# BerkIGuler/AdaFortiTran

Hardware: AMD Instinct MI355X
Metric: OFDM frames/sec (120x14 grid, batch 128) + channel-estimation MSE vs reference (higher is better)
Workload: dtype f32; 1 GPU; C3: AdaFortiTran default config (6 layers, d=128, 4 heads, adaptive tokens), 120x14 grid, pilots 12x2; 128 frames per GPU per step; step = model(pilots_cpu, meta_cpu) through the module surface + device MSE partial; value = SURVEY 8(d)'s metric: H2D of pilots + meta INSIDE the step, output left on the device (= value_h2d_inclusive); the bare engine call on inputs resident in HBM is value_resident;; frames_per_gpu=128, global_batch=128, parallelism=frames sharded over 1 rank(s), lanes=1

## Files before the change

### adafortitran_amd/_abi.py

```python
from __future__ import annotations

import ctypes as C
from typing import Callable, Dict, Optional

AFT_ABI_VERSION = 10
AFT_ENGINE_PACKED, AFT_ENGINE_GENERAL = 0, 1
AFT_OK, AFT_ERR_ARG, AFT_ERR_SHAPE, AFT_ERR_HIP = 0, 1, 2, 3
AFT_ACT_RELU, AFT_ACT_GELU = 0, 1
AFT_ENCODER_AUTO, AFT_ENCODER_LAUNCHES, AFT_ENCODER_PLANE = 0, 1, 2
AFT_PRECISION_F32, AFT_PRECISION_BF16X3 = 0, 1

_fp = C.c_void_p


class AftConfig(C.Structure):
    _fields_ = [
        ("num_scs", C.c_int32), ("num_symbols", C.c_int32),
        ("pilot_scs", C.c_int32), ("pilot_symbols", C.c_int32),
        ("patch_scs", C.c_int32), ("patch_symbols", C.c_int32),
        ("num_layers", C.c_int32), ("model_dim", C.c_int32), ("num_head", C.c_int32),
        ("activation", C.c_int32), ("adaptive", C.c_int32),
        ("hidden", C.c_int32 * 3), ("encoder_path", C.c_int32), ("precision", C.c_int32),
    ]

# ... 76 lines not shown
        ("layers", C.POINTER(AftLayerWeights)),
    ]


def make_config(*, ofdm, pilot, patch, num_layers: int, model_dim: int, num_head: int,
                activation: str = "gelu", adaptive_hidden=None) -> AftConfig:
    cfg = AftConfig()
    cfg.num_scs, cfg.num_symbols = int(ofdm[0]), int(ofdm[1])
    cfg.pilot_scs, cfg.pilot_symbols = int(pilot[0]), int(pilot[1])
    cfg.patch_scs, cfg.patch_symbols = int(patch[0]), int(patch[1])
    cfg.num_layers, cfg.model_dim, cfg.num_head = int(num_layers), int(model_dim), int(num_head)
    cfg.activation = AFT_ACT_GELU if activation == "gelu" else AFT_ACT_RELU
    cfg.adaptive = 1 if adaptive_hidden is not None else 0
    for i in range(3):
        cfg.hidden[i] = int(adaptive_hidden[i]) if adaptive_hidden is not None else 0
    return cfg


def config_from_pydantic(system_config, model_config, adaptive: bool) -> AftConfig:
    return make_config(
        ofdm=(system_config.ofdm.num_scs, system_config.ofdm.num_symbols),
        pilot=(system_config.pilot.num_scs, system_config.pilot.num_symbols),
        patch=tuple(model_config.patch_size), num_layers=model_config.num_layers,
        model_dim=model_config.model_dim, num_head=model_config.num_head,
        activation=model_config.activation,
        adaptive_hidden=tuple(model_config.channel_adaptivity_hidden_sizes) if adaptive else None)


_ENC = ("snr_encoder", "ds_encoder", "dop_encoder")
_TE = "transformer_encoder"


def make_weights(cfg: AftConfig, ptr: Callable[[str], int], pos_key: Optional[str] = None) -> AftWeights:
    w = AftWeights()
    w.up_w, w.up_b = ptr("pilot_upsampler.weight"), ptr("pilot_upsampler.bias")
    for i, slot in enumerate((0, 2, 4, 6)):
        w.enh_w[i] = ptr(f"initial_enhancer.conv_block.{slot}.weight")
        w.enh_b[i] = ptr(f"initial_enhancer.conv_block.{slot}.bias")
        w.ref_w[i] = ptr(f"final_refiner.conv_block.{slot}.weight")
        w.ref_b[i] = ptr(f"final_refiner.conv_block.{slot}.bias")
    if cfg.adaptive:
        for e, enc in enumerate(_ENC):
            for j, slot in enumerate((0, 2, 4)):
                w.ada_w[e][j] = ptr(f"channel_adapter.{enc}.{slot}.weight")
                w.ada_b[e][j] = ptr(f"channel_adapter.{enc}.{slot}.bias")
    w.lin1_w, w.lin1_b = ptr(f"{_TE}.linear_1.weight"), ptr(f"{_TE}.linear_1.bias")
    w.lin2_w, w.lin2_b = ptr(f"{_TE}.linear_2.weight"), ptr(f"{_TE}.linear_2.bias")
    w.pos = ptr(pos_key or f"{_TE}.positional_encoding.position_embeddings")
    table = (AftLayerWeights * cfg.num_layers)()
    w.layers = C.cast(table, C.POINTER(AftLayerWeights))
    w._layer_table = table
    for i in range(cfg.num_layers):
        lp = f"{_TE}.transformer.layers.{i}"
        lw = table[i]
        lw.in_proj_w, lw.in_proj_b = ptr(lp + ".self_attn.in_proj_weight"), ptr(lp + ".self_attn.in_proj_bias")
        lw.out_proj_w, lw.out_proj_b = ptr(lp + ".self_attn.out_proj.weight"), ptr(lp + ".self_attn.out_proj.bias")
        lw.lin1_w, lw.lin1_b = ptr(lp + ".linear1.weight"), ptr(lp + ".linear1.bias")
        lw.lin2_w, lw.lin2_b = ptr(lp + ".linear2.weight"), ptr(lp + ".linear2.bias")
        lw.norm1_w, lw.norm1_b = ptr(lp + ".norm1.weight"), ptr(lp + ".norm1.bias")
        lw.norm2_w, lw.norm2_b = ptr(lp + ".norm2.weight"), ptr(lp + ".norm2.bias")
    return w


def pos_key_of(state: Dict[str, object]) -> str:
    k = f"{_TE}.positional_encoding.position_embeddings"
    return k if k in state else f"{_TE}.positional_encoding.pe"


vp = C.c_void_p
cfgp, wp, lwp, lgp = C.POINTER(AftConfig), C.POINTER(AftWeights), C.POINTER(AftLayerWeights), C.POINTER(AftLayerGrads)
p3, p4, p9, i3 = C.POINTER(vp * 3), C.POINTER(vp * 4), C.POINTER(vp * 9), C.POINTER(C.c_int32 * 3)
i6 = [C.c_int] * 6
SIGNATURES = {
    "aft_version": (C.c_int, []),
    "aft_last_error": (C.c_char_p, []),
    "aft_check_config": (C.c_int, [cfgp]),
    "aft_engine_of": (C.c_int, [cfgp]),
    "aft_set_switch": (C.c_int, [C.c_char_p, C.c_char_p]),
    "aft_get_switch": (C.c_int, [C.c_char_p, C.c_char_p, C.c_size_t]),
    "aft_max_batch": (C.c_int, [cfgp]),
    "aft_workspace_bytes": (C.c_size_t, [cfgp, C.c_int]),
    "aft_workspace_bytes_layer_fused": (C.c_size_t, [cfgp, C.c_int]),
    "aft_layer_fused_of": (C.c_int, [cfgp, C.c_int]),
    "aft_workspace_lanes": (C.c_int, [cfgp, C.c_int, C.POINTER(C.c_int), C.POINTER(C.c_int), C.POINTER(C.c_size_t)]),
    "aft_workspace_region": (C.c_int, [cfgp, C.c_int, C.c_int, C.POINTER(C.c_size_t), C.POINTER(C.c_size_t)]),
    "aft_forward_f32": (C.c_int, [cfgp, wp, vp, vp, vp, vp, vp, vp, C.c_size_t, C.c_int, vp]),
    "aft_packed_weights_bytes": (C.c_size_t, [cfgp]),
    "aft_pack_weights_f32": (C.c_int, [cfgp, wp, vp, C.c_size_t, vp]),
    "aft_forward_prepacked_f32": (C.c_int, [cfgp, wp, vp, vp, vp, vp, vp, vp, vp, C.c_size_t, C.c_int, vp]),
    "aft_linear_forward_f32": (C.c_int, [vp, vp, vp, vp, C.c_int, C.c_int, C.c_int, vp]),
    "aft_mse_partial_f32": (C.c_int, [vp, vp, vp, C.c_longlong, vp]),
    "aft_pilot_gather_f32": (C.c_int, [vp, vp, vp, C.c_int, C.c_int, C.c_int, vp]),
    "aft_ls_mse_db_f32": (C.c_int, [vp, vp, vp, C.c_int, C.c_int, vp]),
    "aft_frame_gather_f32": (C.c_int, [vp, vp, vp, vp, vp, vp, C.c_int, C.c_longlong, C.c_int, C.c_int, vp]),
    "aft_channel_sim_f32": (C.c_int, [C.POINTER(AftChanSim), C.c_ulonglong] + [C.c_longlong] * 4 + [C.c_int, vp, vp, vp, vp]),
    "aft_channel_sim_group_f32": (C.c_int, [C.POINTER(AftChanSim), C.c_int, C.c_int, vp, C.c_ulonglong] + [C.c_longlong] * 4 +
                                  [C.c_int, vp, vp, vp, vp]),
    "aft_lmmse_table_floats": (C.c_size_t, [C.POINTER(AftLmmse)]),
    "aft_lmmse_f32": (C.c_int, [C.POINTER(AftLmmse), vp, vp, vp, vp, vp, vp, C.c_int, vp]),
    "aft_link_errors_f32": (C.c_int, [C.POINTER(AftLink), vp, vp, vp, vp, vp, C.c_int, vp]),
    "aft_link_soft_f32": (C.c_int, [C.POINTER(AftLink), vp, vp, vp, vp, vp, vp, C.c_int, vp, vp, C.c_int, vp]),
    "aft_link_decode_f32": (C.c_int, [C.POINTER(AftLink), vp, vp, C.c_int, C.c_int, C.c_ulonglong, C.c_ulonglong, C.c_float, vp, vp,
                                      C.c_int, vp]),
    "aft_link_ldpc_f32": (C.c_int, [C.POINTER(AftLink), vp, vp, C.c_int, C.c_int, vp, C.c_ulonglong, C.c_ulonglong, C.c_float, C.c_int,
                                    C.c_int, vp, vp, C.c_int, vp]),
    "aft_link_mrc_f32": (C.c_int, [C.POINTER(AftLink), vp, vp, vp, vp, vp, vp, vp, C.c_int, C.c_int, vp, vp, vp, C.c_int, vp]),
    "aft_link_harq_f32": (C.c_int, [C.POINTER(AftLink), vp, vp, C.c_int, C.c_int, vp, C.c_int, C.c_int, vp, C.c_ulonglong, C.c_ulonglong,
                                    C.c_float, C.c_int, C.c_int, vp, vp, C.c_int, vp]),
    "aft_link_sm_f32": (C.c_int, [C.POINTER(AftLink), vp, vp, vp, vp, vp, vp, vp, vp, C.c_int, C.c_int, C.c_int, vp, vp, vp, C.c_int, vp]),
    "aft_link_joint_f32": (C.c_int, [C.POINTER(AftLink), vp, vp, vp, vp, vp, vp, vp, C.c_int, C.c_int, C.c_int, vp, vp, vp, C.c_int, vp]),
    "aft_encoder_tape_bytes": (C.c_size_t, [cfgp, C.c_int]),
    "aft_encoder_train_scratch_bytes": (C.c_size_t, [cfgp, C.c_int]),
    "aft_encoder_layer_fwd_train_f32": (C.c_int, [cfgp, lwp, vp, vp, vp, C.c_size_t, vp, C.c_size_t, C.c_int, C.c_float, C.c_uint64, vp]),
    "aft_encoder_layer_fwd_train_chained_f32": (C.c_int, [cfgp, lwp, vp, vp, vp, C.c_size_t, vp, C.c_size_t, C.c_int, C.c_float, C.c_uint64,
                                                          C.c_int, lwp, vp, C.c_size_t, C.POINTER(C.c_int), vp]),
    "aft_encoder_layer_bwd_f32": (C.c_int, [cfgp, lwp, vp, vp, C.c_size_t, vp, vp, lgp, C.c_int, vp, C.c_size_t, C.c_int, C.c_float,
                                            C.c_uint64, vp]),
    "aft_dense_fwd_f32": (C.c_int, [vp, vp, vp, vp, C.c_int, C.c_int, C.c_int, vp]),
    "aft_dense_bwd_scratch_bytes": (C.c_size_t, [C.c_int, C.c_int, C.c_int]),
    "aft_dense_bwd_f32": (C.c_int, [vp, vp, vp, vp, vp, vp, C.c_int, vp, C.c_size_t, C.c_int, C.c_int, C.c_int, vp]),
    "aft_conv_enhancer_fwd_scratch_bytes": (C.c_size_t, [C.c_int, C.c_int, C.c_int]),
    "aft_conv_enhancer_fwd_train_f32": (C.c_int, [p4, p4, vp, vp, vp, vp, vp, vp, C.c_size_t, C.c_int, C.c_int, C.c_int, vp]),
    "aft_conv_enhancer_scratch_bytes": (C.c_size_t, [C.c_int, C.c_int, C.c_int]),
    "aft_conv_enhancer_bwd_f32": (C.c_int, [p4, vp, vp, vp, vp, vp, vp, p4, p4, C.c_int, vp, C.c_size_t, C.c_int, C.c_int, C.c_int, vp]),
    "aft_adapter_fwd_train_f32": (C.c_int, [p3, p9, p9, i3, C.c_int, C.c_int, vp, vp, vp, vp]),
    "aft_adapter_bwd_f32": (C.c_int, [p3, p9, p9, i3, C.c_int, C.c_int, vp, vp, vp, vp, vp, p9, p9, C.c_int, vp]),
    "aft_embed_bwd_scratch_bytes": (C.c_size_t, i6 + [C.c_int]),
    "aft_embed_fwd_train_f32": (C.c_int, [vp] * 6 + i6 + [vp]),
    "aft_embed_bwd_f32": (C.c_int, [vp] * 9 + [C.c_int, vp, C.c_size_t] + i6 + [vp]),
    "aft_tail_bwd_scratch_bytes": (C.c_size_t, i6),
    "aft_tail_fwd_train_f32": (C.c_int, [vp] * 5 + i6 + [vp]),
    "aft_tail_bwd_f32": (C.c_int, [vp] * 6 + [C.c_int, vp, C.c_size_t] + i6 + [vp]),
    "aft_adam_step_f32": (C.c_int, [vp, vp, vp, vp, C.c_size_t] + [C.c_float] * 6 + [C.c_int, vp]),
    "aft_grad_sumsq_scratch_bytes": (C.c_size_t, [C.c_size_t]),
    "aft_grad_sumsq_f32": (C.c_int, [vp, C.c_size_t, vp, C.c_size_t, vp, vp, vp]),
    "aft_adam_prepare_f32": (C.c_int, [vp, vp, vp, vp, C.c_double, C.c_double, C.c_float, C.c_float, vp]),
    "aft_adam_step_ctrl_f32": (C.c_int, [vp, vp, vp, vp, C.c_size_t] + [C.c_float] * 5 + [vp, vp]),
    "aft_grad_clip_f32": (C.c_int, [vp, C.c_size_t, vp, C.c_double, C.c_double, vp, vp]),
    "aft_stage_upsample_f32": (C.c_int, [cfgp, wp, vp, vp, C.c_int, vp]),
    "aft_stage_adapter_f32": (C.c_int, [cfgp, wp, vp, vp, vp, vp, C.c_int, vp]),
    "aft_stage_embed_f32": (C.c_int, [cfgp, wp, vp, vp, vp, C.c_int, vp]),
    "aft_stage_encoder_layer_f32": (C.c_int, [cfgp, wp, C.c_int, vp, vp, C.c_size_t, C.c_int, vp]),
    "aft_stage_tail_f32": (C.c_int, [cfgp, wp, vp, vp, vp, C.c_int, vp]),
    "aft_profile_kernel_f32": (C.c_int, [cfgp, wp, C.c_int, vp, vp, C.c_size_t, C.c_int, C.c_int, vp]),
    "aft_debug_fill_lds_f32": (C.c_int, [C.c_float, vp]),
    "aft_debug_peek_lds_f32": (C.c_int, [vp, C.c_int, C.c_int, vp]),
}
EXPORTED_SYMBOLS = tuple(SIGNATURES)
REGION_IDS = {"conv_enhanced": 0, "tokens6": 1, "enc_out": 2}
KERNEL_IDS = {"upsample": 0, "embed": 1, "qkv": 2, "attention": 3, "chain": 4, "tail": 5, "chain_last": 6, "prologue": 8}
```

### adafortitran_amd/csrc/aft_api.hip

```cpp
#include <algorithm>
#include <atomic>
#include <cstdlib>
#include <cstdarg>
#include <cstdio>
#include <cstring>
#include <mutex>
#include <string>
#include <vector>

#include "aft_internal.h"

namespace aft {

static thread_local char g_err[512] = "";

void set_error(const char *fmt, ...) {
    va_list ap;
    va_start(ap, fmt);
    vsnprintf(g_err, sizeof(g_err), fmt, ap);
    va_end(ap);
}

int hip_fail(const char *what, hipError_t e) {
    set_error("%s: %s", what, hipGetErrorString(e));
// ... 252 lines not shown
    p.planned = p.total;
    for (int i = 0; i < p.lanes && layer_fused_ok(c); ++i) {
        const size_t block = (size_t)2 * p.frames[i] * round_up(tokens_of(c), kTile) * c.model_dim;
        p.x_pt[i] = p.take(block);
        p.vt2[i] = p.take(block);
    }
    return p;
}
static size_t workspace_floats_any_lanes(const aft_config &c, int batch, bool fused_blocks) {
    size_t m = 0;
    for (int l = 1; l <= kMaxLanes; ++l) {
        const LanePlan lp = plan_lanes(c, batch, l);
        m = std::max(m, fused_blocks ? lp.total : lp.planned);
    }
    return m;
}
struct LaneStreams {
    hipStream_t side[kMaxLanes - 1];
    hipEvent_t fork, join[kMaxLanes - 1];
    int n_side;
};
namespace {
constexpr int kLaneCacheMax = 16;
struct LaneEntry { bool used; int dev; hipStream_t user; LaneStreams ls; int in_use; unsigned long long tick; };
std::mutex g_lane_mu;
LaneEntry g_lane_cache[kLaneCacheMax];
unsigned long long g_lane_tick = 0;
void destroy_lane_streams(LaneStreams &ls) {
    for (int i = 0; i < ls.n_side; ++i) {
        (void)hipEventDestroy(ls.join[i]);
        (void)hipStreamDestroy(ls.side[i]);
    }
    if (ls.fork) (void)hipEventDestroy(ls.fork);
    ls = LaneStreams{};
}
bool grow_lane_streams(LaneStreams &ls, int sides) {
    if (ls.fork == nullptr && hipEventCreateWithFlags(&ls.fork, hipEventDisableTiming) != hipSuccess) { ls.fork = nullptr; return false; }
    while (ls.n_side < sides) {
        hipStream_t s = nullptr;
        hipEvent_t e = nullptr;
        if (hipStreamCreateWithFlags(&s, hipStreamNonBlocking) != hipSuccess) return false;
        if (hipEventCreateWithFlags(&e, hipEventDisableTiming) != hipSuccess) { (void)hipStreamDestroy(s); return false; }
        ls.side[ls.n_side] = s;
        ls.join[ls.n_side] = e;
        ++ls.n_side;
    }
    return true;
}
}
static LaneStreams *acquire_lane_streams(hipStream_t user, int lanes) {
    int dev = 0;
    if (hipGetDevice(&dev) != hipSuccess) return nullptr;
    std::lock_guard<std::mutex> lock(g_lane_mu);
    LaneEntry *hit = nullptr, *victim = nullptr;
    for (auto &en : g_lane_cache) {
        if (en.used && en.dev == dev && en.user == user) { hit = &en; break; }
        if (!en.used) { if (victim == nullptr || victim->used) victim = &en; }
        else if (en.in_use == 0 && (victim == nullptr || (victim->used && en.tick < victim->tick))) victim = &en;
    }
    if (hit == nullptr) {
        if (victim == nullptr) return nullptr;
        if (victim->used) destroy_lane_streams(victim->ls);
        *victim = LaneEntry{true, dev, user, LaneStreams{}, 0, 0};
        hit = victim;
    }
    if (!grow_lane_streams(hit->ls, lanes - 1)) {
        if (hit->in_use == 0) {
            destroy_lane_streams(hit->ls);
            hit->used = false;
        }
        return nullptr;
    }
    ++hit->in_use;
    hit->tick = ++g_lane_tick;
    return &hit->ls;
}
static void release_lane_streams(LaneStreams *ls) {
    if (ls == nullptr) return;
    std::lock_guard<std::mutex> lock(g_lane_mu);
    for (auto &en : g_lane_cache)
        if (&en.ls == ls) { --en.in_use; return; }
}

static bool l0_fold_selected(const aft_config &c) {
    return packed_engine_ok(c) && c.precision == AFT_PRECISION_F32 && switch_int(SW_L0_FOLD, 1) != 0;
}
static L0Fold l0_fold_at(const aft_config &c, const Workspace &ws, float *base) {
    float *tables = base + ws.attn;
    return L0Fold{tables, tables + (size_t)ws.tokpad * c.model_dim, base + ws.wpack + (size_t)c.model_dim * c.model_dim};
}

enum ChainPos { kChainFirst, kChainMiddle, kChainLast };
static ChainFusion chain_fusion_for(ChainPos pos, const aft_config &c, const WeightsDev &w, const Workspace &ws, float *base) {
    ChainFusion f{};
    f.x_blocked = true;
    if (pos == kChainFirst) {
        f.conv_enhanced = base + ws.conv_enhanced;
        f.tokens6 = c.adaptive ? base + ws.tokens6 : nullptr;
        f.lin1_w = w.lin1_w; f.lin1_b = w.lin1_b; f.pos = w.pos;
    } else if (pos == kChainLast) {
        f.lin2_w = w.lin2_w; f.lin2_b = w.lin2_b; f.out6 = base + ws.out6;
    }
    return f;
}

static int run_encoder(const aft_config &c, const WeightsDev &w, const aft_layer_weights *layers, const Workspace &ws, float *base, float *x,
                       int first_layer, int last_layer, hipStream_t st, bool fused = false, const float *prepacked = nullptr,
                       float *x_pt = nullptr, float *vt2 = nullptr, const L0Fold *fold = nullptr) {
    float *attn = base + ws.attn, *q = base + ws.q, *k = base + ws.k, *vt = base + ws.vt;
    const int rows = ws.planes * ws.tokens;
    const size_t pl = packed_layer_floats(c.model_dim);
    const float *wp = prepacked != nullptr ? prepacked : base + ws.wpack;
    if (prepacked == nullptr)
        STEP("pack_weights", launch_pack_weights(c, layers + first_layer, base + ws.wpack + first_layer * pl, last_layer - first_layer + 1, st));
    ChainFusion first = chain_fusion_for(kChainFirst, c, w, ws, base);
    const ChainFusion middle = chain_fusion_for(kChainMiddle, c, w, ws, base), last = chain_fusion_for(kChainLast, c, w, ws, base);
    if (fused && fold != nullptr && first_layer == 0) {
        first.fold_tk = fold->tk; first.fold_tvt = fold->tvt; first.fold_w = fold->wf;
    }
    if (fused && x_pt != nullptr && x == base + ws.x && first_layer == 0 && last_layer == c.num_layers - 1 &&
        layer_fused_selected(c, ws.planes / 2)) {
        x = x_pt;
        float *kbuf[2] = {k, attn}, *vbuf[2] = {vt, vt2};
        STEP("chain(qkv, plane tiles)", launch_chain_plane_tiles(c, &layers[0], wp, x, q, kbuf[0], vbuf[0], ws.planes, ws.tokens, ws.tokpad, st, &first));
        for (int l = 0; l <= last_layer; ++l) {
            const bool more = l < last_layer;
            STEP("layer", launch_layer(c, &layers[l], wp + l * pl, more ? &layers[l + 1] : nullptr, more ? wp + (l + 1) * pl : nullptr, x, q,
                                       kbuf[l & 1], vbuf[l & 1], kbuf[(l + 1) & 1], vbuf[(l + 1) & 1], ws.planes, ws.tokens, ws.tokpad, st,
                                       more ? &middle : &last));
        }
        return AFT_OK;
    }
    STEP("chain(qkv)", launch_chain(c, nullptr, nullptr, &layers[first_layer], wp + first_layer * pl, nullptr, x, q, k, vt, rows,
                                    ws.tokens, ws.tokpad, st, fused ? &first : nullptr));
    for (int l = first_layer; l <= last_layer; ++l) {
        STEP("attention", launch_attention(c, q, k, vt, layers[l].in_proj_b, attn, ws.planes, ws.tokens, ws.tokpad, st));
        const bool more = l < last_layer;
        STEP("chain(mlp)", launch_chain(c, &layers[l], wp + l * pl, more ? &layers[l + 1] : nullptr, more ? wp + (l + 1) * pl : nullptr, attn,
                                        x, q, k, vt, rows, ws.tokens, ws.tokpad, st, fused ? (more ? &middle : &last) : nullptr));
    }
    return AFT_OK;
}

static int general_layer(const aft_config &c, const aft_layer_weights &lw, const Workspace &ws, float *base, float *x, hipStream_t st) {
    const int rows = ws.planes * ws.tokens, d = c.model_dim, ff = 2 * d;
    float *qkv = base + ws.g_qkv, *attn = base + ws.attn, *y = base + ws.g_y, *x1 = base + ws.g_x1, *s = base + ws.g_s,
          *stats = base + ws.g_stats, *a = base + ws.g_a, *hd = base + ws.g_hd;
    STEP("general: in-projection", launch_gemm(0, x, lw.in_proj_w, qkv, lw.in_proj_b, rows, 3 * d, d, d, d, 3 * d, false, st));
    STEP("general: attention", launch_attn_train_fwd(c, qkv, attn, base + ws.g_lse, ws.planes, ws.tokens, 0.f, 0u, st, base + ws.g_pad));
    STEP("general: out-projection", launch_gemm(0, attn, lw.out_proj_w, y, lw.out_proj_b, rows, d, d, d, d, d, false, st));
    STEP("general: norm1", launch_add_ln_fwd(x, y, lw.norm1_w, lw.norm1_b, s, stats, x1, rows, d, 1e-5f, 0.f, 0u, st));
    STEP("general: linear1", launch_gemm(0, x1, lw.lin1_w, a, lw.lin1_b, rows, ff, d, d, d, ff, false, st));
    STEP("general: activation", launch_act_fwd(c.activation, a, hd, rows, ff, 0.f, 0u, st));
    STEP("general: linear2", launch_gemm(0, hd, lw.lin2_w, y, lw.lin2_b, rows, d, ff, ff, ff, d, false, st));
    STEP("general: norm2", launch_add_ln_fwd(x1, y, lw.norm2_w, lw.norm2_b, s, stats, x, rows, d, 1e-5f, 0.f, 0u, st));
    return AFT_OK;
}
static int run_encoder_general(const aft_config &c, const WeightsDev &w, const aft_layer_weights *layers, const Workspace &ws, float *base,
                               int batch, hipStream_t st) {
    float *x = base + ws.x;
    const int rows = ws.planes * ws.tokens, d = c.model_dim, p = c.patch_scs * c.patch_symbols;
    STEP("general: embedding", launch_embed_any(c, w, base + ws.conv_enhanced, c.adaptive ? base + ws.tokens6 : nullptr, x, batch, st));
    for (int l = 0; l < c.num_layers; ++l) {
        const int rc = general_layer(c, layers[l], ws, base, x, st);
        if (rc != AFT_OK) return rc;
    }
    STEP("general: linear_2", launch_gemm(0, x, w.lin2_w, base + ws.out6, w.lin2_b, rows, p, d, d, d, out6_stride(c), false, st));
    return AFT_OK;
}

}

using namespace aft;

extern "C" {

int aft_version(void) { return AFT_ABI_VERSION; }

const char *aft_last_error(void) { return g_err; }

int aft_check_config(const aft_config *cfg) { return check_config(cfg); }

int aft_engine_of(const aft_config *cfg) {
    if (check_config(cfg) != AFT_OK) return -1;
    return packed_engine_ok(*cfg) ? AFT_ENGINE_PACKED : AFT_ENGINE_GENERAL;
}

int aft_set_switch(const char *name, const char *value) {
    const int i = name == nullptr ? -1 : switch_id(name);
    if (i < 0) {
        set_error("aft_set_switch: %s is not a switch (adafortitran_amd/csrc/switches.h lists them)", name ? name : "(null)");
        return AFT_ERR_ARG;
    }
    std::lock_guard<std::mutex> lock(g_switch_mu);
    store_switch(i, value);
    return AFT_OK;
}

int aft_get_switch(const char *name, char *buf, size_t n) {
    const int i = name == nullptr ? -1 : switch_id(name);
    if (i < 0) return -1;
    std::lock_guard<std::mutex> lock(g_switch_mu);
    if (!g_switch_on[i].load(std::memory_order_relaxed)) return 0;
    if (buf != nullptr && n > 0) {
        strncpy(buf, g_switch_text[i].c_str(), n - 1);
        buf[n - 1] = 0;
    }
    return 1;
}

int aft_max_batch(const aft_config *cfg) {
    if (check_config(cfg) != AFT_OK) return 0;
    return max_batch_of(*cfg);
}

size_t aft_workspace_bytes(const aft_config *cfg, int batch) {
    if (check_config(cfg) != AFT_OK || batch <= 0) return 0;
    return workspace_floats_any_lanes(*cfg, batch, false) * sizeof(float);
}

int aft_workspace_region(const aft_config *cfg, int batch, int region, size_t *offset_bytes, size_t *size_bytes) {
    int rc = check_config(cfg);
    if (rc != AFT_OK) return rc;
    if (batch <= 0 || !offset_bytes || !size_bytes) {
        set_error("aft_workspace_region: bad batch or NULL result pointer");
        return AFT_ERR_ARG;
    }
    const Workspace ws = plan_workspace(*cfg, batch);
    size_t off = 0;
    switch (region) {
        case AFT_REGION_CONV_ENHANCED: off = ws.conv_enhanced; break;
        case AFT_REGION_TOKENS6: off = ws.tokens6; break;
        case AFT_REGION_ENC_OUT: off = ws.out6; break;
        default: set_error("aft_workspace_region: unknown region %d", region); return AFT_ERR_ARG;
    }
    *offset_bytes = off * sizeof(float);
    *size_bytes = ws.floats_at(off) * sizeof(float);
    return AFT_OK;
}

size_t aft_workspace_bytes_layer_fused(const aft_config *cfg, int batch) {
    if (check_config(cfg) != AFT_OK || batch <= 0) return 0;
    return workspace_floats_any_lanes(*cfg, batch, true) * sizeof(float);
}

int aft_layer_fused_of(const aft_config *cfg, int batch) {
    if (check_config(cfg) != AFT_OK || batch <= 0) return -1;
    return layer_fused_selected(*cfg, batch) ? 1 : 0;
}

int aft_workspace_lanes(const aft_config *cfg, int batch, int *lanes, int *frames, size_t *offset_bytes) {
    int rc = check_config(cfg);
    if (rc != AFT_OK) return rc;
    if (batch <= 0 || !lanes || !frames || !offset_bytes) {
        set_error("aft_workspace_lanes: bad batch or NULL result pointer");
        return AFT_ERR_ARG;
    }
    static_assert(kMaxLanes == AFT_MAX_LANES, "header and implementation disagree");
    const LanePlan lp = plan_lanes(*cfg, batch, lanes_wanted(*cfg, batch));
    *lanes = lp.lanes;
    for (int i = 0; i < kMaxLanes; ++i) {
        frames[i] = i < lp.lanes ? lp.frames[i] : 0;
        offset_bytes[i] = i < lp.lanes ? lp.ws_off[i] * sizeof(float) : 0;
    }
    return AFT_OK;
}

static int forward_lane(const aft_config *cfg, const aft_weights *w, const float *prepacked, const float *pilots, const float *snr,
                        const float *ds, const float *dop, float *out, float *base, int batch, hipStream_t st, float *x_pt, float *vt2) {
    const Workspace ws = plan_workspace(*cfg, batch);
    const bool general = !packed_engine_ok(*cfg);
    const WeightsDev wd = weights_window(*w, 0, cfg->num_layers);
    float *wpack = prepacked != nullptr || general ? nullptr : base + ws.wpack;
    float *lent = x_holds_planes(*cfg, ws) ? base + ws.x : nullptr;
    float *up_planes = prologue_upsample_ok(*cfg, wd) ? lent : nullptr;
    const bool fold_on = l0_fold_selected(*cfg);
    const L0Fold fold = fold_on ? l0_fold_at(*cfg, ws, base) : L0Fold{};
    STEP("prologue(adapter + pack_weights + upsampler product)",
         launch_prologue(*cfg, wd, snr, ds, dop, base + ws.tokens6, batch, wpack, pilots, up_planes, st, base + ws.convfrag,
                         fold_on ? &fold : nullptr));
    if (wpack != nullptr && cfg->num_layers > kLayerWindow)
        STEP("pack_weights(layers beyond the prologue's window)",
             launch_pack_weights(*cfg, w->layers + kLayerWindow, wpack + packed_layer_floats(cfg->model_dim) * kLayerWindow,
                                 cfg->num_layers - kLayerWindow, st));
    STEP("upsample", launch_upsample(*cfg, wd, pilots, base + ws.conv_enhanced, batch, st, lent, up_planes != nullptr, base + ws.convfrag));
    const int rc = general ? run_encoder_general(*cfg, wd, w->layers, ws, base, batch, st)
                           : run_encoder(*cfg, wd, w->layers, ws, base, base + ws.x, 0, cfg->num_layers - 1, st, true,
                                         prepacked != nullptr ? prepacked : wpack, x_pt, vt2, fold_on ? &fold : nullptr);
    if (rc != AFT_OK) return rc;
    STEP("tail", launch_tail(*cfg, wd, nullptr, base + ws.conv_enhanced, out, batch, st, base + ws.out6, base + ws.convfrag + kConvFragFloats));
    return AFT_OK;
}

static int forward_impl(const aft_config *cfg, const aft_weights *w, const float *prepacked, const float *pilots,
                        const float *snr, const float *ds, const float *dop, float *out, void *workspace,
                        size_t workspace_bytes, int batch, void *stream) {
    int rc = check_config(cfg);
    if (rc != AFT_OK) return rc;
    AFT_REQUIRE(w && pilots && out && workspace, "NULL pointer argument");
    AFT_REQUIRE(batch > 0, "batch must be positive (got %d)", batch);
    AFT_REQUIRE(batch <= max_batch_of(*cfg), "batch %d exceeds aft_max_batch = %d for this configuration (32-bit buffer "
                "offsets: no workspace region may reach 2 GiB); split the batch", batch, max_batch_of(*cfg));
    AFT_REQUIRE(!cfg->adaptive || (snr && ds && dop), "meta_data is required when channel adaptation is enabled");
    hipStream_t user = static_cast<hipStream_t>(stream);
    AFT_REQUIRE(w->layers != nullptr, "aft_weights.layers is NULL (host array of num_layers entries)");
    const LanePlan lp = plan_lanes(*cfg, batch, lanes_wanted(*cfg, batch));
    AFT_REQUIRE(workspace_bytes >= lp.planned * sizeof(float), "workspace too small: %zu < %zu bytes (aft_workspace_bytes)",
                workspace_bytes, lp.planned * sizeof(float));
    const bool fused_blocks = lp.total > lp.planned && workspace_bytes >= lp.total * sizeof(float);
    LaneStreams *ls = lp.lanes > 1 ? acquire_lane_streams(user, lp.lanes) : nullptr;
    struct Lease { LaneStreams *p; ~Lease() { release_lane_streams(p); } } lease{ls};
    if (ls != nullptr) {
        hipError_t ef = hipEventRecord(ls->fork, user);
        for (int i = 1; i < lp.lanes && ef == hipSuccess; ++i) ef = hipStreamWaitEvent(ls->side[i - 1], ls->fork, 0);
        if (ef != hipSuccess) return hip_fail("lanes(fork)", ef);
    }
    const int pil_floats = 2 * cfg->pilot_scs * cfg->pilot_symbols, out_floats = 2 * cfg->num_scs * cfg->num_symbols;
#ifdef AFT_CHECKED
    {
        int covered = 0;
        for (int i = 0; i < lp.lanes; ++i) {
            const Workspace wl = plan_workspace(*cfg, lp.frames[i]);
            AFT_HOST_ASSERT(lp.first[i] == covered && lp.frames[i] > 0, "lane shares are not a partition of the batch");
            covered += lp.frames[i];
            AFT_HOST_ASSERT(lp.ws_off[i] % 64 == 0 && (lp.ws_off[i] + wl.total) * sizeof(float) <= workspace_bytes, "lane slice outside the workspace");
            AFT_HOST_ASSERT(i + 1 == lp.lanes || lp.ws_off[i] + wl.total <= lp.ws_off[i + 1], "lane slices overlap");
            AFT_HOST_ASSERT(check_layout(wl, workspace_bytes - lp.ws_off[i] * sizeof(float)), "workspace region outside its slice");
        }
        AFT_HOST_ASSERT(covered == batch, "lane shares do not cover the batch");
        AFT_HOST_ASSERT(!fused_blocks || check_layout(lp, workspace_bytes), "fused layer sequence's blocks outside the workspace");
    }
#endif
    int result = AFT_OK;
    for (int i = 0; i < lp.lanes; ++i) {
        const int f0 = lp.first[i];
        const int rc_lane = forward_lane(cfg, w, prepacked, pilots + (size_t)f0 * pil_floats, snr ? snr + f0 : nullptr, ds ? ds + f0 : nullptr,
                                         dop ? dop + f0 : nullptr, out + (size_t)f0 * out_floats, static_cast<float *>(workspace) + lp.ws_off[i],
                                         lp.frames[i], i == 0 || ls == nullptr ? user : ls->side[i - 1],
                                         fused_blocks ? static_cast<float *>(workspace) + lp.x_pt[i] : nullptr,
                                         fused_blocks ? static_cast<float *>(workspace) + lp.vt2[i] : nullptr);
        if (rc_lane != AFT_OK && result == AFT_OK) result = rc_lane;
    }
    if (ls != nullptr) {
        hipError_t ej = hipSuccess;
        for (int i = 1; i < lp.lanes && ej == hipSuccess; ++i) {
            ej = hipEventRecord(ls->join[i - 1], ls->side[i - 1]);
            if (ej == hipSuccess) ej = hipStreamWaitEvent(user, ls->join[i - 1], 0);
        }
        if (ej != hipSuccess && result == AFT_OK) return hip_fail("lanes(join)", ej);
    }
    return result;
}

int aft_forward_f32(const aft_config *cfg, const aft_weights *w, const float *pilots, const float *snr,
                    const float *ds, const float *dop, float *out, void *workspace, size_t workspace_bytes,
                    int batch, void *stream) {
    return forward_impl(cfg, w, nullptr, pilots, snr, ds, dop, out, workspace, workspace_bytes, batch, stream);
}

size_t aft_packed_weights_bytes(const aft_config *cfg) {
// ... 87 lines not shown
                           int batch, void *stream) {
    int rc = check_config(cfg);
    if (rc != AFT_OK) return rc;
    AFT_REQUIRE(w && pilots && conv_enhanced && batch > 0, "bad argument");
    hipError_t e = launch_upsample(*cfg, weights_window(*w, 0, 0), pilots, conv_enhanced, batch, static_cast<hipStream_t>(stream));
    return e == hipSuccess ? AFT_OK : hip_fail("upsample", e);
}

int aft_stage_adapter_f32(const aft_config *cfg, const aft_weights *w, const float *snr, const float *ds,
                          const float *dop, float *tokens6, int batch, void *stream) {
    int rc = check_config(cfg);
    if (rc != AFT_OK) return rc;
    AFT_REQUIRE(cfg->adaptive, "adapter stage needs an adaptive config");
    AFT_REQUIRE(w && snr && ds && dop && tokens6 && batch > 0, "bad argument");
    hipError_t e = launch_adapter(*cfg, weights_window(*w, 0, 0), snr, ds, dop, tokens6, batch, static_cast<hipStream_t>(stream));
    return e == hipSuccess ? AFT_OK : hip_fail("adapter", e);
}

int aft_stage_embed_f32(const aft_config *cfg, const aft_weights *w, const float *conv_enhanced,
                        const float *tokens6, float *x, int batch, void *stream) {
    int rc = check_config(cfg);
    if (rc != AFT_OK) return rc;
    AFT_REQUIRE(w && conv_enhanced && x && batch > 0, "bad argument");
    AFT_REQUIRE(!cfg->adaptive || tokens6, "adaptive config needs tokens6");
    hipError_t e = packed_engine_ok(*cfg) ? launch_embed(*cfg, weights_window(*w, 0, 0), conv_enhanced, tokens6, x, batch, static_cast<hipStream_t>(stream))
                                          : launch_embed_any(*cfg, weights_window(*w, 0, 0), conv_enhanced, tokens6, x, batch, static_cast<hipStream_t>(stream));
    return e == hipSuccess ? AFT_OK : hip_fail("embed", e);
}

int aft_stage_encoder_layer_f32(const aft_config *cfg, const aft_weights *w, int layer, float *x, void *scratch,
                                size_t scratch_bytes, int batch, void *stream) {
    int rc = check_config(cfg);
    if (rc != AFT_OK) return rc;
    AFT_REQUIRE(w && w->layers && x && scratch && batch > 0, "bad argument");
    AFT_REQUIRE(layer >= 0 && layer < cfg->num_layers, "layer %d out of range", layer);
    AFT_REQUIRE(batch <= max_batch_of(*cfg), "batch %d exceeds aft_max_batch = %d", batch, max_batch_of(*cfg));
    const Workspace ws = plan_workspace(*cfg, batch);
    AFT_REQUIRE(scratch_bytes >= ws.total * sizeof(float), "scratch too small");
    float *base = static_cast<float *>(scratch);
    hipStream_t st = static_cast<hipStream_t>(stream);
    if (!packed_engine_ok(*cfg)) return general_layer(*cfg, w->layers[layer], ws, base, x, st);
    return run_encoder(*cfg, weights_window(*w, 0, 0), w->layers, ws, base, x, layer, layer, st);
}

int aft_stage_tail_f32(const aft_config *cfg, const aft_weights *w, const float *x, const float *conv_enhanced,
                       float *out, int batch, void *stream) {
    int rc = check_config(cfg);
    if (rc != AFT_OK) return rc;
    AFT_REQUIRE(w && x && conv_enhanced && out && batch > 0, "bad argument");
    {
        const int p = cfg->patch_scs * cfg->patch_symbols;
        if (cfg->model_dim % 16 != 0 || !conv_plan_ok(cfg->num_scs, cfg->num_symbols, p * cfg->model_dim + p)) {
            set_error("aft_stage_tail_f32: linear_2 (%d x %d) does not fit the conv kernel's LDS beside the plane, or model_dim is not a "
                      "multiple of 16 -- only aft_forward_f32 serves this configuration", p, cfg->model_dim);
            return AFT_ERR_SHAPE;
        }
    }
    hipError_t e = launch_tail(*cfg, weights_window(*w, 0, 0), x, conv_enhanced, out, batch, static_cast<hipStream_t>(stream));
    return e == hipSuccess ? AFT_OK : hip_fail("tail", e);
}

int aft_profile_kernel_f32(const aft_config *cfg, const aft_weights *w, int which, float *out, void *workspace,
                           size_t workspace_bytes, int batch, int reps, void *stream) {
    int rc = check_config(cfg);
    if (rc != AFT_OK) return rc;
    AFT_REQUIRE(w && w->layers && workspace && batch > 0 && reps > 0, "bad argument");
    AFT_REQUIRE(batch <= max_batch_of(*cfg), "batch %d exceeds aft_max_batch = %d", batch, max_batch_of(*cfg));
    if (!packed_engine_ok(*cfg)) {
        set_error("aft_profile_kernel_f32 replays the packed engine's kernel classes; this configuration runs the general engine");
        return AFT_ERR_SHAPE;
    }
    const Workspace ws = plan_workspace(*cfg, batch);
    AFT_REQUIRE(workspace_bytes >= ws.total * sizeof(float), "workspace too small");
    const WeightsDev wd = weights_window(*w, 0, cfg->num_layers);
    AFT_REQUIRE(cfg->num_layers >= 2 || which != AFT_KERNEL_CHAIN, "chain profile needs >= 2 layers");
    hipStream_t st = static_cast<hipStream_t>(stream);
    float *base = static_cast<float *>(workspace);
    float *x = base + ws.x, *attn = base + ws.attn, *q = base + ws.q, *k = base + ws.k, *vt = base + ws.vt;
    const int rows = ws.planes * ws.tokens;
    float *lent = x_holds_planes(*cfg, ws) ? x : nullptr;
    const float *wp = base + ws.wpack;
    ChainFusion first = chain_fusion_for(kChainFirst, *cfg, wd, ws, base);
    const ChainFusion middle = chain_fusion_for(kChainMiddle, *cfg, wd, ws, base), last = chain_fusion_for(kChainLast, *cfg, wd, ws, base);
    const bool fold_on = l0_fold_selected(*cfg);
    const L0Fold fold = fold_on ? l0_fold_at(*cfg, ws, base) : L0Fold{};
    if (fold_on) { first.fold_tk = fold.tk; first.fold_tvt = fold.tvt; first.fold_w = fold.wf; }
    hipError_t e = hipSuccess;
    for (int i = 0; i < reps && e == hipSuccess; ++i) {
        switch (which) {
            case AFT_KERNEL_UPSAMPLE:
                AFT_REQUIRE(out != nullptr, "upsample profile needs the pilots pointer in `out`");
                e = launch_upsample(*cfg, wd, out, base + ws.conv_enhanced, batch, st, lent, prologue_upsample_ok(*cfg, wd), base + ws.convfrag);
                break;
            case AFT_KERNEL_EMBED:
                e = launch_embed(*cfg, wd, base + ws.conv_enhanced, cfg->adaptive ? base + ws.tokens6 : nullptr, x, batch, st);
                break;
            case AFT_KERNEL_QKV:
                e = launch_chain(*cfg, nullptr, nullptr, &w->layers[0], wp, nullptr, x, q, k, vt, rows, ws.tokens, ws.tokpad, st, &first);
                break;
            case AFT_KERNEL_ATTENTION:
                e = launch_attention(*cfg, q, k, vt, w->layers[0].in_proj_b, attn, ws.planes, ws.tokens, ws.tokpad, st);
                break;
            case AFT_KERNEL_CHAIN:
                e = launch_chain(*cfg, &w->layers[0], wp, &w->layers[1], wp + packed_layer_floats(cfg->model_dim), attn, x, q, k, vt, rows,
                                 ws.tokens, ws.tokpad, st, &middle);
                break;
            case AFT_KERNEL_CHAIN_LAST:
                e = launch_chain(*cfg, &w->layers[0], wp, nullptr, nullptr, attn, x, q, k, vt, rows, ws.tokens, ws.tokpad, st, &last);
                break;
            case AFT_KERNEL_PROLOGUE: {
                AFT_REQUIRE(out != nullptr, "prologue profile needs the pilots pointer in `out`");
                const float *cond = out + (size_t)batch * cfg->pilot_scs * cfg->pilot_symbols * 2;
                e = launch_prologue(*cfg, wd, cond, cond + batch, cond + 2 * batch, base + ws.tokens6, batch, base + ws.wpack, out,
                                    prologue_upsample_ok(*cfg, wd) && !switch_on(SW_PROLOGUE_NO_UP) ? lent : nullptr, st,
                                    base + ws.convfrag, fold_on ? &fold : nullptr);
                break;
            }
            case AFT_KERNEL_TAIL:
                AFT_REQUIRE(out != nullptr, "tail profile needs an output buffer");
                e = launch_tail(*cfg, wd, nullptr, base + ws.conv_enhanced, out, batch, st, base + ws.out6, base + ws.convfrag + kConvFragFloats);
                break;
            default:
                set_error("unknown kernel id %d", which);
                return AFT_ERR_ARG;
        }
    }
    return e == hipSuccess ? AFT_OK : hip_fail("profile", e);
}

}
```

### adafortitran_amd/csrc/aft_internal.h

```cpp
#pragma once

#include <hip/hip_runtime.h>

#include <cstddef>
#include <cstdint>

#include "../../include/adafortitran_amd.h"
#include "switches.h"
#ifdef AFT_DIAG_STAMPS
#include "stamp_report.h"
#endif

namespace aft {

using f32x2 = __attribute__((ext_vector_type(2))) float;
using f32x4 = __attribute__((ext_vector_type(4))) float;
using f32x16 = __attribute__((ext_vector_type(16))) float;

constexpr int kWave = 64;
constexpr int kHeadDim = 32;
constexpr int kTile = 32;
constexpr int kMaxPatchFeatures = 16;

inline __host__ __device__ int round_up(int v, int m) { return (v + m - 1) / m * m; }
// ... 109 lines not shown
            if (regions[i].off == off) return regions[i].floats;
        return 0;
    }
};
inline bool check_layout(const Layout &l, size_t bytes) {
    if (l.n > kMaxRegions || l.total % 64 != 0 || l.total * sizeof(float) > bytes) return false;
    for (int i = 0; i < l.n; ++i) {
        const size_t end = i + 1 < l.n ? l.regions[i + 1].off : l.total;
        if (l.regions[i].off % 64 != 0 || l.regions[i].off + l.regions[i].floats > end) return false;
    }
    return true;
}

inline int tokens_of(const aft_config &c) { return (c.num_scs / c.patch_scs) * (c.num_symbols / c.patch_symbols); }

struct Workspace : Layout {
    size_t conv_enhanced, tokens6, x, attn, q, k, vt, wpack, out6, convfrag;
    size_t g_x1, g_y, g_s, g_stats, g_qkv, g_lse, g_a, g_hd, g_pad;
    int tokens, tokpad, planes;
};

Workspace plan_workspace(const aft_config &c, int batch);

void set_error(const char *fmt, ...);
int hip_fail(const char *what, hipError_t e);
#define STEP(name, call)                                    \
    do {                                                    \
        hipError_t e_ = (call);                             \
        if (e_ != hipSuccess) return hip_fail(name, e_);    \
    } while (0)
#define AFT_REQUIRE(cond, ...) do { if (!(cond)) { set_error(__VA_ARGS__); return AFT_ERR_ARG; } } while (0)
int check_config(const aft_config *c);
bool packed_engine_ok(const aft_config &c);

constexpr int kLayerWindow = 32;
struct WeightsDev {
    const float *up_w, *up_b;
    const float *enh_w[4], *enh_b[4];
    const float *ref_w[4], *ref_b[4];
    const float *ada_w[3][3], *ada_b[3][3];
    const float *lin1_w, *lin1_b;
    const float *pos;
    const float *lin2_w, *lin2_b;
    aft_layer_weights layers[kLayerWindow];
};
WeightsDev weights_window(const aft_weights &w, int first, int count);

constexpr int kMaxDevices = 64;
int current_device();
int current_device_cus();
struct PerDeviceOnce {
    unsigned long long done = 0;
    bool needed(int dev) const { return !((__atomic_load_n(&done, __ATOMIC_RELAXED) >> dev) & 1ull); }
    void mark(int dev) { __atomic_fetch_or(&done, 1ull << dev, __ATOMIC_RELAXED); }
};
hipError_t ensure_dynamic_lds(PerDeviceOnce &once, const void *kernel, size_t bytes);

#ifdef AFT_DIAG_STAMPS
enum StampKind { kStampChainQkv, kStampChainMlpQkv, kStampChainMlp, kStampAttn, kStampConv, kStampConvStream, kStampChainTrain, kStampKinds };
class StampRun {
public:
    StampRun(Switch sw, StampKind kind, long long rows, hipStream_t st);
    unsigned long long *buffer() const { return dev_; }
    const unsigned long long *collect();
private:
    unsigned long long *dev_ = nullptr;
    std::vector<unsigned long long> host_;
    StampKind kind_;
    long long rows_;
    hipStream_t st_;
};
#endif

constexpr size_t kConvFragFloats = 22 * 64 * 4 + 160;
hipError_t launch_upsample(const aft_config &c, const WeightsDev &w, const float *pilots,
                           float *conv_enhanced, int batch, hipStream_t st, float *scratch_planes = nullptr, bool planes_ready = false,
                           const float *conv_frag = nullptr);
hipError_t launch_adapter(const aft_config &c, const WeightsDev &w, const float *snr, const float *ds,
                          const float *dop, float *tokens6, int batch, hipStream_t st);
bool prologue_upsample_ok(const aft_config &c, const WeightsDev &w);
constexpr int kFoldSteps = (kMaxPatchFeatures + 6 + 1) / 2;
struct L0Fold {
    float *tk, *tvt, *wf;
};
hipError_t launch_prologue(const aft_config &c, const WeightsDev &w, const float *snr, const float *ds, const float *dop,
                           float *tokens6, int batch, float *packed, const float *pilots, float *up_planes, hipStream_t st,
                           float *conv_frag = nullptr, const L0Fold *fold = nullptr);
hipError_t launch_embed(const aft_config &c, const WeightsDev &w, const float *conv_enhanced,
                        const float *tokens6, float *x, int batch, hipStream_t st);
constexpr int kMaxPatchGeneral = 32;
hipError_t launch_embed_any(const aft_config &c, const WeightsDev &w, const float *conv_enhanced,
                            const float *tokens6, float *x, int batch, hipStream_t st);
struct ChainFusion {
    const float *conv_enhanced = nullptr, *tokens6 = nullptr, *lin1_w = nullptr, *lin1_b = nullptr, *pos = nullptr;
    const float *lin2_w = nullptr, *lin2_b = nullptr;
    float *out6 = nullptr;
    const float *fold_tk = nullptr, *fold_tvt = nullptr, *fold_w = nullptr;
    bool x_blocked = false;
};
inline int out6_stride(const aft_config &c) { return round_up(c.patch_scs * c.patch_symbols, 8); }
hipError_t launch_chain(const aft_config &c, const aft_layer_weights *mlp_w, const float *mlp_packed,
                        const aft_layer_weights *qkv_w, const float *qkv_packed, const float *attn, float *x,
                        float *q, float *k, float *vt, int rows, int tokens, int tokpad, hipStream_t st,
                        const ChainFusion *fuse = nullptr);
size_t packed_layer_floats(int d);
bool layer_fused_ok(const aft_config &c);
hipError_t launch_chain_plane_tiles(const aft_config &c, const aft_layer_weights *qkv_w, const float *qkv_packed, float *x, float *q,
                                    float *k, float *vt, int planes, int tokens, int tokpad, hipStream_t st, const ChainFusion *fuse);
hipError_t launch_layer(const aft_config &c, const aft_layer_weights *mlp_w, const float *mlp_packed, const aft_layer_weights *qkv_w,
                        const float *qkv_packed, float *x, float *q, const float *k_in, const float *vt_in, float *k_out, float *vt_out,
                        int planes, int tokens, int tokpad, hipStream_t st, const ChainFusion *fuse);
hipError_t launch_pack_weights(const aft_config &c, const aft_layer_weights *layers, float *packed, int count, hipStream_t st);
hipError_t launch_attention(const aft_config &c, const float *q, const float *k, const float *vt, const float *qbias,
                            float *attn, int planes, int tokens, int tokpad, hipStream_t st);
bool conv_plan_ok(int S, int T, int extra_floats);
hipError_t launch_tail(const aft_config &c, const WeightsDev &w, const float *x, const float *conv_enhanced,
                       float *out, int batch, hipStream_t st, const float *out6 = nullptr, const float *conv_frag = nullptr);
hipError_t launch_linear(const float *weight, const float *bias, const float *pilots, float *out, int batch,
                         int in_features, int out_features, hipStream_t st);
hipError_t launch_pilot_gather(const float *hzero_ls, float *pilots, int *counts, int batch, int grid_elems,
                               int expected, hipStream_t st);
hipError_t launch_ls_mse_db(const float *ls, const float *ideal, float *db, int batch, int grid_elems, hipStream_t st);
hipError_t launch_frame_gather(const float *ideal_all, const float *pilots_all, const long long *index, float *ideal_out,
                               float *pilots_out, int *flags, int batch, long long frames, int grid_elems, int pilot_elems,
                               hipStream_t st);
hipError_t launch_channel_sim(const aft_chansim &sim, unsigned long long seed, long long base, long long start, long long stride,
                              long long modulo, int batch, float *ideal, float *pilots, float *meta, hipStream_t st);
hipError_t launch_channel_sim_group(const aft_chansim &sim, int group, const float *mix_packed, unsigned long long seed, long long base,
                                    long long start, long long stride, long long modulo, int batch, float *ideal, float *pilots,
                                    float *meta, hipStream_t st);

size_t lmmse_fblock_floats(const aft_lmmse &plan);
size_t lmmse_tblock_floats(const aft_lmmse &plan);
hipError_t launch_lmmse(const aft_lmmse &plan, const float *tables, const float *pilots, const float *snr, const float *ds,
                        const float *dop, float *est, int batch, hipStream_t st);
hipError_t launch_link_errors(const aft_link &link, const float *ideal, const float *est, const unsigned long long *keys,
                              const float *sigma, int32_t *counts, int batch, hipStream_t st);
hipError_t launch_link_soft(const aft_link &link, const float *ideal, const float *est, const unsigned long long *keys,
                            const float *sigma, const float *scale, const float *factors, int n_factors, float *loss, float *llr,
                            int batch, hipStream_t st);
hipError_t launch_link_mrc(const aft_link &link, const float *ideal, const float *est, const unsigned long long *keys,
                           const float *sigma, const float *rho, const float *scale, const float *factors, int n_factors, int branches,
                           int32_t *counts, float *loss, float *llr, int batch, hipStream_t st);
int link_code_waves(unsigned steps, unsigned blocks);
hipError_t launch_link_decode(const aft_link &link, const float *llr, const unsigned long long *keys, int info_bits, int rate,
                              unsigned coded_bits, unsigned blocks, unsigned long long stride, float qgain, int32_t *counts,
                              unsigned char *bits, int batch, hipStream_t st);
int link_ldpc_waves(int base_cols, int edges, unsigned blocks);
hipError_t launch_link_ldpc(const aft_link &link, const float *llr, const unsigned long long *keys, int base_rows, int base_cols,
                            const int32_t *shifts, unsigned blocks, unsigned long long stride, float qgain, int offset, int max_iters,
                            int32_t *counts, unsigned char *bits, int batch, hipStream_t st);
int link_harq_waves(int base_cols, int edges, unsigned blocks);
hipError_t launch_link_harq(const aft_link &link, const float *llr, const unsigned long long *keys, int base_rows, int base_cols,
                            const int32_t *shifts, int tx_cols, int rounds, const int32_t *starts, unsigned blocks,
                            unsigned long long stride, float qgain, int offset, int max_iters, int32_t *counts, unsigned char *bits,
                            int batch, hipStream_t st);
hipError_t launch_link2(bool joint, const aft_link &link, const float *ideal, const float *est, const unsigned long long *keys,
                        const float *sigma, const float *rho, const float *scale, const float *reg, const float *factors, int n_factors,
                        int branches, int32_t *counts, float *loss, float *llr, int batch, hipStream_t st);
hipError_t launch_mse(const float *est, const float *ref, double *sum_sq, long long n_complex, hipStream_t st);
hipError_t launch_fill_lds(float value, hipStream_t st);
hipError_t launch_peek_lds(float *out, int workgroups, int n, hipStream_t st);


constexpr int kGemmMaxSlices = 256;
constexpr int kColsumMaxSlices = 1024;
int colsum_slices(int rows);
int gemm_split_slices(int rows, int tiles);
size_t gemm_tn_slice_floats(int M, int N, int R);
constexpr int kMaxReduceJobs = 12;
struct ReduceJobs;
struct ReduceBatchScope {
    ReduceJobs *jobs;
    ReduceBatchScope();
    ~ReduceBatchScope();
    hipError_t flush(hipStream_t st);
    ReduceBatchScope(const ReduceBatchScope &) = delete;
    ReduceBatchScope &operator=(const ReduceBatchScope &) = delete;
};
int ln_bwd_blocks(int rows);
hipError_t launch_gemm(int op, const float *A, const float *B, float *C, const float *bias, int M, int N, int K, int lda,
                       int ldb, int ldc, bool accumulate, hipStream_t st);
hipError_t launch_gemm_tn(const float *A, const float *B, float *C, float *slices, int M, int N, int R, int lda, int ldb,
                          bool accumulate, hipStream_t st);
bool gemm_add_ln_ok(int M, int N, int K, int lda, int ldb);
hipError_t launch_gemm_add_ln(const float *A, const float *W, const float *bias, const float *res, const float *gamma,
                              const float *beta, float *s_out, float *stats, float *out, int M, int N, int K, int lda, int ldw,
                              float eps, float keep_scale, uint32_t threshold, uint32_t seed, hipStream_t st);
bool gemm_act_ok(int M, int N, int K, int lda, int ldb, int ldc);
hipError_t launch_gemm_act(const float *A, const float *W, const float *bias, float *a_out, float *hd, int M, int N, int K, int lda,
                           int ldw, int ldc, int activation, float keep_scale, uint32_t threshold, uint32_t seed, hipStream_t st);
bool gemm_actbwd_ok(int M, int N, int K, int lda, int ldb, int ldc);
hipError_t launch_gemm_actbwd(const float *dy, const float *W, const float *a, float *da, int M, int N, int K, int lda, int ldw,
                              int ldc, int activation, float keep_scale, uint32_t threshold, uint32_t seed, hipStream_t st);
// ... 79 lines not shown
```

### adafortitran_amd/csrc/attn_device.h

```cpp
#pragma once
#include <math.h>

#include <type_traits>

#include "aft_internal.h"
#include "srd.h"
#include "stamps.h"

namespace aft {

#ifndef AFT_ATTN_WAVES
#define AFT_ATTN_WAVES 3
#endif

constexpr float kRescaleThreshold = 64.0f;
constexpr float kZeroRefThreshold = 32.0f;

__device__ __forceinline__ float other_half(float x) {
    const unsigned u = __builtin_bit_cast(unsigned, x);
    const auto r = __builtin_amdgcn_permlane32_swap(u, u, false, false);
    return __builtin_bit_cast(float, (threadIdx.x & 32) ? r[0] : r[1]);
}

__device__ __forceinline__ float max16(const f32x16 &v) {
    float m = __builtin_fmaxf(v[0], v[1]);
#pragma unroll
    for (int e = 2; e < 16; e += 2) m = __builtin_fmaxf(__builtin_fmaxf(m, v[e]), v[e + 1]);
    return m;
}

template <int NB, int NMF = 16 * NB>
__device__ __forceinline__ f32x16 qk_tile(const f32x4 (&kreg)[NB][4], const f32x4 (&qreg)[NB][4], bool zero_ref, float a_one,
                                          float neg_m) {
    f32x16 c;
    if (zero_ref) {
        c = mfma_f32(kreg[0][0][0], qreg[0][0][0], f32x16{0});
    } else {
        c = mfma_f32(a_one, neg_m, f32x16{0});
        c = mfma_f32(kreg[0][0][0], qreg[0][0][0], c);
    }
#pragma unroll
    for (int i = 1; i < NMF; ++i) c = mfma_f32(kreg[i >> 4][(i >> 2) & 3][i & 3], qreg[i >> 4][(i >> 2) & 3][i & 3], c);
    return c;
}

template <int NB>
struct AttnRow {
    float m_ref;
    f32x2 lsum2;
    f32x16 oacc[NB];
    bool zero_ref;
};

__device__ __forceinline__ f32x16 qk_tile_bs(const f32x4 (&kreg)[4], const f32x4 (&qreg)[4], bool zero_ref, float neg_m, int h) {
    f32x16 c = f32x16{0};
    if (!zero_ref) {
        bf16x8 one = {}, mref = {};
        one[0] = (__bf16)(h == 0 ? 1.0f : 0.0f);
        mref[0] = (__bf16)(h == 0 ? neg_m : 0.0f);
        c = __builtin_amdgcn_mfma_f32_32x32x16_bf16(one, mref, c, 0, 0, 0);
    }
#pragma unroll
    for (int m = 0; m < 2; ++m) {
        const bf16x8 kh = __builtin_bit_cast(bf16x8, kreg[2 * m]), kl = __builtin_bit_cast(bf16x8, kreg[2 * m + 1]);
        const bf16x8 qh = __builtin_bit_cast(bf16x8, qreg[2 * m]), ql = __builtin_bit_cast(bf16x8, qreg[2 * m + 1]);
        c = __builtin_amdgcn_mfma_f32_32x32x16_bf16(kh, qh, c, 0, 0, 0);
        c = __builtin_amdgcn_mfma_f32_32x32x16_bf16(kh, ql, c, 0, 0, 0);
        c = __builtin_amdgcn_mfma_f32_32x32x16_bf16(kl, qh, c, 0, 0, 0);
    }
    return c;
}
__device__ __forceinline__ float round_to_bf16(float x) { return (float)(__bf16)x; }

template <bool BS = false, int HD = 32, int TOK = 0, bool SINK = false>
__device__ __forceinline__ void attn_body(const float *__restrict__ q, const float *__restrict__ k,
                                          const float *__restrict__ vt, const float *__restrict__ qbias,
                                          float *__restrict__ out, int nblk, int tokens_rt, int tokpad_rt, int model_dim,
                                          float scale_log2e, const int first_task, const int total_waves, int ntasks,
                                          unsigned long long *stamps, const int tail_task = -1, float *sink = nullptr) {
    static_assert(!SINK || (!BS && HD == 32), "the LDS sink is instantiated for the fp32 head-dimension-32 body");
    int lane_l = threadIdx.x & 63;
    asm volatile("" : "+v"(lane_l));
    const int lane = lane_l;
    const Srd qs = make_srd(q), ks = make_srd(k), vs = make_srd(vt), os = make_srd(out);
    static_assert(HD % 8 == 0 && HD >= 8 && HD <= 64 && HD != 56, "head dimension");
    static_assert(!BS || HD == 32, "the split-precision tier is instantiated for head dimension 32");
    static_assert(HD != 16, "head dimension 16 runs attn16_body (attn16_device.h)");
    constexpr bool GEN = HD != 32 && HD != 64;
    constexpr int NS = HD / 8;
    constexpr int NB = GEN ? (32 % HD == 0 ? 1 : 2) : HD == 64 ? 2 : 1;
    constexpr int NQ = GEN ? (NS + 3) / 4 : NB;
    const int heads = model_dim / HD;
    const int tokens = TOK > 0 ? TOK : tokens_rt;
    const int tokpad = TOK > 0 ? (TOK + kTile - 1) / kTile * kTile : tokpad_rt;
    const int nkt = tokpad / kTile;
    const int r = lane & 31, h = lane >> 5;
    const bool ragged = (tokens & (kTile - 1)) != 0;
    const float a_one = h == 0 ? 1.0f : 0.0f;
    auto first_group = [&](int task) { const int ph = task / nkt, plane = ph / heads; return plane * nblk * 4 + (ph - plane * heads) * NS; };
    auto first_block = [&](int task) {
        if constexpr (GEN) return first_group(task) >> 2;
        return task / nkt * NB;
    };
    auto head_base = [&](int task) { return ((unsigned)first_block(task) * tokpad * kHeadDim + lane * 4) * 4; };
    const unsigned blk_bytes = (unsigned)tokpad * kHeadDim * 4;
    auto second_block_bytes = [&](int task) {
        if constexpr (GEN && NB == 2) return ((first_group(task) + NS - 1) >> 2) != first_block(task) ? blk_bytes : 0u;
        return blk_bytes;
    };
    auto load_tile = [&](Srd src, int kt, f32x4 (&dst)[NB][4], unsigned base, unsigned b1_bytes) {
#pragma unroll
        for (int b = 0; b < NB; ++b)
#pragma unroll
            for (int s = 0; s < 4; ++s) dst[b][s] = srd_load(src, base + b * b1_bytes + (unsigned)(kt * 1024 + s * 256) * 4);
    };
    constexpr int NMF = GEN ? 4 * NS : 16 * NB;
    auto load_qk = [&](Srd src, int kt, f32x4 (&dst)[NQ][4], unsigned base, int sub_) {
        if constexpr (GEN) {
#pragma unroll
            for (int i = 0; i < NS; ++i) {
                const int sl = sub_ + i;
                dst[i >> 2][i & 3] = srd_load(src, base + (unsigned)(sl >> 2) * blk_bytes + (unsigned)(kt * 1024 + (sl & 3) * 256) * 4);
            }
        } else {
            load_tile(src, kt, dst, base, blk_bytes);
        }
    };
    auto sub_of = [&](int task) {
        if constexpr (GEN) return first_group(task) & 3;
        return 0;
    };
    const bool pad8 = (tokens & 7) == 0;
    auto mask_logits = [&](f32x16 &sv, int kt) {
        if (pad8) {
#pragma unroll
            for (int g = 0; g < 4; ++g)
                if (kt * kTile + 8 * g >= tokens) sv[4 * g] = sv[4 * g + 1] = sv[4 * g + 2] = sv[4 * g + 3] = -INFINITY;
            return;
        }
#pragma unroll
        for (int e = 0; e < 16; ++e)
            if (kt * kTile + (e & 3) + 8 * (e >> 2) + 4 * h >= tokens) sv[e] = -INFINITY;
    };
    auto mask_values = [&](f32x4 (&vvb)[NB][4], int kt) {
      if (!BS && pad8) return;
#pragma unroll
      for (int b = 0; b < NB; ++b) {
        f32x4 (&vv)[4] = vvb[b];
        if constexpr (BS) {
#pragma unroll
            for (int sl = 0; sl < 4; ++sl) {
                bf16x8 e = __builtin_bit_cast(bf16x8, vv[sl]);
#pragma unroll
                for (int j = 0; j < 8; ++j)
                    if (kt * kTile + 16 * (sl >> 1) + 8 * (j >> 2) + 4 * h + (j & 3) >= tokens) e[j] = (__bf16)0.0f;
                vv[sl] = __builtin_bit_cast(f32x4, e);
            }
        } else {
#pragma unroll
            for (int g = 0; g < 4; ++g)
#pragma unroll
                for (int j = 0; j < 4; ++j)
                    if (kt * kTile + 8 * g + 4 * h + j >= tokens) vv[g][j] = 0.f;
        }
      }
    };

  const int rounds = SINK ? 1 : (ntasks + total_waves - 1) / total_waves + (tail_task >= 0 ? 1 : 0);
  int round = 0;
  int task = first_task < ntasks ? first_task : tail_task;
  f32x4 qreg[NQ][4], kcur[NQ][4], vcur[NB][4];
  if (task >= 0) {
      const unsigned hb0 = head_base(task);
      load_qk(qs, task % nkt, qreg, hb0, sub_of(task));
      load_qk(ks, 0, kcur, hb0, sub_of(task));
      load_tile(vs, 0, vcur, hb0, second_block_bytes(task));
  }
  for (; task >= 0; ++round) {
    AFT_STAMP(lane == 0, stamps, task, 0);
    AFT_STAMP_WALL(lane == 0, stamps, task, 6);
    const int qt = task % nkt;
    const int pb = first_block(task);
    const int sub = sub_of(task);
    const unsigned hb = head_base(task);
    const unsigned vb1 = second_block_bytes(task);
    const int next_task = SINK || task >= ntasks ? -1 : (task + total_waves < ntasks ? task + total_waves : tail_task);
    const bool has_next = next_task >= 0;

    if constexpr (!BS) {
        const float *bq = qbias + (pb % nblk) * kHeadDim + 4 * h + (GEN ? 8 * sub : 0);
#pragma unroll
        for (int b = 0; b < NQ; ++b)
#pragma unroll
            for (int s = 0; s < 4; ++s)
                if (4 * b + s < (GEN ? NS : 4 * NB))
                    qreg[b][s] = (qreg[b][s] + *reinterpret_cast<const f32x4 *>(bq + 32 * b + 8 * s)) * scale_log2e;
    }
    if (ragged && qt == nkt - 1 && qt * kTile + r >= tokens) {
#pragma unroll
        for (int b = 0; b < NQ; ++b)
#pragma unroll
            for (int s = 0; s < 4; ++s)
                if (4 * b + s < (GEN ? NS : 4 * NB)) qreg[b][s] = f32x4{0.f, 0.f, 0.f, 0.f};
    }

    AttnRow<NB> st;
    f32x16 sA, sB;
    if constexpr (BS) sA = qk_tile_bs(kcur[0], qreg[0], true, 0.f, h);
    else sA = qk_tile<NQ, NMF>(kcur, qreg, true, a_one, 0.f);
    if (nkt > 1) load_qk(ks, 1, kcur, hb, sub);
    if (ragged && nkt == 1) { mask_logits(sA, 0); mask_values(vcur, 0); }
    {
        float m0 = max16(sA);
        m0 = fmaxf(m0, other_half(m0));
        if constexpr (BS) m0 = round_to_bf16(m0);
        st.zero_ref = !__any(fabsf(m0) > kZeroRefThreshold);
        st.m_ref = st.zero_ref ? 0.f : m0;
        if (!st.zero_ref) {
#pragma unroll
            for (int e = 0; e < 16; ++e) sA[e] -= m0;
        }
    }
#pragma unroll
    for (int b = 0; b < NB; ++b) st.oacc[b] = f32x16{0};
    st.lsum2 = f32x2{0.f, 0.f};
    AFT_STAMP(lane == 0, stamps, task, 1);

    auto step = [&](auto fast, f32x16 &cur, f32x16 &nxt, int kt) {
        constexpr bool FAST = decltype(fast)::value;
        set_progress_priority((rounds - 1 - round) * nkt + (nkt - 1 - kt), rounds * nkt);
        const bool more = FAST || kt + 1 < nkt;
        if (more) {
            if constexpr (BS) nxt = qk_tile_bs(kcur[0], qreg[0], st.zero_ref, -st.m_ref, h);
            else nxt = qk_tile<NQ, NMF>(kcur, qreg, st.zero_ref, a_one, -st.m_ref);
            if (FAST || kt + 2 < nkt) load_qk(ks, kt + 2, kcur, hb, sub);
        } else if (has_next) {
            const unsigned hbn = head_base(next_task);
            load_qk(qs, next_task % nkt, qreg, hbn, sub_of(next_task));
            load_qk(ks, 0, kcur, hbn, sub_of(next_task));
        }
        const float tmax = max16(cur);
        if (__builtin_expect(__any(tmax > kRescaleThreshold), 0)) {
            const float tm = fmaxf(tmax, other_half(tmax));
            float grow = fmaxf(tm, 0.f);
            if constexpr (BS) grow = round_to_bf16(st.m_ref + grow) - st.m_ref;
            const float f = __builtin_amdgcn_exp2f(-grow);
            st.m_ref += grow;
            st.zero_ref = false;
#pragma unroll
            for (int e = 0; e < 16; ++e) {
                cur[e] -= grow;
                if (more) nxt[e] -= grow;
#pragma unroll
                for (int b = 0; b < NB; ++b) st.oacc[b][e] *= f;
            }
            st.lsum2 *= f;
        }
        if (!FAST && ragged && more && kt + 2 == nkt) mask_logits(nxt, kt + 1);
        f32x16 p;
// ... 82 lines not shown
```

### adafortitran_amd/csrc/chain_device.h

```cpp
#pragma once
#include "aft_internal.h"
#include "srd.h"
#include "stamps.h"

namespace aft {

template <int D>
struct ChainShape {
    static constexpr int WAVES = D / 32;
    static constexpr int THREADS = 64 * WAVES;
    static constexpr int XB = WAVES * 1024;
    static constexpr int HB = 2 * WAVES * 1024;
    static constexpr int ST = 32 * WAVES * 2;
    static constexpr int PAR = 4 * D;
    static constexpr size_t LDS_BYTES = sizeof(float) * (size_t)(XB + HB + ST + PAR);
};

struct ChainArgs {
    const float *attn;
    float *x;
    const float *wo, *w1, *w2, *wqkv;
    const float *bo, *b1, *b2, *g1, *be1, *g2, *be2;
    const float *bv;
    float *q, *k, *vt;
    int rows, tokens, tokpad, heads;
    int x_blocked;
    const float *lin2_w, *lin2_b;
    float *out6;
    int out6_features, out6_stride;
    const float *emb_conv, *emb_tok6, *emb_w1, *emb_b1, *emb_pos;
    int emb_S, emb_T, emb_p0, emb_p1, emb_K;
    const float *fold_tk;
    const float *fold_tvt;
    const float *fold_w;
    unsigned long long *stamps;
    int tpp;
};

ChainArgs make_chain_args(const aft_config &c, const aft_layer_weights *mlp_w, const float *mlp_packed, const aft_layer_weights *qkv_w,
                          const float *qkv_packed, const float *attn, float *x, float *q, float *k, float *vt, int rows, int tokens,
                          int tokpad, const ChainFusion *fuse);

template <int NT, int PFS>
struct WRing {
    f32x4 b[PFS + 1][NT];
};


template <int NKB, int NT, int PFS, int TS>
__device__ __forceinline__ void ring_load(WRing<NT, PFS> &ring, Srd w, unsigned w_lane, int step) {
    const int kb = step >> 2, s = step & 3;
#pragma unroll
    for (int t = 0; t < NT; ++t)
        ring.b[step % (PFS + 1)][t] = srd_load_c(w, w_lane, (unsigned)((t * TS * NKB + kb) * 1024 + s * 256) * 4);
}

template <int NKB, int NT, int PFS, int TS>
__device__ __forceinline__ void gemm_preload(WRing<NT, PFS> &ring, Srd w, unsigned w_lane) {
#pragma unroll
    for (int p = 0; p < PFS && p < 4 * NKB; ++p) ring_load<NKB, NT, PFS, TS>(ring, w, w_lane, p);
    __builtin_amdgcn_sched_barrier(0);
}

template <int NKB, int NT, int PFS, int TS, unsigned NORMAL, class Act, unsigned ZERO = 0>
__device__ __forceinline__ void gemm_run(WRing<NT, PFS> &ring, Srd w, unsigned w_lane, f32x16 (&acc)[NT], Act act) {
#pragma unroll
    for (int step = 0; step < 4 * NKB; ++step) {
        if (step + PFS < 4 * NKB) ring_load<NKB, NT, PFS, TS>(ring, w, w_lane, step + PFS);
        __builtin_amdgcn_sched_barrier(0);
        const f32x4 a = act(step >> 2, step & 3);
#pragma unroll
        for (int t = 0; t < NT; ++t)
#pragma unroll
            for (int j = 0; j < 4; ++j) {
                const float wv = ring.b[step % (PFS + 1)][t][j];
                if (((ZERO >> t) & 1) && step == 0 && j == 0)
                    acc[t] = (NORMAL >> t) & 1 ? __builtin_amdgcn_mfma_f32_32x32x2f32(a[j], wv, f32x16{0}, 0, 0, 0)
                                               : __builtin_amdgcn_mfma_f32_32x32x2f32(wv, a[j], f32x16{0}, 0, 0, 0);
                else
                    acc[t] = (NORMAL >> t) & 1 ? __builtin_amdgcn_mfma_f32_32x32x2f32(a[j], wv, acc[t], 0, 0, 0)
                                               : __builtin_amdgcn_mfma_f32_32x32x2f32(wv, a[j], acc[t], 0, 0, 0);
            }
        __builtin_amdgcn_sched_barrier(0);
    }
}

__device__ __forceinline__ void bs_publish(float *buf, int block, int lane, const f32x16 &v) {
#pragma unroll
    for (int m = 0; m < 2; ++m) {
        const BsFrag f = bs_split(f32x4{v[8 * m], v[8 * m + 1], v[8 * m + 2], v[8 * m + 3]},
                                  f32x4{v[8 * m + 4], v[8 * m + 5], v[8 * m + 6], v[8 * m + 7]});
        *reinterpret_cast<f32x4 *>(buf + (block * 4 + 2 * m) * 256 + lane * 4) = f.hi;
        *reinterpret_cast<f32x4 *>(buf + (block * 4 + 2 * m + 1) * 256 + lane * 4) = f.lo;
    }
}
__device__ __forceinline__ BsFrag bs_fetch(const float *buf, int kb, int m, int lane) {
    return BsFrag{*reinterpret_cast<const f32x4 *>(buf + (kb * 4 + 2 * m) * 256 + lane * 4),
                  *reinterpret_cast<const f32x4 *>(buf + (kb * 4 + 2 * m + 1) * 256 + lane * 4)};
}

template <int NKB, int NT, int PFS, int TS, unsigned NORMAL, class Act, unsigned ZERO = 0>
__device__ __forceinline__ void gemm_run_bs(WRing<NT, PFS> &ring, Srd w, unsigned w_lane, f32x16 (&acc)[NT], Act act) {
    BsFrag bfrag{};
#pragma unroll
    for (int step = 0; step < 4 * NKB; ++step) {
        if (step + PFS < 4 * NKB) ring_load<NKB, NT, PFS, TS>(ring, w, w_lane, step + PFS);
        __builtin_amdgcn_sched_barrier(0);
        const bool lo_step = step & 1;
        if (!lo_step) bfrag = act(step >> 2, (step & 3) >> 1);
        const bf16x8 bh = __builtin_bit_cast(bf16x8, bfrag.hi), bl = __builtin_bit_cast(bf16x8, bfrag.lo);
#pragma unroll
        for (int t = 0; t < NT; ++t) {
            const bf16x8 wv = __builtin_bit_cast(bf16x8, ring.b[step % (PFS + 1)][t]);
            const bool normal = (NORMAL >> t) & 1;
            if (((ZERO >> t) & 1) && step == 0)
                acc[t] = normal ? __builtin_amdgcn_mfma_f32_32x32x16_bf16(bh, wv, f32x16{0}, 0, 0, 0)
                                : __builtin_amdgcn_mfma_f32_32x32x16_bf16(wv, bh, f32x16{0}, 0, 0, 0);
            else
                acc[t] = normal ? __builtin_amdgcn_mfma_f32_32x32x16_bf16(bh, wv, acc[t], 0, 0, 0)
                                : __builtin_amdgcn_mfma_f32_32x32x16_bf16(wv, bh, acc[t], 0, 0, 0);
            if (!lo_step)
                acc[t] = normal ? __builtin_amdgcn_mfma_f32_32x32x16_bf16(bl, wv, acc[t], 0, 0, 0)
                                : __builtin_amdgcn_mfma_f32_32x32x16_bf16(wv, bl, acc[t], 0, 0, 0);
        }
        __builtin_amdgcn_sched_barrier(0);
    }
}

template <int D>
__device__ __forceinline__ void layernorm_rows(f32x16 &v, float *stats, const float *gamma, const float *beta,
                                               int wave, int r, int h) {
    constexpr int W = D / 32;
    float s = 0.f;
#pragma unroll
    for (int e = 0; e < 16; ++e) s += v[e];
    const float mp = s * (1.0f / 16.0f);
    float m2 = 0.f;
#pragma unroll
    for (int e = 0; e < 16; ++e) m2 = fmaf(v[e] - mp, v[e] - mp, m2);
    const float mo = __shfl_xor(mp, 32), m2o = __shfl_xor(m2, 32);
    const float dlt = mp - mo;
    if (h == 0) *reinterpret_cast<float2 *>(stats + (r * W + wave) * 2) = make_float2(0.5f * (mp + mo), m2 + m2o + 8.0f * dlt * dlt);
    __syncthreads();
    float mean = 0.f, msum = 0.f;
    float pm[W], pM[W];
#pragma unroll
    for (int u = 0; u < W; ++u) {
        const float2 p = *reinterpret_cast<const float2 *>(stats + (r * W + u) * 2);
        pm[u] = p.x;
        pM[u] = p.y;
        mean += p.x;
    }
    mean *= (1.0f / W);
#pragma unroll
    for (int u = 0; u < W; ++u) msum += pM[u] + 32.0f * (pm[u] - mean) * (pm[u] - mean);
    const float rstd = rsqrtf(msum * (1.0f / D) + 1e-5f);
#pragma unroll
    for (int s4 = 0; s4 < 4; ++s4) {
        const f32x4 g = *reinterpret_cast<const f32x4 *>(gamma + 8 * s4 + 4 * h);
        const f32x4 b = *reinterpret_cast<const f32x4 *>(beta + 8 * s4 + 4 * h);
#pragma unroll
        for (int j = 0; j < 4; ++j) v[4 * s4 + j] = (v[4 * s4 + j] - mean) * rstd * g[j] + b[j];
    }
}

__device__ __forceinline__ f32x16 bias_acc(Srd bias, int f0, int h) {
    f32x16 acc;
#pragma unroll
    for (int s = 0; s < 4; ++s) {
        const f32x4 b = srd_load(bias, (unsigned)(f0 + 8 * s + 4 * h) * 4);
#pragma unroll
        for (int j = 0; j < 4; ++j) acc[4 * s + j] = b[j];
    }
    return acc;
}

struct ChainNoPre {
    __device__ __forceinline__ void operator()(int) const {}
};

template <int D, int ACT, bool MLP, bool QKV, bool BS = false, bool PT = false, class Pre = ChainNoPre>
__device__ __forceinline__ void chain_body(const ChainArgs &a, float *smem, const int tid_in, const int first_tile,
                                           const int tile_stride, const int tile_end, Pre pre = Pre{}) {
    using S = ChainShape<D>;
    constexpr int W = S::WAVES;
    static_assert(!PT || !BS, "plane-aligned tiles are instantiated for the fp32 body");
    int tid = tid_in;
    asm volatile("" : "+v"(tid));
    float *xb = smem;
    float *hb = xb + S::XB;
    float *stats = hb + S::HB;
    float *par = stats + S::ST;

    int lane = tid & 63;
    const int w = __builtin_amdgcn_readfirstlane(tid >> 6);
    int r = lane & 31, h = lane >> 5;
    const int fb = 32 * w;

    const Srd srd_wo = make_srd(a.wo), srd_w1 = make_srd(a.w1), srd_w2 = make_srd(a.w2), srd_wq = make_srd(a.wqkv);
    const Srd srd_attn = make_srd(a.attn), srd_x = make_srd(a.x);
    const Srd srd_bo = make_srd(a.bo), srd_b1 = make_srd(a.b1), srd_b2 = make_srd(a.b2);
    const Srd srd_q = make_srd(a.q), srd_k = make_srd(a.k), srd_vt = make_srd(a.vt);
    const unsigned wo_off = (unsigned)w * W * 1024 + lane * 4, w1_off = (unsigned)(2 * w) * W * 1024 + lane * 4;
    const unsigned w2_off = (unsigned)w * (2 * W) * 1024 + lane * 4;
    const unsigned wq_off = (unsigned)w * W * 1024 + lane * 4;
    const Srd srd_bv = make_srd(a.bv);

    if constexpr (MLP) {
        for (int i = tid; i < D; i += S::THREADS) {
            par[i] = a.g1[i];
            par[D + i] = a.be1[i];
            par[2 * D + i] = a.g2[i];
            par[3 * D + i] = a.be2[i];
        }
        __syncthreads();
    }
    constexpr int kEmbSteps = kFoldSteps;
    constexpr int kFoldSteps0 = 6;
    float *emb_w = hb + S::XB;
    int *emb_offs = reinterpret_cast<int *>(emb_w + D * (kMaxPatchFeatures + 6));
    if constexpr (!MLP) {
        if (a.emb_conv != nullptr) {
            const int pk = a.emb_p0 * a.emb_p1;
            for (int i = tid; i < D * a.emb_K; i += S::THREADS) emb_w[i] = a.emb_w1[i];
            for (int k = tid; k < a.emb_K; k += S::THREADS)
                emb_offs[k] = k < pk ? (k / a.emb_p1) * a.emb_T + k % a.emb_p1 : ~(k - pk);
            __syncthreads();
        }
    }
    const int ntiles = (a.rows + 31) / 32;
    const int rounds = (tile_end - first_tile + tile_stride - 1) / tile_stride;
    int round = 0;
#ifndef AFT_CHAIN_PFK
#define AFT_CHAIN_PFK 0
#endif
    constexpr int PFK = MLP ? (AFT_CHAIN_PFK < W ? AFT_CHAIN_PFK : W) : 0;
    constexpr bool AHEAD = AFT_CHAIN_PFK > 0;
    static_assert(!PT || !AHEAD, "plane-aligned tiles request a tile's operands at the tile's start");
    f32x4 of[MLP ? W : 1][4], xres[4];
    auto request_attn = [&](int t, int kb0, int kb1) {
        const unsigned ap = ((unsigned)t * W * 1024 + lane * 4) * 4;
#pragma unroll
        for (int kb = 0; kb < W; ++kb)
#pragma unroll
            for (int s = 0; s < 4; ++s)
                if (kb >= kb0 && kb < kb1) of[kb][s] = srd_load_c(srd_attn, ap, (unsigned)(kb * 1024 + s * 256) * 4);
    };
    auto request_x_pt = [&](int t, int valid) {
        const unsigned xr = ((unsigned)t * 32 * D + w * 1024 + (min(r, valid - 1) + 32 * h) * 4) * 4;
#pragma unroll
        for (int s = 0; s < 4; ++s) xres[s] = srd_load(srd_x, xr + 1024 * s);
    };
    auto request_x = [&](int t) {
        if (a.x_blocked) {
            const unsigned xr = ((unsigned)t * 32 * D + w * 1024 + lane * 4) * 4;
#pragma unroll
            for (int s = 0; s < 4; ++s) xres[s] = srd_load(srd_x, xr + 1024 * s);
        } else {
            const unsigned xr = ((unsigned)min(t * 32 + r, a.rows - 1) * D + fb + 4 * h) * 4;
#pragma unroll
            for (int s = 0; s < 4; ++s) xres[s] = srd_load(srd_x, xr + 32 * s);
        }
    };
    auto request_tile = [&](int t) {
        if constexpr (MLP) request_attn(t, 0, PFK);
        if (MLP || a.emb_conv == nullptr) request_x(t);
    };
    if (AHEAD && first_tile < ntiles) request_tile(first_tile);
    f32x16 emb_acc0;
    float emb_bv[kEmbSteps];
    auto emb_request = [&](int t) {
        int plane, tok;
        if constexpr (PT) {
            plane = t / a.tpp;
            tok = min((t - plane * a.tpp) * 32 + r, a.tokens - 1);
        } else {
            const int grow_n = min(t * 32 + r, a.rows - 1);
            plane = grow_n / a.tokens;
            tok = grow_n - plane * a.tokens;
        }
        const int tpr = a.emb_T / a.emb_p1, g = tok / tpr, tc = tok - g * tpr;
        const float *cplane = a.emb_conv + ((size_t)plane * a.emb_S + g * a.emb_p0) * a.emb_T + tc * a.emb_p1;
        const float *t6 = a.emb_tok6 ? a.emb_tok6 + ((size_t)(plane >> 1) * a.tokens + tok) * 6 : nullptr;
#pragma unroll
        for (int s = 0; s < 4; ++s) {
            const f32x4 b = *reinterpret_cast<const f32x4 *>(a.emb_b1 + fb + 8 * s + 4 * h);
            const f32x4 ps = *reinterpret_cast<const f32x4 *>(a.emb_pos + (size_t)tok * D + fb + 8 * s + 4 * h);
#pragma unroll
            for (int j = 0; j < 4; ++j) emb_acc0[4 * s + j] = b[j] + ps[j];
        }
#pragma unroll
        for (int st = 0; st < kEmbSteps; ++st) {
            const int k = 2 * st + h;
            emb_bv[st] = 0.f;
            if (k < a.emb_K) {
                const int off = emb_offs[k];
                emb_bv[st] = off >= 0 ? cplane[off] : t6[~off];
            }
        }
    };
    if constexpr (!MLP) {
        if (a.emb_conv != nullptr && first_tile < tile_end) emb_request(first_tile);
    }
    bool fold = false;
    if constexpr (!MLP && !BS) fold = a.emb_conv != nullptr && a.fold_tk != nullptr;
    const Srd srd_tk = make_srd(a.fold_tk), srd_tvt = make_srd(a.fold_tvt), srd_fw = make_srd(a.fold_w);
    int pending_row0 = -1, pending_valid = 0;
    auto reduce_out6 = [&]() {
        const int P = a.out6_features;
        if (PT ? r < pending_valid : pending_row0 + r < a.rows) {
#pragma unroll
            for (int half = 0; half < 2; ++half) {
                const int f0 = 8 * half + 4 * h;
                if (f0 < P) {
                    f32x4 sum = *reinterpret_cast<const f32x4 *>(hb + lane * 8 + 4 * half);
#pragma unroll
                    for (int u = 1; u < W; ++u) {
                        const f32x4 t = *reinterpret_cast<const f32x4 *>(hb + (u * 64 + lane) * 8 + 4 * half);
                        sum += t;
                    }
#pragma unroll
                    for (int j = 0; j < 4; ++j) sum[j] += f0 + j < P ? a.lin2_b[f0 + j] : 0.f;
                    *reinterpret_cast<f32x4 *>(a.out6 + (size_t)(pending_row0 + r) * a.out6_stride + f0) = sum;
                }
            }
        }
    };
#pragma unroll 1
  for (int tile = first_tile; tile < tile_end; tile += tile_stride, ++round) {
    if constexpr (MLP && !QKV) {
        if (pending_row0 >= 0 && w == (round & (W - 1 < 3 ? W - 1 : 3))) reduce_out6();
    }
    pre(tile);
    if constexpr (PT && MLP) {
        int tid2 = tid_in;
        asm volatile("" : "+v"(tid2));
        lane = tid2 & 63;
        r = lane & 31;
        h = lane >> 5;
    }
#ifndef AFT_NO_PROGRESS_PRIORITY
    {
        const int left = rounds - 1 - round;
        if (left >= 3) __builtin_amdgcn_s_setprio(3);
        else if (left == 2) __builtin_amdgcn_s_setprio(2);
        else if (left == 1) __builtin_amdgcn_s_setprio(1);
        else __builtin_amdgcn_s_setprio(0);
    }
#endif
    const int row0 = tile * 32;
    const int grow = min(row0 + r, a.rows - 1);
    int plane_pt = 0, qt_pt = 0, valid_pt = 32;
    if constexpr (PT) {
        plane_pt = tile / a.tpp;
        qt_pt = tile - plane_pt * a.tpp;
        valid_pt = min(32, a.tokens - qt_pt * 32);
    }
    const bool row_ok = PT ? r < valid_pt : row0 + r < a.rows;
    const bool blocked = PT || a.x_blocked;
    const unsigned xrow = ((unsigned)grow * D + fb + 4 * h) * 4;
    unsigned lo = 0;
    asm volatile("" : "+v"(lo));
    const unsigned lo_lane = PT && MLP ? lo + lane * 4 : lo;
    const unsigned wo_lane = ((PT && MLP ? (unsigned)w * W * 1024 : wo_off) + lo_lane) * 4,
                   w1_lane = ((PT && MLP ? (unsigned)(2 * w) * W * 1024 : w1_off) + lo_lane) * 4,
                   w2_lane = ((PT && MLP ? (unsigned)w * (2 * W) * 1024 : w2_off) + lo_lane) * 4,
                   wq_lane = ((PT && MLP ? (unsigned)w * W * 1024 : wq_off) + lo_lane) * 4;
    AFT_STAMP(tid == 0, a.stamps, tile, 0);
    AFT_STAMP_WALL(tid == 0, a.stamps, tile, 12);
    AFT_STAMP_VALUE(tid == 0, a.stamps, tile, 14, ((unsigned long long)__builtin_amdgcn_s_getreg((4 << 0) | (0 << 6) | (31 << 11)) << 32) |
                                                      __builtin_amdgcn_s_getreg((20 << 0) | (0 << 6) | (31 << 11)));
#ifndef AFT_CHAIN_PFS
#define AFT_CHAIN_PFS 4
#endif
    constexpr int PFD = AFT_CHAIN_PFS, PFF = (AFT_CHAIN_PFS + 1) / 2, PFQ = (AFT_CHAIN_PFS + 2) / 3;
    WRing<1, PFD> ring_d;
    WRing<2, PFF> ring_ff;
    WRing<3, PFQ> ring_qkv;
    f32x16 cur;
    f32x16 acc[3];
    auto in_projection = [&]() {
        const float bias_v = __builtin_bit_cast(float, __builtin_amdgcn_raw_buffer_load_b32(srd_bv, (unsigned)(fb + r) * 4, 0, 0));
        float *xq = xb;
        if constexpr (!MLP) xq = (round & 1) ? hb : xb;
        if constexpr (BS) {
            bs_publish(xq, w, lane, cur);
        } else {
#pragma unroll
            for (int s = 0; s < 4; ++s)
                *reinterpret_cast<f32x4 *>(xq + (w * 4 + s) * 256 + lane * 4) = f32x4{cur[4 * s], cur[4 * s + 1], cur[4 * s + 2], cur[4 * s + 3]};
        }
        __syncthreads();
        AFT_STAMP(tid == 0, a.stamps, tile, 9);
        f32x16 vinit;
#pragma unroll
        for (int e = 0; e < 16; ++e) vinit[e] = bias_v;
        acc[2] = vinit;
        if constexpr (BS) {
            acc[0] = bias_acc(make_srd(a.bv - 2 * D), fb, h);
            auto xq_bs = [&](int kb, int m) { return bs_fetch(xq, kb, m, lane); };
            gemm_run_bs<W, 3, PFQ, W, 0x4, decltype(xq_bs), 0x2>(ring_qkv, srd_wq, wq_lane, acc, xq_bs);
        } else {
            auto xq_frag = [&](int kb, int s) { return *reinterpret_cast<const f32x4 *>(xq + (kb * 4 + s) * 256 + lane * 4); };
            gemm_run<W, 3, PFQ, W, 0x4, decltype(xq_frag), 0x3>(ring_qkv, srd_wq, wq_lane, acc, xq_frag);
        }
    };
    if constexpr (MLP) {
        f32x16 acc_o[1] = {bias_acc(srd_bo, fb, h)};
        gemm_preload<W, 1, PFD, 1>(ring_d, srd_wo, wo_lane);
        if constexpr (PT) {
            request_x_pt(tile, valid_pt);
        } else {
            request_attn(tile, AHEAD ? PFK : 0, W);
            if (!AHEAD) request_x(tile);
        }
        AFT_STAMP(tid == 0, a.stamps, tile, 1);
        if constexpr (BS)
            gemm_run_bs<W, 1, PFD, 1, 0>(ring_d, srd_wo, wo_lane, acc_o, [&](int kb, int m) { return bs_split(of[kb][2 * m], of[kb][2 * m + 1]); });
        else if constexpr (PT)
            gemm_run<W, 1, PFD, 1, 0>(ring_d, srd_wo, wo_lane, acc_o, [&](int kb, int s) {
                return *reinterpret_cast<const f32x4 *>(hb + S::XB + (kb * 4 + s) * 256 + lane * 4);
            });
        else
            gemm_run<W, 1, PFD, 1, 0>(ring_d, srd_wo, wo_lane, acc_o, [&](int kb, int s) { return of[kb][s]; });
        f32x16 acc_h[2] = {bias_acc(srd_b1, 2 * fb, h), bias_acc(srd_b1, 2 * fb + 32, h)};
        gemm_preload<W, 2, PFF, 1>(ring_ff, srd_w1, w1_lane);
#pragma unroll
        for (int s = 0; s < 4; ++s)
#pragma unroll
            for (int j = 0; j < 4; ++j) cur[4 * s + j] = acc_o[0][4 * s + j] + xres[s][j];
        AFT_STAMP(tid == 0, a.stamps, tile, 2);
        layernorm_rows<D>(cur, stats, par + fb, par + D + fb, w, r, h);
        AFT_STAMP(tid == 0, a.stamps, tile, 3);
        if constexpr (BS) {
            bs_publish(xb, w, lane, cur);
        } else {
#pragma unroll
            for (int s = 0; s < 4; ++s)
                *reinterpret_cast<f32x4 *>(xb + (w * 4 + s) * 256 + lane * 4) = f32x4{cur[4 * s], cur[4 * s + 1], cur[4 * s + 2], cur[4 * s + 3]};
        }
        __syncthreads();
        AFT_STAMP(tid == 0, a.stamps, tile, 4);
        if constexpr (BS)
            gemm_run_bs<W, 2, PFF, 1, 0>(ring_ff, srd_w1, w1_lane, acc_h, [&](int kb, int m) { return bs_fetch(xb, kb, m, lane); });
        else
            gemm_run<W, 2, PFF, 1, 0>(ring_ff, srd_w1, w1_lane, acc_h, [&](int kb, int s) {
                return *reinterpret_cast<const f32x4 *>(xb + (kb * 4 + s) * 256 + lane * 4);
            });
        f32x16 acc_d[1] = {bias_acc(srd_b2, fb, h)};
        gemm_preload<2 * W, 1, PFD, 1>(ring_d, srd_w2, w2_lane);
        AFT_STAMP(tid == 0, a.stamps, tile, 5);
#pragma unroll
        for (int t = 0; t < 2; ++t) {
            f32x16 hid;
#pragma unroll
            for (int s = 0; s < 4; ++s) {
                const f32x2 g0 = activate2<ACT>(f32x2{acc_h[t][4 * s], acc_h[t][4 * s + 1]});
                const f32x2 g1 = activate2<ACT>(f32x2{acc_h[t][4 * s + 2], acc_h[t][4 * s + 3]});
                if constexpr (BS) {
                    hid[4 * s] = g0[0]; hid[4 * s + 1] = g0[1]; hid[4 * s + 2] = g1[0]; hid[4 * s + 3] = g1[1];
                } else {
                    *reinterpret_cast<f32x4 *>(hb + ((2 * w + t) * 4 + s) * 256 + lane * 4) = f32x4{g0[0], g0[1], g1[0], g1[1]};
                }
            }
            if constexpr (BS) bs_publish(hb, 2 * w + t, lane, hid);
        }
        __syncthreads();
        AFT_STAMP(tid == 0, a.stamps, tile, 6);
        if constexpr (BS)
            gemm_run_bs<2 * W, 1, PFD, 1, 0>(ring_d, srd_w2, w2_lane, acc_d, [&](int kb, int m) { return bs_fetch(hb, kb, m, lane); });
        else
            gemm_run<2 * W, 1, PFD, 1, 0>(ring_d, srd_w2, w2_lane, acc_d, [&](int kb, int s) {
                return *reinterpret_cast<const f32x4 *>(hb + (kb * 4 + s) * 256 + lane * 4);
            });
        if constexpr (QKV) gemm_preload<W, 3, PFQ, W>(ring_qkv, srd_wq, wq_lane);
#pragma unroll
        for (int e = 0; e < 16; ++e) cur[e] += acc_d[0][e];
        AFT_STAMP(tid == 0, a.stamps, tile, 7);
        layernorm_rows<D>(cur, stats, par + 2 * D + fb, par + 3 * D + fb, w, r, h);
        AFT_STAMP(tid == 0, a.stamps, tile, 8);
        if constexpr (!QKV) {
            if (AHEAD && tile + tile_stride < ntiles) request_tile(tile + tile_stride);
        }
        bool store_x = true;
        if constexpr (!QKV) {
            if (a.out6 != nullptr) {
                store_x = false;
                const int P = a.out6_features;
                f32x16 acc6 = f32x16{0};
#pragma unroll
                for (int s = 0; s < 4; ++s) {
                    f32x4 wv = {0.f, 0.f, 0.f, 0.f};
                    if (r < P) wv = *reinterpret_cast<const f32x4 *>(a.lin2_w + (size_t)r * D + fb + 8 * s + 4 * h);
#pragma unroll
                    for (int j = 0; j < 4; ++j) acc6 = __builtin_amdgcn_mfma_f32_32x32x2f32(wv[j], cur[4 * s + j], acc6, 0, 0, 0);
                }
                float *part = hb + (w * 64 + lane) * 8;
                *reinterpret_cast<f32x4 *>(part) = f32x4{acc6[0], acc6[1], acc6[2], acc6[3]};
                *reinterpret_cast<f32x4 *>(part + 4) = f32x4{acc6[4], acc6[5], acc6[6], acc6[7]};
                pending_row0 = PT ? plane_pt * a.tokens + qt_pt * 32 : row0;
                pending_valid = valid_pt;
            }
        }
        if (store_x && row_ok) {
            if (blocked) {
                const unsigned xblk = ((unsigned)row0 * D + w * 1024 + lane * 4) * 4;
#pragma unroll
                for (int s = 0; s < 4; ++s)
                    srd_store(srd_x, xblk + 1024 * s, f32x4{cur[4 * s], cur[4 * s + 1], cur[4 * s + 2], cur[4 * s + 3]});
            } else {
#pragma unroll
                for (int s = 0; s < 4; ++s)
                    srd_store(srd_x, xrow + 32 * s, f32x4{cur[4 * s], cur[4 * s + 1], cur[4 * s + 2], cur[4 * s + 3]});
            }
        }
    } else {
        auto embed_x0 = [&]() {
            f32x16 acc0 = emb_acc0;
            float av[kEmbSteps];
#pragma unroll
            for (int st = 0; st < kEmbSteps; ++st) {
                const int k = 2 * st + h;
                av[st] = k < a.emb_K ? emb_w[(fb + r) * a.emb_K + k] : 0.f;
            }
#pragma unroll
            for (int st = 0; st < kEmbSteps; ++st)
                if (2 * st < a.emb_K) acc0 = __builtin_amdgcn_mfma_f32_32x32x2f32(av[st], emb_bv[st], acc0, 0, 0, 0);
            return acc0;
        };
        auto store_x0 = [&](const f32x16 &v) {
            if (row_ok) {
                if (blocked) {
                    const unsigned xblk = ((unsigned)row0 * D + w * 1024 + lane * 4) * 4;
#pragma unroll
                    for (int s = 0; s < 4; ++s)
                        srd_store(srd_x, xblk + 1024 * s, f32x4{v[4 * s], v[4 * s + 1], v[4 * s + 2], v[4 * s + 3]});
                } else {
#pragma unroll
                    for (int s = 0; s < 4; ++s)
                        srd_store(srd_x, xrow + 32 * s, f32x4{v[4 * s], v[4 * s + 1], v[4 * s + 2], v[4 * s + 3]});
                }
            }
        };
        if (fold) {
          if constexpr (!BS) {
            gemm_preload<W, 1, PFD, 1>(ring_d, srd_wq, wq_lane);
            const f32x16 x0 = embed_x0();
            const unsigned tok_k = PT ? (unsigned)min(qt_pt * 32 + r, a.tokens - 1) : (unsigned)grow % (unsigned)a.tokens;
#pragma unroll
            for (int s = 0; s < 4; ++s) {
                const f32x4 t = srd_load(srd_tk, (tok_k * D + fb + 8 * s + 4 * h) * 4);
#pragma unroll
                for (int j = 0; j < 4; ++j) acc[1][4 * s + j] = t[j];
            }
            const unsigned vrow = (unsigned)(fb + r) * (unsigned)a.tokpad;
#pragma unroll
            for (int g = 0; g < 4; ++g) {
                if constexpr (PT) {
                    const f32x4 t = srd_load(srd_tvt, (vrow + qt_pt * 32 + 8 * g + 4 * h) * 4);
#pragma unroll
                    for (int j = 0; j < 4; ++j) acc[2][4 * g + j] = t[j];
                } else {
                    unsigned t = (unsigned)(row0 + 8 * g + 4 * h) % (unsigned)a.tokens;
#pragma unroll
                    for (int j = 0; j < 4; ++j) {
                        acc[2][4 * g + j] = __builtin_bit_cast(float, __builtin_amdgcn_raw_buffer_load_b32(srd_tvt, (vrow + t) * 4, 0, 0));
                        if (++t >= (unsigned)a.tokens) t = 0;
                    }
                }
            }
            float fold_wk[kEmbSteps], fold_wv[kEmbSteps];
            auto frag = [&](int st) {
                const unsigned fo = ((unsigned)(w * kEmbSteps + st) * 64 + lane + lo) * 4;
                fold_wk[st] = __builtin_bit_cast(float, __builtin_amdgcn_raw_buffer_load_b32(srd_fw, fo, 0, 0));
                fold_wv[st] = __builtin_bit_cast(float, __builtin_amdgcn_raw_buffer_load_b32(srd_fw, fo + W * kEmbSteps * 64 * 4, 0, 0));
            };
            const bool more_steps = a.emb_K > 2 * kFoldSteps0;
#pragma unroll
            for (int st = 0; st < kEmbSteps; ++st) fold_wk[st] = fold_wv[st] = 0.f;
#pragma unroll
            for (int st = 0; st < kFoldSteps0; ++st) frag(st);
            if (more_steps) {
#pragma unroll
                for (int st = kFoldSteps0; st < kEmbSteps; ++st) frag(st);
            }
            store_x0(x0);
            float *xq = (round & 1) ? hb : xb;
#pragma unroll
            for (int s = 0; s < 4; ++s)
                *reinterpret_cast<f32x4 *>(xq + (w * 4 + s) * 256 + lane * 4) = f32x4{x0[4 * s], x0[4 * s + 1], x0[4 * s + 2], x0[4 * s + 3]};
            auto kv_step = [&](int st) {
                acc[1] = __builtin_amdgcn_mfma_f32_32x32x2f32(fold_wk[st], emb_bv[st], acc[1], 0, 0, 0);
                acc[2] = __builtin_amdgcn_mfma_f32_32x32x2f32(emb_bv[st], fold_wv[st], acc[2], 0, 0, 0);
            };
#pragma unroll
            for (int st = 0; st < kFoldSteps0; ++st) kv_step(st);
            if (more_steps) {
#pragma unroll
                for (int st = kFoldSteps0; st < kEmbSteps; ++st) kv_step(st);
            }
            __syncthreads();
            AFT_STAMP(tid == 0, a.stamps, tile, 9);
            f32x16 acc_q[1];
            auto xq_frag = [&](int kb, int s) { return *reinterpret_cast<const f32x4 *>(xq + (kb * 4 + s) * 256 + lane * 4); };
            gemm_run<W, 1, PFD, 1, 0, decltype(xq_frag), 0x1>(ring_d, srd_wq, wq_lane, acc_q, xq_frag);
            acc[0] = acc_q[0];
          }
        } else {
            gemm_preload<W, 3, PFQ, W>(ring_qkv, srd_wq, wq_lane);
            if (a.emb_conv == nullptr) {
                if (!AHEAD) request_x(tile);
#pragma unroll
                for (int s = 0; s < 4; ++s)
#pragma unroll
                    for (int j = 0; j < 4; ++j) cur[4 * s + j] = xres[s][j];
            } else {
                cur = embed_x0();
                store_x0(cur);
            }
            if constexpr (QKV) in_projection();
        }
    }

    if constexpr (QKV) {
      if constexpr (MLP) in_projection();
        AFT_STAMP(tid == 0, a.stamps, tile, 10);
        if (AHEAD && tile + tile_stride < ntiles) request_tile(tile + tile_stride);
        if constexpr (!MLP) {
            if (a.emb_conv != nullptr && tile + tile_stride < tile_end) emb_request(tile + tile_stride);
        }
        if constexpr (PT) {
            const unsigned ph_base = (unsigned)(plane_pt * a.heads + w) * ((unsigned)a.tokpad * kHeadDim) + (unsigned)qt_pt * 1024;
            if (row_ok) {
#pragma unroll
                for (int s = 0; s < 4; ++s) {
                    srd_store(srd_q, (ph_base + lane * 4 + s * 256) * 4, f32x4{acc[0][4 * s], acc[0][4 * s + 1], acc[0][4 * s + 2], acc[0][4 * s + 3]});
                    srd_store(srd_k, (ph_base + lane * 4 + s * 256) * 4, f32x4{acc[1][4 * s], acc[1][4 * s + 1], acc[1][4 * s + 2], acc[1][4 * s + 3]});
                }
            }
#pragma unroll
            for (int gq = 0; gq < 4; ++gq) {
                const int tok = qt_pt * 32 + 8 * gq + 4 * h;
                const f32x4 v = {acc[2][4 * gq], acc[2][4 * gq + 1], acc[2][4 * gq + 2], acc[2][4 * gq + 3]};
                if (tok + 3 < a.tokens) {
                    srd_store(srd_vt, (ph_base + gq * 256 + lane * 4) * 4, v);
                } else {
#pragma unroll
                    for (int j = 0; j < 4; ++j)
                        if (tok + j < a.tokens) {
                            const float vj = acc[2][4 * gq + j];
                            __builtin_amdgcn_raw_buffer_store_b32(__builtin_bit_cast(unsigned, vj), srd_vt, (ph_base + gq * 256 + lane * 4 + j) * 4, 0, 0);
                        }
                }
            }
        } else {
        const int plane0 = row0 / a.tokens, tok0 = row0 - plane0 * a.tokens;
        const unsigned head_stride = (unsigned)a.tokpad * kHeadDim;
        auto wrap_plane = [&](int &tok, unsigned &ph) {
            if (tok >= a.tokens) { tok -= a.tokens; ph += a.heads; }
            if (a.tokens < kTile)
                while (tok >= a.tokens) { tok -= a.tokens; ph += a.heads; }
        };
        const unsigned ph0 = (unsigned)(plane0 * a.heads + w);
        const bool full = row0 + 32 <= a.rows;
        if constexpr (BS) {
            const float qscale = 1.4426950408889634f * 0.17677669529663687f;
#pragma unroll
            for (int e = 0; e < 16; ++e) acc[0][e] *= qscale;
            {
                int tok = tok0 + r;
                unsigned ph = ph0;
                wrap_plane(tok, ph);
                const unsigned lane_off = (ph * head_stride + (unsigned)(tok >> 5) * 1024 + ((tok & 31) + 32 * h) * 4) * 4;
                if (full || row_ok) {
#pragma unroll
                    for (int t = 0; t < 2; ++t)
#pragma unroll
                        for (int m = 0; m < 2; ++m) {
                            const BsFrag f = bs_split(f32x4{acc[t][8 * m], acc[t][8 * m + 1], acc[t][8 * m + 2], acc[t][8 * m + 3]},
                                                      f32x4{acc[t][8 * m + 4], acc[t][8 * m + 5], acc[t][8 * m + 6], acc[t][8 * m + 7]});
                            srd_store(t == 0 ? srd_q : srd_k, lane_off + (2 * m) * 1024, f.hi);
                            srd_store(t == 0 ? srd_q : srd_k, lane_off + (2 * m + 1) * 1024, f.lo);
                        }
                }
            }
            __bf16 *vt16 = reinterpret_cast<__bf16 *>(a.vt);
#pragma unroll
            for (int gq = 0; gq < 4; ++gq) {
                int tok = tok0 + 8 * gq + 4 * h;
                unsigned ph = ph0;
                wrap_plane(tok, ph);
                __bf16 vh[4], vl[4];
#pragma unroll
                for (int j = 0; j < 4; ++j) {
                    vh[j] = (__bf16)acc[2][4 * gq + j];
                    vl[j] = (__bf16)(acc[2][4 * gq + j] - (float)vh[j]);
                }
                const bool in_rows = full || row0 + 8 * gq + 4 * h + 3 < a.rows;
                if ((tok & 3) == 0 && tok + 3 < a.tokens && in_rows) {
                    const unsigned g = (tok >> 3) & 3, hh = (tok >> 2) & 1;
                    const size_t e16 = ((size_t)ph * head_stride + (size_t)(tok >> 5) * 1024 + (2 * (g >> 1)) * 256 + (r + 32 * hh) * 4) * 2 + 4 * (g & 1);
                    using bf16x4 = __attribute__((__vector_size__(4 * sizeof(__bf16)))) __bf16;
                    *reinterpret_cast<bf16x4 *>(vt16 + e16) = bf16x4{vh[0], vh[1], vh[2], vh[3]};
                    *reinterpret_cast<bf16x4 *>(vt16 + e16 + 512) = bf16x4{vl[0], vl[1], vl[2], vl[3]};
                } else {
#pragma unroll
                    for (int j = 0; j < 4; ++j) {
                        int tj = tok + j;
                        unsigned pj = ph;
                        wrap_plane(tj, pj);
                        if (row0 + 8 * gq + 4 * h + j < a.rows) {
                            const unsigned g = (tj >> 3) & 3, hh = (tj >> 2) & 1;
                            const size_t e16 = ((size_t)pj * head_stride + (size_t)(tj >> 5) * 1024 + (2 * (g >> 1)) * 256 + (r + 32 * hh) * 4) * 2 +
                                               4 * (g & 1) + (tj & 3);
                            vt16[e16] = vh[j];
                            vt16[e16 + 512] = vl[j];
                        }
                    }
                }
// ... 71 lines not shown
```

### adafortitran_amd/csrc/k_chain.hip

```cpp
#include <algorithm>
#include <cstdlib>

#include "chain_device.h"
#include "pack_device.h"

#ifndef AFT_CHAIN_MANY_MAX_D
#define AFT_CHAIN_MANY_MAX_D 96
#endif

namespace aft {

template <int D, int ACT, bool MLP, bool QKV>
__global__ __launch_bounds__(D * 2, D <= 128 ? 3 : 2) void chain_kernel(const ChainArgs a) {
    extern __shared__ __attribute__((aligned(16))) float smem[];
    chain_body<D, ACT, MLP, QKV>(a, smem, threadIdx.x, blockIdx.x, gridDim.x, (a.rows + 31) / 32);
}


template <int D, int ACT, bool MLP, bool QKV>
__global__ __launch_bounds__(D * 2, D <= 128 ? 3 : 2) void chain_split_kernel(const ChainArgs a) {
    extern __shared__ __attribute__((aligned(16))) float smem[];
    chain_body<D, ACT, MLP, QKV, true>(a, smem, threadIdx.x, blockIdx.x, gridDim.x, (a.rows + 31) / 32);
}

// ... 11 lines not shown
template <int D, int ACT>
static hipError_t launch_chain_split_t(const ChainArgs &args, bool mlp, bool qkv, hipStream_t st) {
    if (mlp && qkv) return launch_chain_split_v<D, ACT, true, true>(args, st);
    if (mlp) return launch_chain_split_v<D, ACT, true, false>(args, st);
    return launch_chain_split_v<D, ACT, false, true>(args, st);
}

template <int D, int ACT, bool MLP, bool QKV>
static hipError_t launch_chain_v(const ChainArgs &args, hipStream_t st) {
    using S = ChainShape<D>;
    static PerDeviceOnce lds_attr;
    hipError_t ea = ensure_dynamic_lds(lds_attr, reinterpret_cast<const void *>(chain_kernel<D, ACT, MLP, QKV>), S::LDS_BYTES);
    if (ea != hipSuccess) return ea;
    constexpr int kGranules = (int)((S::LDS_BYTES + 1279) / 1280);
    constexpr int kPerCu = D <= AFT_CHAIN_MANY_MAX_D ? std::min(12 / S::WAVES, 128 / kGranules) : (D <= 128 ? 3 : 1);
    const int resident = current_device_cus() * kPerCu;
    const int blocks = std::min((args.rows + 31) / 32, resident);
    const size_t lds = S::LDS_BYTES;
#ifdef AFT_DIAG_STAMPS
    StampRun run(SW_STAMPS, MLP && QKV ? kStampChainMlpQkv : MLP ? kStampChainMlp : kStampChainQkv, (args.rows + 31) / 32, st);
    ChainArgs stamped = args;
    stamped.stamps = run.buffer();
    const ChainArgs &a = stamped;
#else
    const ChainArgs &a = args;
#endif
    hipLaunchKernelGGL((chain_kernel<D, ACT, MLP, QKV>), dim3(blocks), dim3(S::THREADS), lds, st, a);
    const hipError_t e = hipGetLastError();
#ifdef AFT_DIAG_STAMPS
    if (const unsigned long long *h = run.collect()) {
        int per_cu = 0;
        (void)hipOccupancyMaxActiveBlocksPerMultiprocessor(&per_cu, chain_kernel<D, ACT, MLP, QKV>, S::THREADS, lds);
        report_chain(stdout, h, (args.rows + 31) / 32, blocks, D, (int)MLP, (int)QKV, per_cu, lds);
    }
#endif
    return e;
}

size_t packed_layer_floats(int d) { return (size_t)8 * d * d; }

__global__ __launch_bounds__(256) void pack_weights_kernel(const WeightsDev w, float *__restrict__ packed, int d,
                                                           int num_layers, int split) {
    pack_weights_vec(w, packed, d, 0, num_layers, split, (size_t)blockIdx.x * 256 + threadIdx.x);
}

hipError_t launch_pack_weights(const aft_config &c, const aft_layer_weights *layers, float *packed, int count, hipStream_t st) {
    for (int first = 0; first < count; first += kLayerWindow) {
        const int n = std::min(kLayerWindow, count - first);
        WeightsDev win{};
        for (int i = 0; i < n; ++i) win.layers[i] = layers[first + i];
        const size_t vecs = packed_layer_floats(c.model_dim) * n / 4;
        hipLaunchKernelGGL(pack_weights_kernel, dim3((unsigned)((vecs + 255) / 256)), dim3(256), 0, st, win,
                           packed + packed_layer_floats(c.model_dim) * first, c.model_dim, n, c.precision == AFT_PRECISION_BF16X3 ? 1 : 0);
        hipError_t e = hipGetLastError();
        if (e != hipSuccess) return e;
    }
    return hipSuccess;
}

template <int D, int ACT>
static hipError_t launch_chain_t(const ChainArgs &args, bool mlp, bool qkv, hipStream_t st) {
    if (mlp && qkv) return launch_chain_v<D, ACT, true, true>(args, st);
    if (mlp) return launch_chain_v<D, ACT, true, false>(args, st);
    return launch_chain_v<D, ACT, false, true>(args, st);
}

ChainArgs make_chain_args(const aft_config &c, const aft_layer_weights *m, const float *m_packed, const aft_layer_weights *qw,
                          const float *q_packed, const float *attn, float *x, float *q, float *k, float *vt, int rows, int tokens,
                          int tokpad, const ChainFusion *fuse) {
    const size_t dd = (size_t)c.model_dim * c.model_dim;
    ChainArgs a{};
    if (fuse != nullptr && fuse->out6 != nullptr && m != nullptr && qw == nullptr) {
        a.lin2_w = fuse->lin2_w; a.lin2_b = fuse->lin2_b; a.out6 = fuse->out6;
        a.out6_features = c.patch_scs * c.patch_symbols;
        a.out6_stride = out6_stride(c);
    }
    if (fuse != nullptr && fuse->conv_enhanced != nullptr && m == nullptr) {
        a.emb_conv = fuse->conv_enhanced; a.emb_tok6 = fuse->tokens6; a.emb_w1 = fuse->lin1_w; a.emb_b1 = fuse->lin1_b;
        a.emb_pos = fuse->pos;
        a.emb_S = c.num_scs; a.emb_T = c.num_symbols; a.emb_p0 = c.patch_scs; a.emb_p1 = c.patch_symbols;
        a.emb_K = c.patch_scs * c.patch_symbols + (fuse->tokens6 ? 6 : 0);
        if (fuse->fold_tk != nullptr && c.precision == AFT_PRECISION_F32) {
            a.fold_tk = fuse->fold_tk; a.fold_tvt = fuse->fold_tvt; a.fold_w = fuse->fold_w;
        }
    }
    a.attn = attn;
    a.x = x;
    a.x_blocked = fuse != nullptr && fuse->x_blocked ? 1 : 0;
    if (m != nullptr) {
        a.wo = m_packed + 3 * dd; a.bo = m->out_proj_b;
        a.w1 = m_packed + 4 * dd; a.b1 = m->lin1_b;
        a.w2 = m_packed + 6 * dd; a.b2 = m->lin2_b;
        a.g1 = m->norm1_w; a.be1 = m->norm1_b;
        a.g2 = m->norm2_w; a.be2 = m->norm2_b;
    }
    if (qw != nullptr) {
        a.wqkv = q_packed;
        a.bv = qw->in_proj_b + 2 * c.model_dim;
    }
    a.q = q; a.k = k; a.vt = vt;
    a.rows = rows; a.tokens = tokens; a.tokpad = tokpad;
    a.heads = c.model_dim / kHeadDim;
    return a;
}

hipError_t launch_chain(const aft_config &c, const aft_layer_weights *m, const float *m_packed,
                        const aft_layer_weights *qw, const float *q_packed,
                        const float *attn, float *x, float *q, float *k, float *vt, int rows, int tokens,
                        int tokpad, hipStream_t st, const ChainFusion *fuse) {
    const ChainArgs a = make_chain_args(c, m, m_packed, qw, q_packed, attn, x, q, k, vt, rows, tokens, tokpad, fuse);
    const bool gelu = c.activation == AFT_ACT_GELU;
    const bool mlp = m != nullptr, qkv = qw != nullptr;
    if (c.precision == AFT_PRECISION_BF16X3) {
        if (c.model_dim == 128)
            return gelu ? launch_chain_split_t<128, AFT_ACT_GELU>(a, mlp, qkv, st) : launch_chain_split_t<128, AFT_ACT_RELU>(a, mlp, qkv, st);
        if (c.model_dim == 256)
            return gelu ? launch_chain_split_t<256, AFT_ACT_GELU>(a, mlp, qkv, st) : launch_chain_split_t<256, AFT_ACT_RELU>(a, mlp, qkv, st);
        return hipErrorInvalidValue;
    }
#define AFT_CHAIN_DIM(DD) \
    if (c.model_dim == DD) return gelu ? launch_chain_t<DD, AFT_ACT_GELU>(a, mlp, qkv, st) : launch_chain_t<DD, AFT_ACT_RELU>(a, mlp, qkv, st);
    AFT_CHAIN_DIM(32) AFT_CHAIN_DIM(96) AFT_CHAIN_DIM(160) AFT_CHAIN_DIM(224)
#undef AFT_CHAIN_DIM
    if (c.model_dim == 64)
        return gelu ? launch_chain_t<64, AFT_ACT_GELU>(a, mlp, qkv, st) : launch_chain_t<64, AFT_ACT_RELU>(a, mlp, qkv, st);
    if (c.model_dim == 192)
        return gelu ? launch_chain_t<192, AFT_ACT_GELU>(a, mlp, qkv, st) : launch_chain_t<192, AFT_ACT_RELU>(a, mlp, qkv, st);
    if (c.model_dim == 128)
        return gelu ? launch_chain_t<128, AFT_ACT_GELU>(a, mlp, qkv, st) : launch_chain_t<128, AFT_ACT_RELU>(a, mlp, qkv, st);
    if (c.model_dim == 256)
        return gelu ? launch_chain_t<256, AFT_ACT_GELU>(a, mlp, qkv, st) : launch_chain_t<256, AFT_ACT_RELU>(a, mlp, qkv, st);
    return hipErrorInvalidValue;
}

}
```

### adafortitran_amd/csrc/k_layer.hip

```cpp
#include <algorithm>

#include "attn_device.h"
#include "chain_device.h"

namespace aft {

struct LayerArgs {
    ChainArgs c;
    const float *aq, *ak, *avt, *qbias;
    float scale_log2e;
    int planes;
};

template <int D, int TOK>
struct LayerAttention {
    const LayerArgs &a;
    float *sink;
    __device__ __forceinline__ void operator()(int tile) const {
        const int w = __builtin_amdgcn_readfirstlane(threadIdx.x >> 6);
        const int plane = tile / a.c.tpp, qt = tile - plane * a.c.tpp;
        const int task = (plane * (D / kHeadDim) + w) * a.c.tpp + qt;
        attn_body<false, kHeadDim, TOK, true>(a.aq, a.ak, a.avt, a.qbias, nullptr, D / kHeadDim, a.c.tokens, a.c.tokpad, D, a.scale_log2e, task,
                                              1 << 30, task + 1, nullptr, -1, sink + w * 1024);
        __syncthreads();
    }
};

template <int D, int ACT, bool QKV, int TOK>
__global__ __launch_bounds__(D * 2, 3) void layer_kernel(const LayerArgs a) {
    extern __shared__ __attribute__((aligned(16))) float smem[];
    using S = ChainShape<D>;
    int vblock = blockIdx.x;
    if ((gridDim.x & 7) == 0) vblock = (blockIdx.x & 7) * (gridDim.x >> 3) + (blockIdx.x >> 3);
    chain_body<D, ACT, true, QKV, false, true>(a.c, smem, threadIdx.x, vblock, gridDim.x, a.planes * a.c.tpp,
                                               LayerAttention<D, TOK>{a, smem + S::XB + S::XB});
}

template <int D>
__global__ __launch_bounds__(D * 2, 3) void chain_plane_tiles_kernel(const ChainArgs a, int planes) {
    extern __shared__ __attribute__((aligned(16))) float smem[];
    int vblock = blockIdx.x;
    if ((gridDim.x & 7) == 0) vblock = (blockIdx.x & 7) * (gridDim.x >> 3) + (blockIdx.x >> 3);
    chain_body<D, AFT_ACT_RELU, false, true, false, true>(a, smem, threadIdx.x, vblock, gridDim.x, planes * a.tpp);
}

template <class K, class A, class... Rest>
static hipError_t launch_plane_tiles(K kernel, const A &args, int planes, int tpp, hipStream_t st, PerDeviceOnce &lds_attr, Rest... rest) {
    using S = ChainShape<128>;
    hipError_t ea = ensure_dynamic_lds(lds_attr, reinterpret_cast<const void *>(kernel), S::LDS_BYTES);
    if (ea != hipSuccess) return ea;
    const int blocks = std::min(planes * tpp, current_device_cus() * 3);
    hipLaunchKernelGGL(kernel, dim3(blocks), dim3(S::THREADS), S::LDS_BYTES, st, args, rest...);
    return hipGetLastError();
}

bool layer_fused_ok(const aft_config &c) {
    return packed_engine_ok(c) && c.precision == AFT_PRECISION_F32 && c.model_dim == 128 && c.num_head * kHeadDim == c.model_dim &&
           tokens_of(c) >= kTile;
}

hipError_t launch_chain_plane_tiles(const aft_config &c, const aft_layer_weights *qw, const float *q_packed, float *x, float *q, float *k,
                                    float *vt, int planes, int tokens, int tokpad, hipStream_t st, const ChainFusion *fuse) {
    if (!layer_fused_ok(c) || fuse == nullptr || fuse->conv_enhanced == nullptr) return hipErrorInvalidValue;
    ChainArgs a = make_chain_args(c, nullptr, nullptr, qw, q_packed, nullptr, x, q, k, vt, planes * tokens, tokens, tokpad, fuse);
    a.tpp = tokpad / kTile;
    static PerDeviceOnce once;
    return launch_plane_tiles(chain_plane_tiles_kernel<128>, a, planes, a.tpp, st, once, planes);
}

template <int ACT, bool QKV, int TOK>
static hipError_t launch_layer_v(const LayerArgs &a, hipStream_t st) {
    static PerDeviceOnce once;
    return launch_plane_tiles(layer_kernel<128, ACT, QKV, TOK>, a, a.planes, a.c.tpp, st, once);
}
template <int ACT, bool QKV>
static hipError_t launch_layer_t(const LayerArgs &a, hipStream_t st) {
    return a.c.tokens == 280 ? launch_layer_v<ACT, QKV, 280>(a, st) : launch_layer_v<ACT, QKV, 0>(a, st);
}

hipError_t launch_layer(const aft_config &c, const aft_layer_weights *m, const float *m_packed, const aft_layer_weights *qw,
                        const float *q_packed, float *x, float *q, const float *k_in, const float *vt_in, float *k_out, float *vt_out,
                        int planes, int tokens, int tokpad, hipStream_t st, const ChainFusion *fuse) {
    if (!layer_fused_ok(c) || m == nullptr || k_in == k_out || vt_in == vt_out) return hipErrorInvalidValue;
    LayerArgs a{};
    a.c = make_chain_args(c, m, m_packed, qw, q_packed, nullptr, x, q, k_out, vt_out, planes * tokens, tokens, tokpad, fuse);
    a.c.tpp = tokpad / kTile;
    a.aq = q; a.ak = k_in; a.avt = vt_in;
    a.qbias = m->in_proj_b;
    a.scale_log2e = 1.4426950408889634f / sqrtf((float)kHeadDim);
    a.planes = planes;
    const bool gelu = c.activation == AFT_ACT_GELU;
    if (qw != nullptr) return gelu ? launch_layer_t<AFT_ACT_GELU, true>(a, st) : launch_layer_t<AFT_ACT_RELU, true>(a, st);
    return gelu ? launch_layer_t<AFT_ACT_GELU, false>(a, st) : launch_layer_t<AFT_ACT_RELU, false>(a, st);
}

}
```

### adafortitran_amd/csrc/k_misc.hip

```cpp
#include <algorithm>

#include "aft_internal.h"
#include "conv_device.h"
#include "pack_device.h"

namespace aft {

struct AdapterArgs {
    const float *cond[3];
    const float *w[3][3], *b[3][3];
    float *tokens6;
    int h0, h1, h2, tokens;
};

__device__ __forceinline__ void adapter_body(const AdapterArgs &a, int b, int e, float *sm) {
    float *a0 = sm, *a1 = sm + a.h0;
    const int tid = threadIdx.x;
    const float x = a.cond[e][b];
    constexpr int kH0Max = 8, kPer2 = 3;
    const bool fast = a.h0 <= kH0Max && a.h1 == 42 && a.h2 <= kPer2 * 256 && a.h1 <= 256;
    if (fast) {
        float w0 = 0.f, b0 = 0.f, w1[kH0Max], b1 = 0.f, b2[kPer2];
        f32x2 w2[kPer2][21];
        if (tid < a.h0) { w0 = a.w[e][0][tid]; b0 = a.b[e][0][tid]; }
#pragma unroll
        for (int k = 0; k < kH0Max; ++k) w1[k] = (tid < a.h1 && k < a.h0) ? a.w[e][1][tid * a.h0 + k] : 0.f;
        if (tid < a.h1) b1 = a.b[e][1][tid];
#pragma unroll
        for (int u = 0; u < kPer2; ++u) {
            const int i = tid + 256 * u;
            const bool ok = i < a.h2;
            const float *wr = a.w[e][2] + (size_t)(ok ? i : 0) * 42;
#pragma unroll
            for (int k = 0; k < 21; ++k) w2[u][k] = *reinterpret_cast<const f32x2 *>(wr + 2 * k);
            b2[u] = ok ? a.b[e][2][i] : 0.f;
        }
        if (tid < a.h0) a0[tid] = fmaxf(fmaf(w0, x, b0), 0.f);
        __syncthreads();
        if (tid < a.h1) {
            float acc = b1;
#pragma unroll
            for (int k = 0; k < kH0Max; ++k)
                if (k < a.h0) acc = fmaf(w1[k], a0[k], acc);
            a1[tid] = fmaxf(acc, 0.f);
        }
        __syncthreads();
#pragma unroll
        for (int u = 0; u < kPer2; ++u) {
            const int i = tid + 256 * u;
            if (i >= a.h2) break;
            float acc = b2[u];
#pragma unroll
            for (int k = 0; k < 21; ++k) {
                acc = fmaf(w2[u][k][0], a1[2 * k], acc);
                acc = fmaf(w2[u][k][1], a1[2 * k + 1], acc);
            }
            a.tokens6[((size_t)b * a.tokens + (i >> 1)) * 6 + 2 * e + (i & 1)] = acc;
        }
        return;
    }
    for (int i = tid; i < a.h0; i += 256) a0[i] = fmaxf(fmaf(a.w[e][0][i], x, a.b[e][0][i]), 0.f);
    __syncthreads();
    for (int i = tid; i < a.h1; i += 256) {
        float acc = a.b[e][1][i];
        for (int k = 0; k < a.h0; ++k) acc = fmaf(a.w[e][1][i * a.h0 + k], a0[k], acc);
        a1[i] = fmaxf(acc, 0.f);
    }
    __syncthreads();
    for (int i = tid; i < a.h2; i += 256) {
        float acc = a.b[e][2][i];
        const float *wr = a.w[e][2] + (size_t)i * a.h1;
        for (int k = 0; k < a.h1; ++k) acc = fmaf(wr[k], a1[k], acc);
        a.tokens6[((size_t)b * a.tokens + (i >> 1)) * 6 + 2 * e + (i & 1)] = acc;
    }
}

__global__ __launch_bounds__(256) void adapter_kernel(const AdapterArgs a) {
    extern __shared__ float sm[];
    adapter_body(a, blockIdx.x, blockIdx.y, sm);
}

static AdapterArgs adapter_args(const aft_config &c, const WeightsDev &w, const float *snr, const float *ds,
                                const float *dop, float *tokens6) {
    AdapterArgs a{};
    a.cond[0] = snr; a.cond[1] = ds; a.cond[2] = dop;
    for (int e = 0; e < 3; ++e)
        for (int j = 0; j < 3; ++j) { a.w[e][j] = w.ada_w[e][j]; a.b[e][j] = w.ada_b[e][j]; }
    a.tokens6 = tokens6;
    a.h0 = c.hidden[0]; a.h1 = c.hidden[1]; a.h2 = c.hidden[2];
    a.tokens = (c.num_scs / c.patch_scs) * (c.num_symbols / c.patch_symbols);
    return a;
}

hipError_t launch_adapter(const aft_config &c, const WeightsDev &w, const float *snr, const float *ds,
                          const float *dop, float *tokens6, int batch, hipStream_t st) {
    const AdapterArgs a = adapter_args(c, w, snr, ds, dop, tokens6);
    hipLaunchKernelGGL(adapter_kernel, dim3(batch, 3), dim3(256), sizeof(float) * (a.h0 + a.h1), st, a);
    return hipGetLastError();
}


constexpr int kFoldTok = 2, kFoldChunk = 16;
struct FoldArgs {
    const float *wkv, *bv;
    const float *w1, *b1, *pos;
    float *tk, *tvt, *wf;
    int d, K, tokens, tokpad;
};
inline size_t fold_tables_lds(int d) { return sizeof(float) * ((size_t)256 * (kFoldChunk + 1) + (size_t)kFoldTok * d); }

__device__ __forceinline__ void fold_tables_body(const FoldArgs &f, int blk, float *sm) {
    float *sw = sm, *sc = sm + 256 * (kFoldChunk + 1);
    const int tid = threadIdx.x, chunks = (2 * f.d + 255) / 256;
    const int t0 = (blk / chunks) * kFoldTok, row0 = (blk % chunks) * 256, row = row0 + tid;
    for (int i = tid; i < kFoldTok * f.d; i += 256) {
        const int tt = i / f.d, k = i - tt * f.d, t = t0 + tt;
        sc[i] = t < f.tokens ? f.b1[k] + f.pos[(size_t)t * f.d + k] : 0.f;
    }
    float acc[kFoldTok];
#pragma unroll
    for (int tt = 0; tt < kFoldTok; ++tt) acc[tt] = row >= f.d && row < 2 * f.d ? f.bv[row - f.d] : 0.f;
    constexpr int kPieces = kFoldChunk / 4;
    f32x4 piece[kPieces];
    auto request = [&](int kc) {
#pragma unroll
        for (int m = 0; m < kPieces; ++m) {
            const int i = tid + 256 * m, rr = i / kPieces, c4 = (i % kPieces) * 4;
            piece[m] = f32x4{0.f, 0.f, 0.f, 0.f};
            if (row0 + rr < 2 * f.d) piece[m] = *reinterpret_cast<const f32x4 *>(f.wkv + (size_t)(row0 + rr) * f.d + kc + c4);
        }
    };
    request(0);
    for (int kc = 0; kc < f.d; kc += kFoldChunk) {
        __syncthreads();
#pragma unroll
        for (int m = 0; m < kPieces; ++m) {
            const int i = tid + 256 * m, rr = i / kPieces, c4 = (i % kPieces) * 4;
#pragma unroll
            for (int j = 0; j < 4; ++j) sw[rr * (kFoldChunk + 1) + c4 + j] = piece[m][j];
        }
        if (kc + kFoldChunk < f.d) request(kc + kFoldChunk);
        __syncthreads();
#pragma unroll
        for (int kk = 0; kk < kFoldChunk; ++kk) {
            const float wv = sw[tid * (kFoldChunk + 1) + kk];
#pragma unroll
            for (int tt = 0; tt < kFoldTok; ++tt) acc[tt] = fmaf(wv, sc[tt * f.d + kc + kk], acc[tt]);
        }
    }
#pragma unroll
    for (int tt = 0; tt < kFoldTok; ++tt) {
        const int t = t0 + tt;
        if (row < f.d) {
            if (t < f.tokens) f.tk[(size_t)t * f.d + row] = acc[tt];
        } else if (row < 2 * f.d && t < f.tokpad) {
            f.tvt[(size_t)(row - f.d) * f.tokpad + t] = t < f.tokens ? acc[tt] : 0.f;
        }
    }
}

__device__ __forceinline__ void fold_matrices_body(const FoldArgs &f, int blk) {
    const int o = blk * 256 + threadIdx.x, per_part = (f.d / 32) * kFoldSteps * 64;
    if (o >= 2 * per_part) return;
    const int part = o / per_part, rem = o - part * per_part;
    const int wblock = rem / (kFoldSteps * 64), st = rem / 64 % kFoldSteps, lane = rem & 63;
    const int row = part * f.d + 32 * wblock + (lane & 31), k = 2 * st + (lane >> 5);
    float acc = 0.f;
    if (k < f.K) {
        const float *wr = f.wkv + (size_t)row * f.d;
        for (int j = 0; j < f.d; j += 4) {
            const f32x4 wv = *reinterpret_cast<const f32x4 *>(wr + j);
#pragma unroll
            for (int jj = 0; jj < 4; ++jj) acc = fmaf(wv[jj], f.w1[(size_t)(j + jj) * f.K + k], acc);
        }
    }
    f.wf[o] = acc;
}

struct PrologueArgs {
    AdapterArgs ad;
    float *packed;
    const float *pilots;
    float *up_planes;
    int adapter_blocks, pack_blocks, d, num_layers, split;
    int up_bx, npix, pf, nplanes;
    float *conv_frag;
    int frag_blocks;
    FoldArgs fold;
    int fold_table_blocks, fold_matrix_blocks;
};

__global__ __launch_bounds__(256) void prologue_kernel(const WeightsDev w, const PrologueArgs a) {
    extern __shared__ __attribute__((aligned(16))) float sm[];
    int blk = blockIdx.x;
    if (blk < a.adapter_blocks) {
        adapter_body(a.ad, blk / 3, blk % 3, sm);
        return;
    }
    blk -= a.adapter_blocks;
    if (blk < a.fold_table_blocks) {
        fold_tables_body(a.fold, blk, sm);
        return;
    }
    blk -= a.fold_table_blocks;
    if (blk < a.fold_matrix_blocks) {
        fold_matrices_body(a.fold, blk);
        return;
    }
    blk -= a.fold_matrix_blocks;
    if (blk < a.pack_blocks) {
        const size_t v = (size_t)blk * 256 + threadIdx.x, dd4 = (size_t)a.d * a.d / 4;
        if (a.fold_table_blocks > 0 && v >= dd4 && v < 3 * dd4) return;
        pack_weights_vec(w, a.packed, a.d, 0, a.num_layers, a.split, v);
        return;
    }
    blk -= a.pack_blocks;
    if (blk < a.frag_blocks) {
        const int v = blk * 256 + threadIdx.x;
        constexpr int kPerStack = kFragFloats / 4;
        if (v < 2 * kPerStack) {
            const int stack = v / kPerStack, rem = v - stack * kPerStack;
            const float *const *cw = stack ? w.ref_w : w.enh_w;
            const float *const *cb = stack ? w.ref_b : w.enh_b;
            f32x4 o;
            if (rem < kFragQuads * 64) {
                const int quad = rem >> 6, lane = rem & 63;
#pragma unroll
                for (int jj = 0; jj < 4; ++jj) o[jj] = conv_frag16_entry(cw[1], cb[1], cw[2], cb[2], 4 * quad + jj, lane);
            } else {
                const int i0 = 4 * (rem - kFragQuads * 64), h = i0 / 80;
#pragma unroll
                for (int jj = 0; jj < 4; ++jj) o[jj] = conv_helper_entry(cw[0], cb[0], cw[3], cb[3], h, i0 - 80 * h + jj);
            }
            *reinterpret_cast<f32x4 *>(a.conv_frag + (size_t)v * 4) = o;
        }
        return;
    }
    blk -= a.frag_blocks;
    upsample_planes_body(sm, w.up_w, w.up_b, a.pilots, a.up_planes, a.npix, a.pf, a.nplanes, blk % a.up_bx, blk / a.up_bx);
}

bool prologue_upsample_ok(const aft_config &c, const WeightsDev &w) {
    return upsample_planes_ok(w.up_w, c.pilot_scs * c.pilot_symbols);
}

hipError_t launch_prologue(const aft_config &c, const WeightsDev &w, const float *snr, const float *ds, const float *dop,
                           float *tokens6, int batch, float *packed, const float *pilots, float *up_planes, hipStream_t st,
                           float *conv_frag, const L0Fold *fold) {
    PrologueArgs a{};
    if (conv_frag != nullptr) {
        a.conv_frag = conv_frag;
        a.frag_blocks = (2 * (kFragFloats / 4) + 255) / 256;
    }
    size_t lds = 0;
    if (c.adaptive) {
        a.ad = adapter_args(c, w, snr, ds, dop, tokens6);
        a.adapter_blocks = 3 * batch;
        lds = sizeof(float) * (a.ad.h0 + a.ad.h1);
    }
    if (packed != nullptr) {
        a.packed = packed; a.d = c.model_dim; a.num_layers = std::min(c.num_layers, kLayerWindow);
        a.split = c.precision == AFT_PRECISION_BF16X3 ? 1 : 0;
        a.pack_blocks = (int)((packed_layer_floats(c.model_dim) * a.num_layers / 4 + 255) / 256);
    }
    int up_blocks = 0;
    if (up_planes != nullptr && prologue_upsample_ok(c, w)) {
        a.pilots = pilots; a.up_planes = up_planes;
        a.npix = c.num_scs * c.num_symbols; a.pf = c.pilot_scs * c.pilot_symbols; a.nplanes = 2 * batch;
        a.up_bx = (a.npix + kUpPix - 1) / kUpPix;
        up_blocks = a.up_bx * ((a.nplanes + kUpPlanes - 1) / kUpPlanes);
        lds = std::max(lds, upsample_planes_lds(a.pf));
    }
    if (fold != nullptr && fold->tk != nullptr) {
        FoldArgs &f = a.fold;
        f.d = c.model_dim; f.K = c.patch_scs * c.patch_symbols + (c.adaptive ? 6 : 0);
        f.tokens = tokens_of(c); f.tokpad = round_up(f.tokens, kTile);
        f.wkv = w.layers[0].in_proj_w + (size_t)f.d * f.d; f.bv = w.layers[0].in_proj_b + 2 * f.d;
        f.w1 = w.lin1_w; f.b1 = w.lin1_b; f.pos = w.pos;
        f.tk = fold->tk; f.tvt = fold->tvt; f.wf = fold->wf;
        a.d = c.model_dim;
        a.fold_table_blocks = (f.tokpad + kFoldTok - 1) / kFoldTok * ((2 * f.d + 255) / 256);
        a.fold_matrix_blocks = (2 * (f.d / 32) * kFoldSteps * 64 + 255) / 256;
        lds = std::max(lds, fold_tables_lds(f.d));
    }
    const int blocks = a.adapter_blocks + a.fold_table_blocks + a.fold_matrix_blocks + a.pack_blocks + a.frag_blocks + up_blocks;
    if (blocks == 0) return hipSuccess;
    hipLaunchKernelGGL(prologue_kernel, dim3(blocks), dim3(256), lds, st, w, a);
    return hipGetLastError();
}

struct EmbedArgs {
    const float *conv_enhanced, *tokens6, *w1, *b1, *pos;
    float *x;
    int S, T, p0, p1, tokens, d, din, planes;
};

template <int D, bool ADAPTIVE, int PMAX>
__global__ __launch_bounds__(256) void embed_kernel(const EmbedArgs a) {
    constexpr int PER = D / 32, NF = ADAPTIVE ? PMAX + 6 : PMAX;
    const int tid = threadIdx.x, hw = tid >> 5, lane32 = tid & 31;
    const int tw = a.T / a.p1, p = a.p0 * a.p1;
    extern __shared__ float sm[];
    for (int i = tid; i < a.din * D; i += 256) sm[(i % a.din) * D + i / a.din] = a.w1[i];
    __syncthreads();
    float w[NF][PER], b1[PER];
#pragma unroll
    for (int f = 0; f < NF; ++f) {
        const int frow = f < PMAX ? f : p + (f - PMAX);
#pragma unroll
        for (int i = 0; i < PER; ++i) w[f][i] = (f < PMAX && f >= p) ? 0.f : sm[frow * D + lane32 * PER + i];
    }
#pragma unroll
    for (int i = 0; i < PER; ++i) b1[i] = a.b1[lane32 * PER + i];
    const unsigned rows = (unsigned)a.planes * a.tokens, rstep = gridDim.x * 8u, tokens = a.tokens;
    const unsigned dn = rstep / tokens, dt = rstep % tokens;
    int poff[PMAX];
#pragma unroll
    for (int f = 0; f < PMAX; ++f) poff[f] = (f / a.p1) * a.T + f % a.p1;
    struct Tok { unsigned row, n, t; };
    auto advance = [&](Tok k) {
        k.row += rstep; k.n += dn; k.t += dt;
        if (k.t >= tokens) { k.t -= tokens; ++k.n; }
        return k;
    };
    auto fetch = [&](const Tok &k, float (&vin)[NF], float (&ps)[PER]) {
        const unsigned tq = k.t / (unsigned)tw, tr = k.t - tq * tw;
        const float *ce = a.conv_enhanced + ((size_t)k.n * a.S + tq * a.p0) * a.T + tr * a.p1;
#pragma unroll
        for (int f = 0; f < PMAX; ++f) vin[f] = f < p ? ce[poff[f]] : 0.f;
        if constexpr (ADAPTIVE) {
            const float *tk = a.tokens6 + ((size_t)(k.n >> 1) * tokens + k.t) * 6;
#pragma unroll
            for (int f = 0; f < 6; ++f) vin[PMAX + f] = tk[f];
        }
#pragma unroll
        for (int i = 0; i < PER; ++i) ps[i] = a.pos[k.t * D + lane32 * PER + i];
    };
    auto emit = [&](const Tok &k, const float (&vin)[NF], const float (&ps)[PER]) {
        float acc[PER];
#pragma unroll
        for (int i = 0; i < PER; ++i) acc[i] = b1[i] + ps[i];
#pragma unroll
        for (int f = 0; f < NF; ++f)
#pragma unroll
            for (int i = 0; i < PER; ++i) acc[i] = fmaf(w[f][i], vin[f], acc[i]);
#pragma unroll
        for (int i = 0; i < PER; ++i) a.x[(size_t)k.row * D + lane32 * PER + i] = acc[i];
    };
    float va[NF], pa[PER], vb[NF], pb[PER];
    Tok k0;
    k0.row = blockIdx.x * 8u + hw;
    k0.n = k0.row / tokens;
    k0.t = k0.row - k0.n * tokens;
    if (k0.row < rows) fetch(k0, va, pa);
    while (k0.row < rows) {
        const Tok k1 = advance(k0), k2 = advance(k1);
        if (k1.row < rows) fetch(k1, vb, pb);
        emit(k0, va, pa);
        if (k1.row < rows) {
            if (k2.row < rows) fetch(k2, va, pa);
            emit(k1, vb, pb);
        }
        k0 = k2;
    }
}
// ... 327 lines not shown
```

### adafortitran_amd/csrc/switches.h

```cpp
#pragma once

#define AFT_SWITCHES(X) \
    X(LANES, "AFT_LANES", "1 = never split a forward into lanes; 2 .. 4 = always that many shares (header section \"Lanes\")") \
    X(L0_FOLD, "AFT_L0_FOLD", "0 = layer 0's keys and values by the model_dim-deep product over x0, not from the input features on the prologue's tables (DESIGN.md 4.1)") \
    X(LAYER_FUSED, "AFT_LAYER_FUSED", "0 = never the one-launch-per-layer sequence (k_layer.hip), 1 = wherever its shape is covered (default: where plane-aligned tiles add no round)") \
    X(PROLOGUE_NO_UP, "AFT_PROLOGUE_NO_UP", "measurement: the profiled prologue launch without the pilot upsampler product") \
    X(CONV_NSPLIT, "AFT_CONV_NSPLIT", "1 | 2 | 4 column ranges per plane in the streaming conv kernels (default: by the batch)") \
    X(CONV_BANDED, "AFT_CONV_BANDED", "the banded conv kernel instead of the column- / row-streaming ones") \
    X(CONV_COLUMN_TILES, "AFT_CONV_COLUMN_TILES", "the column-tiled conv path even where a band plan fits; n > 2 = at least n tiles per plane") \
    X(GEMM_BM, "AFT_GEMM_BM", "64 | 96: row tile of the training GEMM (default: by the shape)") \
    X(EMBED_ANY_OLD, "AFT_EMBED_ANY_OLD", "the general engine's own embedding kernel instead of the training path's") \
    X(EMBED_BWD_GENERIC, "AFT_EMBED_BWD_GENERIC", "the vector embedding backward instead of the MFMA one (model_dim 128)") \
    X(TRAIN_UNFUSED_FWD, "AFT_TRAIN_UNFUSED_FWD", "the launch sequence the fused forward chain of a training layer replaced") \
    X(TRAIN_UNFUSED_BWD, "AFT_TRAIN_UNFUSED_BWD", "the launch sequence the fused backward chain of a training layer replaced") \
    X(TRAIN_ATTN_BWD_SPLIT, "AFT_TRAIN_ATTN_BWD_SPLIT", "the two-pass attention backward instead of the one-pass kernel") \
    X(ATTN_BWD_GROUPS, "AFT_ATTN_BWD_GROUPS", "1 | 4 problems per workgroup of the one-pass attention backward (default: by shape)") \
    X(STAMPS, "AFT_STAMPS", "phase stamps printed on the host: the diag variant only (libaft_hip_diag.so, build.build_diag(): -DAFT_DIAG_STAMPS)") \
    X(ALLOW_COMPOSITE, "AFT_ALLOW_COMPOSITE", "1 = run a configuration the kernels do not cover on the PyTorch-ROCm composite") \
    X(TRAIN_NO_FUSED_ENDS, "AFT_TRAIN_NO_FUSED_ENDS", "training: PyTorch's unfold / cat / add around the dense ends, not fused") \
    X(TRAIN_NO_QKV_CHAIN, "AFT_TRAIN_NO_QKV_CHAIN", "training: every layer runs its own in-projection GEMM (no chained tapes)") \
    X(PRECISION, "AFT_PRECISION", "f32 | bf16x3: the estimators' default hip_precision") \
    X(ENCODER_PATH, "AFT_ENCODER_PATH", "auto | launches | plane: aft_config.encoder_path of every HipEngine (`plane`: retired, runs the launches)")

namespace aft {

enum Switch : int {
#define AFT_SWITCH_ID(id, name, purpose) SW_##id,
    AFT_SWITCHES(AFT_SWITCH_ID)
#undef AFT_SWITCH_ID
    kNumSwitches
};

bool switch_on(Switch s);
int switch_int(Switch s, int dflt);

}
```

### include/adafortitran_amd.h

```cpp
#ifndef ADAFORTITRAN_AMD_H
#define ADAFORTITRAN_AMD_H

#include <stddef.h>
#include <stdint.h>

#ifdef __cplusplus
extern "C" {
#endif

#define AFT_ABI_VERSION 10

#define AFT_OK 0
#define AFT_ERR_ARG 1
#define AFT_ERR_SHAPE 2
#define AFT_ERR_HIP 3

#define AFT_ENCODER_AUTO 0
#define AFT_ENCODER_LAUNCHES 1
#define AFT_ENCODER_PLANE 2

#define AFT_PRECISION_F32 0
#define AFT_PRECISION_BF16X3 1

#define AFT_ACT_RELU 0
#define AFT_ACT_GELU 1

typedef struct aft_config {
    int32_t num_scs, num_symbols;
    int32_t pilot_scs, pilot_symbols;
    int32_t patch_scs, patch_symbols;
    int32_t num_layers, model_dim, num_head;
    int32_t activation;
    int32_t adaptive;
    int32_t hidden[3];
    int32_t encoder_path;
    int32_t precision;
} aft_config;

typedef struct aft_layer_weights {
    const float *in_proj_w, *in_proj_b;
    const float *out_proj_w, *out_proj_b;
    const float *lin1_w, *lin1_b;
    const float *lin2_w, *lin2_b;
    const float *norm1_w, *norm1_b, *norm2_w, *norm2_b;
} aft_layer_weights;

typedef struct aft_weights {
    const float *up_w, *up_b;
    const float *enh_w[4], *enh_b[4];
    const float *ref_w[4], *ref_b[4];
    const float *ada_w[3][3], *ada_b[3][3];
    const float *lin1_w, *lin1_b;
    const float *pos;
    const float *lin2_w, *lin2_b;
    const aft_layer_weights *layers;
} aft_weights;

int aft_version(void);
const char *aft_last_error(void);

int aft_check_config(const aft_config *cfg);

#define AFT_ENGINE_PACKED 0
#define AFT_ENGINE_GENERAL 1
int aft_engine_of(const aft_config *cfg);

int aft_set_switch(const char *name, const char *value);
int aft_get_switch(const char *name, char *buf, size_t n);

int aft_max_batch(const aft_config *cfg);

size_t aft_workspace_bytes(const aft_config *cfg, int batch);

size_t aft_workspace_bytes_layer_fused(const aft_config *cfg, int batch);
int aft_layer_fused_of(const aft_config *cfg, int batch);

#define AFT_MAX_LANES 4
int aft_workspace_lanes(const aft_config *cfg, int batch, int *lanes, int *frames, size_t *offset_bytes);

#define AFT_REGION_CONV_ENHANCED 0
#define AFT_REGION_TOKENS6 1
#define AFT_REGION_ENC_OUT 2
int aft_workspace_region(const aft_config *cfg, int batch, int region, size_t *offset_bytes, size_t *size_bytes);

int aft_forward_f32(const aft_config *cfg, const aft_weights *w, const float *pilots,
                    const float *snr, const float *ds, const float *dop, float *out,
                    void *workspace, size_t workspace_bytes, int batch, void *stream);

size_t aft_packed_weights_bytes(const aft_config *cfg);
int aft_pack_weights_f32(const aft_config *cfg, const aft_weights *w, void *packed, size_t packed_bytes, void *stream);
int aft_forward_prepacked_f32(const aft_config *cfg, const aft_weights *w, const void *packed, const float *pilots,
                              const float *snr, const float *ds, const float *dop, float *out, void *workspace,
                              size_t workspace_bytes, int batch, void *stream);

int aft_linear_forward_f32(const float *weight, const float *bias, const float *pilots,
                           float *out, int batch, int in_features, int out_features,
                           void *stream);

int aft_mse_partial_f32(const float *est, const float *ref, double *sum_sq,
                        long long n_complex, void *stream);


int aft_pilot_gather_f32(const float *hzero_ls, float *pilots, int *counts, int batch, int grid_elems,
                         int expected, void *stream);

int aft_ls_mse_db_f32(const float *ls, const float *ideal, float *db, int batch, int grid_elems, void *stream);

int aft_frame_gather_f32(const float *ideal_all, const float *pilots_all, const long long *index, float *ideal_out,
                         float *pilots_out, int *flags, int batch, long long frames, int grid_elems, int pilot_elems, void *stream);

#define AFT_CHANSIM_MAX_TAPS 32
#define AFT_CHANSIM_MAX_RAYS 16
#define AFT_CHANSIM_MAX_VALUES 16
#define AFT_CHANSIM_MAX_PILOT_SCS 64
#define AFT_CHANSIM_MAX_PILOT_SYMBOLS 16
typedef struct aft_chansim {
    int32_t num_scs, num_symbols;
    int32_t pilot_scs, pilot_symbols;
    int32_t taps, rays;
    int32_t n_snr, n_ds, n_dop;
    int32_t reserved;
    double subcarrier_spacing_hz, symbol_period_s;
    float tap_delay[AFT_CHANSIM_MAX_TAPS];
    float tap_amp[AFT_CHANSIM_MAX_TAPS];
    float snr_db[AFT_CHANSIM_MAX_VALUES], noise_sigma[AFT_CHANSIM_MAX_VALUES];
    float delay_spread_ns[AFT_CHANSIM_MAX_VALUES], doppler_hz[AFT_CHANSIM_MAX_VALUES];
    int32_t pilot_sc_index[AFT_CHANSIM_MAX_PILOT_SCS], pilot_symbol_index[AFT_CHANSIM_MAX_PILOT_SYMBOLS];
} aft_chansim;

int aft_channel_sim_f32(const aft_chansim *sim, unsigned long long seed, long long base, long long start, long long stride,
                        long long modulo, int batch, float *ideal, float *pilots, float *meta, void *stream);

#define AFT_CHANSIM_MAX_GROUP 16
int aft_channel_sim_group_f32(const aft_chansim *sim, int rx, int tx, const float *mix, unsigned long long seed, long long base,
                              long long start, long long stride, long long modulo, int batch, float *ideal, float *pilots,
                              float *meta, void *stream);

typedef struct aft_lmmse {
    int32_t num_scs, num_symbols;
    int32_t pilot_scs, pilot_symbols;
    int32_t n_snr, n_ds, n_dop;
    int32_t fixed_snr, fixed_ds, fixed_dop;
    float snr_db[AFT_CHANSIM_MAX_VALUES], delay_spread_ns[AFT_CHANSIM_MAX_VALUES], doppler_hz[AFT_CHANSIM_MAX_VALUES];
    float noise_var[AFT_CHANSIM_MAX_VALUES];
} aft_lmmse;

size_t aft_lmmse_table_floats(const aft_lmmse *plan);

int aft_lmmse_f32(const aft_lmmse *plan, const float *tables, const float *pilots, const float *snr, const float *ds,
                  const float *dop, float *est, int batch, void *stream);

typedef struct aft_link {
    int32_t num_scs, num_symbols;
    int32_t pilot_scs, pilot_symbols;
    int32_t bits_per_symbol, reserved;
    int32_t pilot_sc_index[AFT_CHANSIM_MAX_PILOT_SCS], pilot_symbol_index[AFT_CHANSIM_MAX_PILOT_SYMBOLS];
} aft_link;

// ... 173 lines not shown
```

Before: 85950 frames/s.

## Fold layer-0 queries into prologue tables and rebuild them inside the layer-0 launch

Extends the layer-0 fold so the queries, as well as the keys and values, are computed from the raw input features through precomputed per-token tables and folded weight matrices. Layer 0's fused launch regathers the embedding inputs, forms Q in registers with a short MFMA product, and passes it straight into attention. A lighter fold kernel produces only K and V. This drops the separate model_dim-deep QKV chain launch for layer 0 and the write and reread of Q. In exchange the prologue does more folding work, and the layer kernel and attention body gain new template variants that use more registers.

```diff
diff --git a/adafortitran_amd/_abi.py b/adafortitran_amd/_abi.py
--- a/adafortitran_amd/_abi.py
+++ b/adafortitran_amd/_abi.py
@@ -182,6 +182,7 @@
     "aft_workspace_bytes": (C.c_size_t, [cfgp, C.c_int]),
     "aft_workspace_bytes_layer_fused": (C.c_size_t, [cfgp, C.c_int]),
     "aft_layer_fused_of": (C.c_int, [cfgp, C.c_int]),
+    "aft_l0_fold_of": (C.c_int, [cfgp]),
     "aft_workspace_lanes": (C.c_int, [cfgp, C.c_int, C.POINTER(C.c_int), C.POINTER(C.c_int), C.POINTER(C.c_size_t)]),
     "aft_workspace_region": (C.c_int, [cfgp, C.c_int, C.c_int, C.POINTER(C.c_size_t), C.POINTER(C.c_size_t)]),
     "aft_forward_f32": (C.c_int, [cfgp, wp, vp, vp, vp, vp, vp, vp, C.c_size_t, C.c_int, vp]),
diff --git a/adafortitran_amd/csrc/aft_api.hip b/adafortitran_amd/csrc/aft_api.hip
--- a/adafortitran_amd/csrc/aft_api.hip
+++ b/adafortitran_amd/csrc/aft_api.hip
@@ -358,12 +358,18 @@
         if (&en.ls == ls) { --en.in_use; return; }
 }
 
-static bool l0_fold_selected(const aft_config &c) {
-    return packed_engine_ok(c) && c.precision == AFT_PRECISION_F32 && switch_int(SW_L0_FOLD, 1) != 0;
-}
-static L0Fold l0_fold_at(const aft_config &c, const Workspace &ws, float *base) {
+static int l0_fold_selected(const aft_config &c) {
+    if (!packed_engine_ok(c) || c.precision != AFT_PRECISION_F32) return 0;
+    const int want = switch_int(SW_L0_FOLD, 2);
+    if (want == 0) return 0;
+    const size_t d = (size_t)c.model_dim;
+    const bool home = 3 * fold_matrix_floats(c.model_dim) + (size_t)tokens_of(c) * d <= 3 * d * d;
+    return want == 2 && home ? 2 : 1;
+}
+static L0Fold l0_fold_at(const aft_config &c, const Workspace &ws, float *base, int level) {
     float *tables = base + ws.attn;
-    return L0Fold{tables, tables + (size_t)ws.tokpad * c.model_dim, base + ws.wpack + (size_t)c.model_dim * c.model_dim};
+    const size_t dd = (size_t)c.model_dim * c.model_dim;
+    return L0Fold{tables, tables + (size_t)ws.tokpad * c.model_dim, base + ws.wpack + (level == 2 ? 0 : dd), level == 2};
 }
 
 enum ChainPos { kChainFirst, kChainMiddle, kChainLast };
@@ -392,14 +398,22 @@
     ChainFusion first = chain_fusion_for(kChainFirst, c, w, ws, base);
     const ChainFusion middle = chain_fusion_for(kChainMiddle, c, w, ws, base), last = chain_fusion_for(kChainLast, c, w, ws, base);
     if (fused && fold != nullptr && first_layer == 0) {
-        first.fold_tk = fold->tk; first.fold_tvt = fold->tvt; first.fold_w = fold->wf;
+        first.fold_tk = fold->tk; first.fold_tvt = fold->tvt; first.fold_w = fold->wf; first.fold_q = fold->q;
     }
     if (fused && x_pt != nullptr && x == base + ws.x && first_layer == 0 && last_layer == c.num_layers - 1 &&
         layer_fused_selected(c, ws.planes / 2)) {
         x = x_pt;
         float *kbuf[2] = {k, attn}, *vbuf[2] = {vt, vt2};
-        STEP("chain(qkv, plane tiles)", launch_chain_plane_tiles(c, &layers[0], wp, x, q, kbuf[0], vbuf[0], ws.planes, ws.tokens, ws.tokpad, st, &first));
-        for (int l = 0; l <= last_layer; ++l) {
+        const bool self0 = first.fold_q;
+        if (self0) {
+            STEP("fold(k, v; plane tiles)", launch_fold_kv_plane_tiles(c, &layers[0], kbuf[0], vbuf[0], ws.planes, ws.tokens, ws.tokpad, st, &first));
+            const bool more = last_layer > 0;
+            STEP("layer 0", launch_layer(c, &layers[0], wp, more ? &layers[1] : nullptr, more ? wp + pl : nullptr, x, q, kbuf[0], vbuf[0],
+                                         kbuf[1], vbuf[1], ws.planes, ws.tokens, ws.tokpad, st, more ? &middle : &last, &first));
+        } else {
+            STEP("chain(qkv, plane tiles)", launch_chain_plane_tiles(c, &layers[0], wp, x, q, kbuf[0], vbuf[0], ws.planes, ws.tokens, ws.tokpad, st, &first));
+        }
+        for (int l = self0 ? 1 : 0; l <= last_layer; ++l) {
             const bool more = l < last_layer;
             STEP("layer", launch_layer(c, &layers[l], wp + l * pl, more ? &layers[l + 1] : nullptr, more ? wp + (l + 1) * pl : nullptr, x, q,
                                        kbuf[l & 1], vbuf[l & 1], kbuf[(l + 1) & 1], vbuf[(l + 1) & 1], ws.planes, ws.tokens, ws.tokpad, st,
@@ -520,6 +534,11 @@
     return workspace_floats_any_lanes(*cfg, batch, true) * sizeof(float);
 }
 
+int aft_l0_fold_of(const aft_config *cfg) {
+    if (check_config(cfg) != AFT_OK) return -1;
+    return l0_fold_selected(*cfg);
+}
+
 int aft_layer_fused_of(const aft_config *cfg, int batch) {
     if (check_config(cfg) != AFT_OK || batch <= 0) return -1;
     return layer_fused_selected(*cfg, batch) ? 1 : 0;
@@ -550,8 +569,9 @@
     float *wpack = prepacked != nullptr || general ? nullptr : base + ws.wpack;
     float *lent = x_holds_planes(*cfg, ws) ? base + ws.x : nullptr;
     float *up_planes = prologue_upsample_ok(*cfg, wd) ? lent : nullptr;
-    const bool fold_on = l0_fold_selected(*cfg);
-    const L0Fold fold = fold_on ? l0_fold_at(*cfg, ws, base) : L0Fold{};
+    const int fold_level = l0_fold_selected(*cfg);
+    const bool fold_on = fold_level != 0;
+    const L0Fold fold = fold_on ? l0_fold_at(*cfg, ws, base, fold_level) : L0Fold{};
     STEP("prologue(adapter + pack_weights + upsampler product)",
          launch_prologue(*cfg, wd, snr, ds, dop, base + ws.tokens6, batch, wpack, pilots, up_planes, st, base + ws.convfrag,
                          fold_on ? &fold : nullptr));
@@ -805,8 +825,8 @@
     const float *wp = base + ws.wpack;
     ChainFusion first = chain_fusion_for(kChainFirst, *cfg, wd, ws, base);
     const ChainFusion middle = chain_fusion_for(kChainMiddle, *cfg, wd, ws, base), last = chain_fusion_for(kChainLast, *cfg, wd, ws, base);
-    const bool fold_on = l0_fold_selected(*cfg);
-    const L0Fold fold = fold_on ? l0_fold_at(*cfg, ws, base) : L0Fold{};
+    const bool fold_on = l0_fold_selected(*cfg) != 0;
+    const L0Fold fold = fold_on ? l0_fold_at(*cfg, ws, base, 1) : L0Fold{};
     if (fold_on) { first.fold_tk = fold.tk; first.fold_tvt = fold.tvt; first.fold_w = fold.wf; }
     hipError_t e = hipSuccess;
     for (int i = 0; i < reps && e == hipSuccess; ++i) {
diff --git a/adafortitran_amd/csrc/aft_internal.h b/adafortitran_amd/csrc/aft_internal.h
--- a/adafortitran_amd/csrc/aft_internal.h
+++ b/adafortitran_amd/csrc/aft_internal.h
@@ -215,7 +215,9 @@
 constexpr int kFoldSteps = (kMaxPatchFeatures + 6 + 1) / 2;
 struct L0Fold {
     float *tk, *tvt, *wf;
-};
+    bool q = false;
+};
+inline size_t fold_matrix_floats(int d) { return (size_t)(d / 32) * kFoldSteps * 64; }
 hipError_t launch_prologue(const aft_config &c, const WeightsDev &w, const float *snr, const float *ds, const float *dop,
                            float *tokens6, int batch, float *packed, const float *pilots, float *up_planes, hipStream_t st,
                            float *conv_frag = nullptr, const L0Fold *fold = nullptr);
@@ -229,6 +231,7 @@
     const float *lin2_w = nullptr, *lin2_b = nullptr;
     float *out6 = nullptr;
     const float *fold_tk = nullptr, *fold_tvt = nullptr, *fold_w = nullptr;
+    bool fold_q = false;
     bool x_blocked = false;
 };
 inline int out6_stride(const aft_config &c) { return round_up(c.patch_scs * c.patch_symbols, 8); }
@@ -242,7 +245,9 @@
                                     float *k, float *vt, int planes, int tokens, int tokpad, hipStream_t st, const ChainFusion *fuse);
 hipError_t launch_layer(const aft_config &c, const aft_layer_weights *mlp_w, const float *mlp_packed, const aft_layer_weights *qkv_w,
                         const float *qkv_packed, float *x, float *q, const float *k_in, const float *vt_in, float *k_out, float *vt_out,
-                        int planes, int tokens, int tokpad, hipStream_t st, const ChainFusion *fuse);
+                        int planes, int tokens, int tokpad, hipStream_t st, const ChainFusion *fuse, const ChainFusion *self = nullptr);
+hipError_t launch_fold_kv_plane_tiles(const aft_config &c, const aft_layer_weights *qkv_w, float *k, float *vt, int planes, int tokens,
+                                      int tokpad, hipStream_t st, const ChainFusion *fuse);
 hipError_t launch_pack_weights(const aft_config &c, const aft_layer_weights *layers, float *packed, int count, hipStream_t st);
 hipError_t launch_attention(const aft_config &c, const float *q, const float *k, const float *vt, const float *qbias,
                             float *attn, int planes, int tokens, int tokpad, hipStream_t st);
diff --git a/adafortitran_amd/csrc/attn_device.h b/adafortitran_amd/csrc/attn_device.h
--- a/adafortitran_amd/csrc/attn_device.h
+++ b/adafortitran_amd/csrc/attn_device.h
@@ -72,13 +72,16 @@
 }
 __device__ __forceinline__ float round_to_bf16(float x) { return (float)(__bf16)x; }
 
-template <bool BS = false, int HD = 32, int TOK = 0, bool SINK = false>
+struct AttnLoadQ {};
+template <bool BS = false, int HD = 32, int TOK = 0, bool SINK = false, class QSrc = AttnLoadQ>
 __device__ __forceinline__ void attn_body(const float *__restrict__ q, const float *__restrict__ k,
                                           const float *__restrict__ vt, const float *__restrict__ qbias,
                                           float *__restrict__ out, int nblk, int tokens_rt, int tokpad_rt, int model_dim,
                                           float scale_log2e, const int first_task, const int total_waves, int ntasks,
-                                          unsigned long long *stamps, const int tail_task = -1, float *sink = nullptr) {
+                                          unsigned long long *stamps, const int tail_task = -1, float *sink = nullptr, QSrc qsrc = QSrc{}) {
     static_assert(!SINK || (!BS && HD == 32), "the LDS sink is instantiated for the fp32 head-dimension-32 body");
+    constexpr bool QREG = !std::is_same<QSrc, AttnLoadQ>::value;
+    static_assert(!QREG || SINK, "queries from registers: one task per call, no hand-over of the next task's Q");
     int lane_l = threadIdx.x & 63;
     asm volatile("" : "+v"(lane_l));
     const int lane = lane_l;
@@ -172,9 +175,14 @@
   f32x4 qreg[NQ][4], kcur[NQ][4], vcur[NB][4];
   if (task >= 0) {
       const unsigned hb0 = head_base(task);
-      load_qk(qs, task % nkt, qreg, hb0, sub_of(task));
+      if constexpr (!QREG) load_qk(qs, task % nkt, qreg, hb0, sub_of(task));
       load_qk(ks, 0, kcur, hb0, sub_of(task));
       load_tile(vs, 0, vcur, hb0, second_block_bytes(task));
+      if constexpr (QREG) {
+          const f32x16 qf = qsrc();
+#pragma unroll
+          for (int s = 0; s < 4; ++s) qreg[0][s] = f32x4{qf[4 * s], qf[4 * s + 1], qf[4 * s + 2], qf[4 * s + 3]};
+      }
   }
   for (; task >= 0; ++round) {
     AFT_STAMP(lane == 0, stamps, task, 0);
diff --git a/adafortitran_amd/csrc/chain_device.h b/adafortitran_amd/csrc/chain_device.h
--- a/adafortitran_amd/csrc/chain_device.h
+++ b/adafortitran_amd/csrc/chain_device.h
@@ -35,7 +35,10 @@
     const float *fold_w;
     unsigned long long *stamps;
     int tpp;
+    int fold_q;
 };
+
+enum ChainL0 : int { kL0None = 0, kL0KeysValues = 1, kL0Self = 2, kL0SelfDefaultGrid = 3 };
 
 ChainArgs make_chain_args(const aft_config &c, const aft_layer_weights *mlp_w, const float *mlp_packed, const aft_layer_weights *qkv_w,
                           const float *qkv_packed, const float *attn, float *x, float *q, float *k, float *vt, int rows, int tokens,
@@ -175,16 +178,94 @@
     return acc;
 }
 
+template <bool DEFG = false>
+__device__ __forceinline__ void emb_gather(const ChainArgs &a, int plane, int tok, int h, float (&bv)[kFoldSteps]) {
+    constexpr int kSteps0 = 6;
+    const Srd srd_c = make_srd(a.emb_conv), srd_6 = make_srd(a.emb_tok6);
+    int zero = 0;
+    if constexpr (!DEFG) asm volatile("" : "+s"(zero));
+    const int p0 = DEFG ? 3 : a.emb_p0, p1 = DEFG ? 2 : a.emb_p1, T = DEFG ? 14 : a.emb_T, pk = p0 * p1, K = a.emb_K;
+    const int tpr = T / p1, g = tok / tpr, tc = tok - g * tpr;
+    const unsigned bc = (unsigned)((plane * a.emb_S + g * p0) * T + tc * p1) * 4;
+    const unsigned b6 = (unsigned)(((plane >> 1) * a.tokens + tok) * 6 - pk) * 4;
+    auto ld = [](Srd r, unsigned off) { return __builtin_bit_cast(float, __builtin_amdgcn_raw_buffer_load_b32(r, off, 0, 0)); };
+    int col = zero, rowoff = zero;
+    auto next = [&]() {
+        const int o = rowoff + col;
+        if (++col == p1) { col = 0; rowoff += T; }
+        return o;
+    };
+    auto step = [&](int st) {
+        const int k0 = 2 * st, o0 = next(), o1 = next();
+        float v = 0.f;
+        if (k0 + 1 < pk) {
+            v = ld(srd_c, bc + 4 * (unsigned)(h ? o1 : o0));
+        } else if (k0 >= pk) {
+            if (k0 < K) v = ld(srd_6, b6 + 4 * (unsigned)(k0 + h));
+            if (k0 + 1 >= K && h) v = 0.f;
+        } else {
+            const float v0 = ld(srd_c, bc + 4 * (unsigned)o0);
+            const float v1 = k0 + 1 < K ? ld(srd_6, b6 + 4 * (unsigned)(k0 + 1)) : 0.f;
+            v = h ? v1 : v0;
+        }
+        bv[st] = v;
+    };
+#pragma unroll
+    for (int st = 0; st < kFoldSteps; ++st) bv[st] = 0.f;
+#pragma unroll
+    for (int st = 0; st < kSteps0; ++st) step(st);
+    if (K > 2 * kSteps0) {
+#pragma unroll
+        for (int st = kSteps0; st < kFoldSteps; ++st) step(st);
+    }
+}
+
+template <int D>
+__device__ __forceinline__ f32x16 fold_q_tile(const ChainArgs &a, unsigned tok, int w, int lane, unsigned lo, const float (&bv)[kFoldSteps]) {
+    constexpr int W = D / 32, kSteps0 = 6;
+    const int h = lane >> 5;
+    const Srd srd_fw = make_srd(a.fold_w), srd_tq = make_srd(a.fold_w + 3 * W * kFoldSteps * 64);
+    f32x16 acc;
+#pragma unroll
+    for (int s = 0; s < 4; ++s) {
+        const f32x4 t = srd_load(srd_tq, (tok * D + 32 * w + 8 * s + 4 * h) * 4);
+#pragma unroll
+        for (int j = 0; j < 4; ++j) acc[4 * s + j] = t[j];
+    }
+    float wq[kFoldSteps];
+    auto frag = [&](int st) {
+        wq[st] = __builtin_bit_cast(float, __builtin_amdgcn_raw_buffer_load_b32(srd_fw, ((unsigned)((2 * W + w) * kFoldSteps + st) * 64 + lane + lo) * 4, 0, 0));
+    };
+    const bool more_steps = a.emb_K > 2 * kSteps0;
+#pragma unroll
+    for (int st = 0; st < kFoldSteps; ++st) wq[st] = 0.f;
+#pragma unroll
+    for (int st = 0; st < kSteps0; ++st) frag(st);
+    if (more_steps) {
+#pragma unroll
+        for (int st = kSteps0; st < kFoldSteps; ++st) frag(st);
+    }
+#pragma unroll
+    for (int st = 0; st < kSteps0; ++st) acc = __builtin_amdgcn_mfma_f32_32x32x2f32(wq[st], bv[st], acc, 0, 0, 0);
+    if (more_steps) {
+#pragma unroll
+        for (int st = kSteps0; st < kFoldSteps; ++st) acc = __builtin_amdgcn_mfma_f32_32x32x2f32(wq[st], bv[st], acc, 0, 0, 0);
+    }
+    return acc;
+}
+
 struct ChainNoPre {
     __device__ __forceinline__ void operator()(int) const {}
 };
 
-template <int D, int ACT, bool MLP, bool QKV, bool BS = false, bool PT = false, class Pre = ChainNoPre>
+template <int D, int ACT, bool MLP, bool QKV, bool BS = false, bool PT = false, class Pre = ChainNoPre, int L0 = kL0None>
 __device__ __forceinline__ void chain_body(const ChainArgs &a, float *smem, const int tid_in, const int first_tile,
                                            const int tile_stride, const int tile_end, Pre pre = Pre{}) {
     using S = ChainShape<D>;
     constexpr int W = S::WAVES;
     static_assert(!PT || !BS, "plane-aligned tiles are instantiated for the fp32 body");
+    static_assert(L0 == kL0None || (PT && (L0 == kL0KeysValues ? !MLP && QKV : MLP)), "ChainL0: the fused layer sequence's forms");
+    constexpr bool SELF = L0 == kL0Self || L0 == kL0SelfDefaultGrid;
     int tid = tid_in;
     asm volatile("" : "+v"(tid));
     float *xb = smem;
@@ -219,7 +300,7 @@
     constexpr int kFoldSteps0 = 6;
     float *emb_w = hb + S::XB;
     int *emb_offs = reinterpret_cast<int *>(emb_w + D * (kMaxPatchFeatures + 6));
-    if constexpr (!MLP) {
+    if constexpr (!MLP && L0 == kL0None) {
         if (a.emb_conv != nullptr) {
             const int pk = a.emb_p0 * a.emb_p1;
             for (int i = tid; i < D * a.emb_K; i += S::THREADS) emb_w[i] = a.emb_w1[i];
@@ -279,6 +360,8 @@
             plane = grow_n / a.tokens;
             tok = grow_n - plane * a.tokens;
         }
+        if constexpr (L0 != kL0None) emb_gather<L0 == kL0SelfDefaultGrid>(a, plane, tok, h, emb_bv);
+        if constexpr (L0 == kL0KeysValues) return;
         const int tpr = a.emb_T / a.emb_p1, g = tok / tpr, tc = tok - g * tpr;
         const float *cplane = a.emb_conv + ((size_t)plane * a.emb_S + g * a.emb_p0) * a.emb_T + tc * a.emb_p1;
         const float *t6 = a.emb_tok6 ? a.emb_tok6 + ((size_t)(plane >> 1) * a.tokens + tok) * 6 : nullptr;
@@ -289,6 +372,7 @@
 #pragma unroll
             for (int j = 0; j < 4; ++j) emb_acc0[4 * s + j] = b[j] + ps[j];
         }
+        if constexpr (L0 == kL0None) {
 #pragma unroll
         for (int st = 0; st < kEmbSteps; ++st) {
             const int k = 2 * st + h;
@@ -298,6 +382,21 @@
                 emb_bv[st] = off >= 0 ? cplane[off] : t6[~off];
             }
         }
+        }
+    };
+    auto embed_w1_rows = [&](const float *w1, float (&av)[kEmbSteps]) {
+#pragma unroll
+        for (int st = 0; st < kEmbSteps; ++st) {
+            const int k = 2 * st + h;
+            av[st] = k < a.emb_K ? w1[(fb + r) * a.emb_K + k] : 0.f;
+        }
+    };
+    auto embed_x0_on = [&](const float (&av)[kEmbSteps]) {
+        f32x16 acc0 = emb_acc0;
+#pragma unroll
+        for (int st = 0; st < kEmbSteps; ++st)
+            if (2 * st < a.emb_K) acc0 = __builtin_amdgcn_mfma_f32_32x32x2f32(av[st], emb_bv[st], acc0, 0, 0, 0);
+        return acc0;
     };
     if constexpr (!MLP) {
         if (a.emb_conv != nullptr && first_tile < tile_end) emb_request(first_tile);
@@ -408,7 +507,24 @@
     if constexpr (MLP) {
         f32x16 acc_o[1] = {bias_acc(srd_bo, fb, h)};
         gemm_preload<W, 1, PFD, 1>(ring_d, srd_wo, wo_lane);
-        if constexpr (PT) {
+        float l0_av[kEmbSteps];
+        if constexpr (SELF) {
+            emb_request(tile);
+            const Srd srd_e = make_srd(a.emb_w1);
+            auto w1_row = [&](int st) {
+                const int k = 2 * st + h;
+                const float v = __builtin_bit_cast(float, __builtin_amdgcn_raw_buffer_load_b32(srd_e, (unsigned)((fb + r) * a.emb_K + min(k, a.emb_K - 1)) * 4, 0, 0));
+                l0_av[st] = k < a.emb_K ? v : 0.f;
+            };
+#pragma unroll
+            for (int st = 0; st < kEmbSteps; ++st) l0_av[st] = 0.f;
+#pragma unroll
+            for (int st = 0; st < kFoldSteps0; ++st) w1_row(st);
+            if (a.emb_K > 2 * kFoldSteps0) {
+#pragma unroll
+                for (int st = kFoldSteps0; st < kEmbSteps; ++st) w1_row(st);
+            }
+        } else if constexpr (PT) {
             request_x_pt(tile, valid_pt);
         } else {
             request_attn(tile, AHEAD ? PFK : 0, W);
@@ -425,10 +541,16 @@
             gemm_run<W, 1, PFD, 1, 0>(ring_d, srd_wo, wo_lane, acc_o, [&](int kb, int s) { return of[kb][s]; });
         f32x16 acc_h[2] = {bias_acc(srd_b1, 2 * fb, h), bias_acc(srd_b1, 2 * fb + 32, h)};
         gemm_preload<W, 2, PFF, 1>(ring_ff, srd_w1, w1_lane);
+        if constexpr (SELF) {
+            const f32x16 x0 = embed_x0_on(l0_av);
+#pragma unroll
+            for (int e = 0; e < 16; ++e) cur[e] = acc_o[0][e] + x0[e];
+        } else {
 #pragma unroll
         for (int s = 0; s < 4; ++s)
 #pragma unroll
             for (int j = 0; j < 4; ++j) cur[4 * s + j] = acc_o[0][4 * s + j] + xres[s][j];
+        }
         AFT_STAMP(tid == 0, a.stamps, tile, 2);
         layernorm_rows<D>(cur, stats, par + fb, par + D + fb, w, r, h);
         AFT_STAMP(tid == 0, a.stamps, tile, 3);
@@ -516,17 +638,9 @@
         }
     } else {
         auto embed_x0 = [&]() {
-            f32x16 acc0 = emb_acc0;
             float av[kEmbSteps];
-#pragma unroll
-            for (int st = 0; st < kEmbSteps; ++st) {
-                const int k = 2 * st + h;
-                av[st] = k < a.emb_K ? emb_w[(fb + r) * a.emb_K + k] : 0.f;
-            }
-#pragma unroll
-            for (int st = 0; st < kEmbSteps; ++st)
-                if (2 * st < a.emb_K) acc0 = __builtin_amdgcn_mfma_f32_32x32x2f32(av[st], emb_bv[st], acc0, 0, 0, 0);
-            return acc0;
+            embed_w1_rows(emb_w, av);
+            return embed_x0_on(av);
         };
         auto store_x0 = [&](const f32x16 &v) {
             if (row_ok) {
@@ -542,10 +656,12 @@
                 }
             }
         };
-        if (fold) {
+        if (fold || L0 == kL0KeysValues) {
           if constexpr (!BS) {
-            gemm_preload<W, 1, PFD, 1>(ring_d, srd_wq, wq_lane);
-            const f32x16 x0 = embed_x0();
+            const bool fq = L0 == kL0KeysValues || a.fold_q != 0;
+            if (!fq) gemm_preload<W, 1, PFD, 1>(ring_d, srd_wq, wq_lane);
+            f32x16 x0;
+            if constexpr (L0 != kL0KeysValues) x0 = embed_x0();
             const unsigned tok_k = PT ? (unsigned)min(qt_pt * 32 + r, a.tokens - 1) : (unsigned)grow % (unsigned)a.tokens;
 #pragma unroll
             for (int s = 0; s < 4; ++s) {
@@ -584,11 +700,15 @@
 #pragma unroll
                 for (int st = kFoldSteps0; st < kEmbSteps; ++st) frag(st);
             }
-            store_x0(x0);
+            if constexpr (L0 != kL0KeysValues) store_x0(x0);
             float *xq = (round & 1) ? hb : xb;
-#pragma unroll
-            for (int s = 0; s < 4; ++s)
-                *reinterpret_cast<f32x4 *>(xq + (w * 4 + s) * 256 + lane * 4) = f32x4{x0[4 * s], x0[4 * s + 1], x0[4 * s + 2], x0[4 * s + 3]};
+            if constexpr (L0 != kL0KeysValues) {
+                if (!fq) {
+#pragma unroll
+                    for (int s = 0; s < 4; ++s)
+                        *reinterpret_cast<f32x4 *>(xq + (w * 4 + s) * 256 + lane * 4) = f32x4{x0[4 * s], x0[4 * s + 1], x0[4 * s + 2], x0[4 * s + 3]};
+                }
+            }
             auto kv_step = [&](int st) {
                 acc[1] = __builtin_amdgcn_mfma_f32_32x32x2f32(fold_wk[st], emb_bv[st], acc[1], 0, 0, 0);
                 acc[2] = __builtin_amdgcn_mfma_f32_32x32x2f32(emb_bv[st], fold_wv[st], acc[2], 0, 0, 0);
@@ -599,12 +719,18 @@
 #pragma unroll
                 for (int st = kFoldSteps0; st < kEmbSteps; ++st) kv_step(st);
             }
-            __syncthreads();
-            AFT_STAMP(tid == 0, a.stamps, tile, 9);
-            f32x16 acc_q[1];
-            auto xq_frag = [&](int kb, int s) { return *reinterpret_cast<const f32x4 *>(xq + (kb * 4 + s) * 256 + lane * 4); };
-            gemm_run<W, 1, PFD, 1, 0, decltype(xq_frag), 0x1>(ring_d, srd_wq, wq_lane, acc_q, xq_frag);
-            acc[0] = acc_q[0];
+            if constexpr (L0 != kL0KeysValues) {
+                if (fq) {
+                    acc[0] = fold_q_tile<D>(a, tok_k, w, lane, lo, emb_bv);
+                } else {
+                    __syncthreads();
+                    AFT_STAMP(tid == 0, a.stamps, tile, 9);
+                    f32x16 acc_q[1];
+                    auto xq_frag = [&](int kb, int s) { return *reinterpret_cast<const f32x4 *>(xq + (kb * 4 + s) * 256 + lane * 4); };
+                    gemm_run<W, 1, PFD, 1, 0, decltype(xq_frag), 0x1>(ring_d, srd_wq, wq_lane, acc_q, xq_frag);
+                    acc[0] = acc_q[0];
+                }
+            }
           }
         } else {
             gemm_preload<W, 3, PFQ, W>(ring_qkv, srd_wq, wq_lane);
@@ -634,7 +760,8 @@
             if (row_ok) {
 #pragma unroll
                 for (int s = 0; s < 4; ++s) {
-                    srd_store(srd_q, (ph_base + lane * 4 + s * 256) * 4, f32x4{acc[0][4 * s], acc[0][4 * s + 1], acc[0][4 * s + 2], acc[0][4 * s + 3]});
+                    if constexpr (L0 != kL0KeysValues)
+                        srd_store(srd_q, (ph_base + lane * 4 + s * 256) * 4, f32x4{acc[0][4 * s], acc[0][4 * s + 1], acc[0][4 * s + 2], acc[0][4 * s + 3]});
                     srd_store(srd_k, (ph_base + lane * 4 + s * 256) * 4, f32x4{acc[1][4 * s], acc[1][4 * s + 1], acc[1][4 * s + 2], acc[1][4 * s + 3]});
                 }
             }
diff --git a/adafortitran_amd/csrc/k_chain.hip b/adafortitran_amd/csrc/k_chain.hip
--- a/adafortitran_amd/csrc/k_chain.hip
+++ b/adafortitran_amd/csrc/k_chain.hip
@@ -117,6 +117,7 @@
         a.emb_K = c.patch_scs * c.patch_symbols + (fuse->tokens6 ? 6 : 0);
         if (fuse->fold_tk != nullptr && c.precision == AFT_PRECISION_F32) {
             a.fold_tk = fuse->fold_tk; a.fold_tvt = fuse->fold_tvt; a.fold_w = fuse->fold_w;
+            a.fold_q = fuse->fold_q ? 1 : 0;
         }
     }
     a.attn = attn;
diff --git a/adafortitran_amd/csrc/k_layer.hip b/adafortitran_amd/csrc/k_layer.hip
--- a/adafortitran_amd/csrc/k_layer.hip
+++ b/adafortitran_amd/csrc/k_layer.hip
@@ -26,6 +26,29 @@
     }
 };
 
+template <int D, int TOK, bool DEFG>
+struct LayerAttentionSelf {
+    const LayerArgs &a;
+    float *sink;
+    __device__ __forceinline__ void operator()(int tile) const {
+        const int w = __builtin_amdgcn_readfirstlane(threadIdx.x >> 6);
+        const int plane = tile / a.c.tpp, qt = tile - plane * a.c.tpp;
+        const int task = (plane * (D / kHeadDim) + w) * a.c.tpp + qt;
+        auto queries = [&]() {
+            int lane = threadIdx.x & 63;
+            unsigned lo = 0;
+            asm volatile("" : "+v"(lane), "+v"(lo));
+            const int tok = min(qt * kTile + (lane & 31), a.c.tokens - 1);
+            float bv[kFoldSteps];
+            emb_gather<DEFG>(a.c, plane, tok, lane >> 5, bv);
+            return fold_q_tile<D>(a.c, (unsigned)tok, w, lane, lo, bv);
+        };
+        attn_body<false, kHeadDim, TOK, true>(nullptr, a.ak, a.avt, a.qbias, nullptr, D / kHeadDim, a.c.tokens, a.c.tokpad, D, a.scale_log2e, task,
+                                              1 << 30, task + 1, nullptr, -1, sink + w * 1024, queries);
+        __syncthreads();
+    }
+};
+
 template <int D, int ACT, bool QKV, int TOK>
 __global__ __launch_bounds__(D * 2, 3) void layer_kernel(const LayerArgs a) {
     extern __shared__ __attribute__((aligned(16))) float smem[];
@@ -34,6 +57,25 @@
     if ((gridDim.x & 7) == 0) vblock = (blockIdx.x & 7) * (gridDim.x >> 3) + (blockIdx.x >> 3);
     chain_body<D, ACT, true, QKV, false, true>(a.c, smem, threadIdx.x, vblock, gridDim.x, a.planes * a.c.tpp,
                                                LayerAttention<D, TOK>{a, smem + S::XB + S::XB});
+}
+
+template <int D, int ACT, bool QKV, int TOK>
+__global__ __launch_bounds__(D * 2, 3) void layer0_self_kernel(const LayerArgs a) {
+    using Attention = LayerAttentionSelf<D, TOK, TOK == 280>;
+    extern __shared__ __attribute__((aligned(16))) float smem[];
+    using S = ChainShape<D>;
+    int vblock = blockIdx.x;
+    if ((gridDim.x & 7) == 0) vblock = (blockIdx.x & 7) * (gridDim.x >> 3) + (blockIdx.x >> 3);
+    chain_body<D, ACT, true, QKV, false, true, Attention, TOK == 280 ? kL0SelfDefaultGrid : kL0Self>(a.c, smem, threadIdx.x, vblock, gridDim.x,
+                                                                                                     a.planes * a.c.tpp, Attention{a, smem + S::XB + S::XB});
+}
+
+template <int D>
+__global__ __launch_bounds__(D * 2, 3) void fold_kv_tiles_kernel(const ChainArgs a, int planes) {
+    int vblock = blockIdx.x;
+    if ((gridDim.x & 7) == 0) vblock = (blockIdx.x & 7) * (gridDim.x >> 3) + (blockIdx.x >> 3);
+    extern __shared__ __attribute__((aligned(16))) float smem[];
+    chain_body<D, AFT_ACT_RELU, false, true, false, true, ChainNoPre, kL0KeysValues>(a, smem, threadIdx.x, vblock, gridDim.x, planes * a.tpp);
 }
 
 template <int D>
@@ -68,6 +110,22 @@
     return launch_plane_tiles(chain_plane_tiles_kernel<128>, a, planes, a.tpp, st, once, planes);
 }
 
+hipError_t launch_fold_kv_plane_tiles(const aft_config &c, const aft_layer_weights *qw, float *k, float *vt, int planes, int tokens, int tokpad,
+                                      hipStream_t st, const ChainFusion *fuse) {
+    if (!layer_fused_ok(c) || fuse == nullptr || fuse->conv_enhanced == nullptr || fuse->fold_tk == nullptr || !fuse->fold_q)
+        return hipErrorInvalidValue;
+    ChainArgs a = make_chain_args(c, nullptr, nullptr, qw, nullptr, nullptr, nullptr, nullptr, k, vt, planes * tokens, tokens, tokpad, fuse);
+    a.tpp = tokpad / kTile;
+    const int blocks = std::min(planes * a.tpp, current_device_cus() * 3);
+    hipLaunchKernelGGL(fold_kv_tiles_kernel<128>, dim3(blocks), dim3(ChainShape<128>::THREADS), 0, st, a, planes);
+    return hipGetLastError();
+}
+
+template <int ACT, bool QKV, int TOK>
+static hipError_t launch_layer_self_v(const LayerArgs &a, hipStream_t st) {
+    static PerDeviceOnce once;
+    return launch_plane_tiles(layer0_self_kernel<128, ACT, QKV, TOK>, a, a.planes, a.c.tpp, st, once);
+}
 template <int ACT, bool QKV, int TOK>
 static hipError_t launch_layer_v(const LayerArgs &a, hipStream_t st) {
     static PerDeviceOnce once;
@@ -75,16 +133,27 @@
 }
 template <int ACT, bool QKV>
 static hipError_t launch_layer_t(const LayerArgs &a, hipStream_t st) {
+    if (a.c.fold_q) {
+        const bool default_grid = a.c.tokens == 280 && a.c.emb_p0 == 3 && a.c.emb_p1 == 2 && a.c.emb_T == 14;
+        return default_grid ? launch_layer_self_v<ACT, QKV, 280>(a, st) : launch_layer_self_v<ACT, QKV, 0>(a, st);
+    }
     return a.c.tokens == 280 ? launch_layer_v<ACT, QKV, 280>(a, st) : launch_layer_v<ACT, QKV, 0>(a, st);
 }
 
 hipError_t launch_layer(const aft_config &c, const aft_layer_weights *m, const float *m_packed, const aft_layer_weights *qw,
                         const float *q_packed, float *x, float *q, const float *k_in, const float *vt_in, float *k_out, float *vt_out,
-                        int planes, int tokens, int tokpad, hipStream_t st, const ChainFusion *fuse) {
+                        int planes, int tokens, int tokpad, hipStream_t st, const ChainFusion *fuse, const ChainFusion *self) {
     if (!layer_fused_ok(c) || m == nullptr || k_in == k_out || vt_in == vt_out) return hipErrorInvalidValue;
     LayerArgs a{};
     a.c = make_chain_args(c, m, m_packed, qw, q_packed, nullptr, x, q, k_out, vt_out, planes * tokens, tokens, tokpad, fuse);
     a.c.tpp = tokpad / kTile;
+    if (self != nullptr) {
+        if (self->conv_enhanced == nullptr || self->fold_tk == nullptr || !self->fold_q) return hipErrorInvalidValue;
+        const ChainArgs e = make_chain_args(c, nullptr, nullptr, m, nullptr, nullptr, nullptr, nullptr, nullptr, nullptr, planes * tokens, tokens, tokpad, self);
+        a.c.emb_conv = e.emb_conv; a.c.emb_tok6 = e.emb_tok6; a.c.emb_w1 = e.emb_w1; a.c.emb_b1 = e.emb_b1; a.c.emb_pos = e.emb_pos;
+        a.c.emb_S = e.emb_S; a.c.emb_T = e.emb_T; a.c.emb_p0 = e.emb_p0; a.c.emb_p1 = e.emb_p1; a.c.emb_K = e.emb_K;
+        a.c.fold_w = e.fold_w; a.c.fold_q = e.fold_q;
+    }
     a.aq = q; a.ak = k_in; a.avt = vt_in;
     a.qbias = m->in_proj_b;
     a.scale_log2e = 1.4426950408889634f / sqrtf((float)kHeadDim);
diff --git a/adafortitran_amd/csrc/k_misc.hip b/adafortitran_amd/csrc/k_misc.hip
--- a/adafortitran_amd/csrc/k_misc.hip
+++ b/adafortitran_amd/csrc/k_misc.hip
@@ -103,15 +103,19 @@
 constexpr int kFoldTok = 2, kFoldChunk = 16;
 struct FoldArgs {
     const float *wkv, *bv;
+    const float *wq;
     const float *w1, *b1, *pos;
     float *tk, *tvt, *wf;
+    float *tq;
     int d, K, tokens, tokpad;
+    __device__ __forceinline__ int rows() const { return tq != nullptr ? 3 * d : 2 * d; }
+    __device__ __forceinline__ const float *row(int r) const { return r < 2 * d ? wkv + (size_t)r * d : wq + (size_t)(r - 2 * d) * d; }
 };
 inline size_t fold_tables_lds(int d) { return sizeof(float) * ((size_t)256 * (kFoldChunk + 1) + (size_t)kFoldTok * d); }
 
 __device__ __forceinline__ void fold_tables_body(const FoldArgs &f, int blk, float *sm) {
     float *sw = sm, *sc = sm + 256 * (kFoldChunk + 1);
-    const int tid = threadIdx.x, chunks = (2 * f.d + 255) / 256;
+    const int tid = threadIdx.x, chunks = (f.rows() + 255) / 256;
     const int t0 = (blk / chunks) * kFoldTok, row0 = (blk % chunks) * 256, row = row0 + tid;
     for (int i = tid; i < kFoldTok * f.d; i += 256) {
         const int tt = i / f.d, k = i - tt * f.d, t = t0 + tt;
@@ -127,7 +131,7 @@
         for (int m = 0; m < kPieces; ++m) {
             const int i = tid + 256 * m, rr = i / kPieces, c4 = (i % kPieces) * 4;
             piece[m] = f32x4{0.f, 0.f, 0.f, 0.f};
-            if (row0 + rr < 2 * f.d) piece[m] = *reinterpret_cast<const f32x4 *>(f.wkv + (size_t)(row0 + rr) * f.d + kc + c4);
+            if (row0 + rr < f.rows()) piece[m] = *reinterpret_cast<const f32x4 *>(f.row(row0 + rr) + kc + c4);
         }
     };
     request(0);
@@ -153,21 +157,23 @@
         const int t = t0 + tt;
         if (row < f.d) {
             if (t < f.tokens) f.tk[(size_t)t * f.d + row] = acc[tt];
-        } else if (row < 2 * f.d && t < f.tokpad) {
-            f.tvt[(size_t)(row - f.d) * f.tokpad + t] = t < f.tokens ? acc[tt] : 0.f;
+        } else if (row < 2 * f.d) {
+            if (t < f.tokpad) f.tvt[(size_t)(row - f.d) * f.tokpad + t] = t < f.tokens ? acc[tt] : 0.f;
+        } else if (row < f.rows() && t < f.tokens) {
+            f.tq[(size_t)t * f.d + row - 2 * f.d] = acc[tt];
         }
     }
 }
 
 __device__ __forceinline__ void fold_matrices_body(const FoldArgs &f, int blk) {
     const int o = blk * 256 + threadIdx.x, per_part = (f.d / 32) * kFoldSteps * 64;
-    if (o >= 2 * per_part) return;
+    if (o >= (f.tq != nullptr ? 3 : 2) * per_part) return;
     const int part = o / per_part, rem = o - part * per_part;
     const int wblock = rem / (kFoldSteps * 64), st = rem / 64 % kFoldSteps, lane = rem & 63;
     const int row = part * f.d + 32 * wblock + (lane & 31), k = 2 * st + (lane >> 5);
     float acc = 0.f;
     if (k < f.K) {
-        const float *wr = f.wkv + (size_t)row * f.d;
+        const float *wr = f.row(row);
         for (int j = 0; j < f.d; j += 4) {
             const f32x4 wv = *reinterpret_cast<const f32x4 *>(wr + j);
 #pragma unroll
@@ -210,7 +216,7 @@
     blk -= a.fold_matrix_blocks;
     if (blk < a.pack_blocks) {
         const size_t v = (size_t)blk * 256 + threadIdx.x, dd4 = (size_t)a.d * a.d / 4;
-        if (a.fold_table_blocks > 0 && v >= dd4 && v < 3 * dd4) return;
+        if (a.fold_table_blocks > 0 && v < 3 * dd4 && (v >= dd4 || a.fold.tq != nullptr)) return;
         pack_weights_vec(w, a.packed, a.d, 0, a.num_layers, a.split, v);
         return;
     }
@@ -278,9 +284,11 @@
         f.wkv = w.layers[0].in_proj_w + (size_t)f.d * f.d; f.bv = w.layers[0].in_proj_b + 2 * f.d;
         f.w1 = w.lin1_w; f.b1 = w.lin1_b; f.pos = w.pos;
         f.tk = fold->tk; f.tvt = fold->tvt; f.wf = fold->wf;
+        const int parts = fold->q ? 3 : 2;
+        if (fold->q) { f.wq = w.layers[0].in_proj_w; f.tq = fold->wf + 3 * fold_matrix_floats(f.d); }
         a.d = c.model_dim;
-        a.fold_table_blocks = (f.tokpad + kFoldTok - 1) / kFoldTok * ((2 * f.d + 255) / 256);
-        a.fold_matrix_blocks = (2 * (f.d / 32) * kFoldSteps * 64 + 255) / 256;
+        a.fold_table_blocks = (f.tokpad + kFoldTok - 1) / kFoldTok * ((parts * f.d + 255) / 256);
+        a.fold_matrix_blocks = (int)((parts * fold_matrix_floats(f.d) + 255) / 256);
         lds = std::max(lds, fold_tables_lds(f.d));
     }
     const int blocks = a.adapter_blocks + a.fold_table_blocks + a.fold_matrix_blocks + a.pack_blocks + a.frag_blocks + up_blocks;
diff --git a/adafortitran_amd/csrc/switches.h b/adafortitran_amd/csrc/switches.h
--- a/adafortitran_amd/csrc/switches.h
+++ b/adafortitran_amd/csrc/switches.h
@@ -2,7 +2,7 @@
 
 #define AFT_SWITCHES(X) \
     X(LANES, "AFT_LANES", "1 = never split a forward into lanes; 2 .. 4 = always that many shares (header section \"Lanes\")") \
-    X(L0_FOLD, "AFT_L0_FOLD", "0 = layer 0's keys and values by the model_dim-deep product over x0, not from the input features on the prologue's tables (DESIGN.md 4.1)") \
+    X(L0_FOLD, "AFT_L0_FOLD", "0 = layer 0's q, k, v by the model_dim-deep product over x0; 1 = k and v from the input features on the prologue's tables; 2 (default) = q as well, layer 0's launch rebuilds its queries and residual (DESIGN.md 4.1)") \
     X(LAYER_FUSED, "AFT_LAYER_FUSED", "0 = never the one-launch-per-layer sequence (k_layer.hip), 1 = wherever its shape is covered (default: where plane-aligned tiles add no round)") \
     X(PROLOGUE_NO_UP, "AFT_PROLOGUE_NO_UP", "measurement: the profiled prologue launch without the pilot upsampler product") \
     X(CONV_NSPLIT, "AFT_CONV_NSPLIT", "1 | 2 | 4 column ranges per plane in the streaming conv kernels (default: by the batch)") \
diff --git a/include/adafortitran_amd.h b/include/adafortitran_amd.h
--- a/include/adafortitran_amd.h
+++ b/include/adafortitran_amd.h
@@ -74,6 +74,8 @@
 
 size_t aft_workspace_bytes_layer_fused(const aft_config *cfg, int batch);
 int aft_layer_fused_of(const aft_config *cfg, int batch);
+
+int aft_l0_fold_of(const aft_config *cfg);
 
 #define AFT_MAX_LANES 4
 int aft_workspace_lanes(const aft_config *cfg, int batch, int *lanes, int *frames, size_t *offset_bytes);
```

Result: no change. 86150 frames/s, median of 2 (+0.2%).
